# CalebisGross/fresnel

Measured on AMD Instinct MI355X. Metric: composited Gaussian-pixels/sec + train-step ms, 512^2 render, higher is better.
Workload: dtype f32

## Files before the change

### fresnel_amd/_binding.py

```python
import ctypes
import os
import re

_HERE = os.path.dirname(os.path.abspath(__file__))
LIB_PATH = os.environ.get("FGS_LIB", os.path.join(_HERE, "_lib", "libfgs_hip.so"))

FGS_CAMERA_FLOATS = 24
FGS_TILE = 16

_PROTOTYPES = """
int fgs_workspace_bytes(FgsDims* dims, size_t* saved_bytes scratch_bytes)
int fgs_saved_layout(FgsDims* dims, FgsSavedLayout* layout)
int fgs_forward(FgsDims* dims, ptr cameras pos scale quat color opacity phase out_rgb out_depth saved scratch, stream)
int fgs_backward(FgsDims* dims, ptr cameras pos scale quat color opacity phase saved scratch g_rgb g_depth g_pos g_scale g_quat g_color
                 g_opacity g_phase, stream)
int fgs_count_pairs(FgsDims* dims, ptr saved out_pairs, stream)
int fgs_asm_workspace_bytes(FgsAsmDims* dims, size_t* saved_bytes scratch_bytes)
int fgs_asm_forward(FgsAsmDims* dims, ptr cameras pos scale quat color opacity phase wavelengths out_rgb saved scratch, stream)
int fgs_asm_backward(FgsAsmDims* dims, ptr cameras pos scale quat color opacity phase wavelengths saved scratch g_rgb g_pos g_scale
                     g_quat g_color g_opacity g_phase g_wavelengths, stream)
int fgs_wave_workspace_bytes(FgsWaveDims* dims, size_t* saved_bytes scratch_bytes)
int fgs_wave_forward(FgsWaveDims* dims, ptr cameras pos scale quat color opacity phase out_rgb out_depth saved scratch, stream)
int fgs_wave_backward(FgsWaveDims* dims, ptr cameras pos scale quat color opacity phase saved scratch g_rgb g_depth g_pos g_scale
                      g_quat g_color g_opacity g_phase, stream)
int fgs_fourier_workspace_bytes(FgsFourierDims* dims, size_t* saved_bytes scratch_bytes)
int fgs_fourier_forward(FgsFourierDims* dims, ptr cameras pos scale quat color opacity out_rgb saved scratch, stream)
int fgs_fourier_backward(FgsFourierDims* dims, ptr cameras pos scale quat color opacity saved scratch g_rgb g_pos g_scale g_quat
                         g_color g_opacity, stream)
int fgs_asm_propagate_workspace_bytes(int32_t height width channels, size_t* scratch_bytes)
int fgs_asm_propagate_forward(int32_t height width channels, double pixel_pitch, int32_t band_limit, ptr field z wavelengths out
                              spectrum scratch, stream)
int fgs_asm_propagate_backward(int32_t height width channels, double pixel_pitch, int32_t band_limit, ptr spectrum z wavelengths
                               g_out g_field g_z g_wavelengths scratch, stream)
int fgs_spectral_workspace_bytes(FgsSpectralDims* dims, size_t* saved_bytes scratch_bytes)
int fgs_spectral_loss_forward(FgsSpectralDims* dims, ptr rendered target depth wavelength loss saved scratch, stream)
int fgs_spectral_loss_backward(FgsSpectralDims* dims, ptr rendered target depth wavelength saved scratch g_loss g_rendered g_target
                               g_depth g_wavelength, stream)
int fgs_helmholtz_loss_forward(int32_t images height width, float wavelength pixel_spacing, ptr field loss residual scratch, stream)
int fgs_helmholtz_loss_backward(int32_t images height width, float wavelength pixel_spacing, ptr residual g_loss g_field, stream)
size_t fgs_reduction_scratch_bytes()
int fgs_ssim_workspace_bytes(FgsSsimDims* dims, size_t* saved_bytes scratch_bytes)
int fgs_ssim_forward(FgsSsimDims* dims, ptr x y out saved scratch, stream)
int fgs_ssim_backward(FgsSsimDims* dims, ptr x y saved g_out g_x g_y scratch, stream)
int fgs_pixel_loss_workspace_bytes(FgsPixelLossDims* dims, size_t* stats_bytes scratch_bytes)
int fgs_pixel_loss_stage1(FgsPixelLossDims* dims, ptr rendered target rendered_depth target_depth density out stats scratch, stream)
int fgs_pixel_loss_stage2(FgsPixelLossDims* dims, ptr rendered_depth target_depth stats scratch, stream)
int fgs_pixel_loss_stage3(FgsPixelLossDims* dims, ptr rendered_depth target_depth out stats scratch, stream)
int fgs_pixel_loss_forward(FgsPixelLossDims* dims, ptr rendered target rendered_depth target_depth density out stats scratch, stream)
int fgs_pixel_loss_backward(FgsPixelLossDims* dims, ptr rendered target rendered_depth target_depth density stats g_rgb g_boundary
                            g_depth g_rendered g_rendered_depth, stream)
int fgs_head_workspace_bytes(FgsHeadDims* dims, size_t* scratch_bytes)
int fgs_head_forward(FgsHeadDims* dims, ptr raw base_xy base_z pose opacity_mod edge positions scales rotations colors opacities
                     phases, stream)
int fgs_head_backward(FgsHeadDims* dims, ptr raw pose opacity_mod edge g_positions g_scales g_rotations g_colors g_opacities g_phases
                      g_raw g_base_z g_edge g_opacity_mod scratch, stream)
int fgs_nca_workspace_bytes(FgsNcaDims* dims, size_t* scratch_bytes)
int fgs_nca_perceive_forward(FgsNcaDims* dims, ptr state perception neighbors, stream)
int fgs_nca_perceive_backward(FgsNcaDims* dims, ptr neighbors g_perception g_state, stream)
int fgs_nca_update_forward(FgsNcaDims* dims, ptr state delta step_size uniform, float update_prob, ptr new_state, stream)
int fgs_nca_update_backward(FgsNcaDims* dims, ptr delta step_size uniform, float update_prob, ptr g_new_state g_delta g_step_size
                            scratch, stream)
int fgs_saag_workspace_bytes(FgsSaagDims* dims, size_t* scratch_bytes)
int fgs_saag_inputs_forward(FgsSaagDims* dims, ptr features positions scales rotations colors opacities mlp_inputs, stream)
int fgs_saag_refine_forward(FgsSaagDims* dims, ptr raw positions scales rotations colors opacities gains o_positions o_scales
                            o_rotations o_colors o_opacities pos_delta scale_delta color_delta opacity_delta, stream)
int fgs_saag_refine_backward(FgsSaagDims* dims, ptr raw scales rotations colors opacities gains g_positions g_scales g_rotations
                             g_colors g_opacities g_pos_delta g_scale_delta g_color_delta g_opacity_delta g_raw g_gains scratch, stream)
int fgs_physics_workspace_bytes(FgsPhysicsDims* dims, size_t* scratch_bytes)
int fgs_physics_forward(FgsPhysicsDims* dims, ptr raw base_xy base_z wavelength_raw positions scales rotations colors opacities phases
                        range scratch, stream)
int fgs_physics_backward(FgsPhysicsDims* dims, ptr raw base_z wavelength_raw range g_positions g_scales g_rotations g_colors
                         g_opacities g_phases g_raw g_base_z g_wavelength_raw scratch, stream)
int fgs_surface_workspace_bytes(FgsSurfaceDims* dims, FgsSurfaceParams* params, size_t* scratch_bytes)
int fgs_surface_count(FgsSurfaceDims* dims, FgsSurfaceParams* params, ptr depth scratch offsets, stream)
int fgs_surface_emit(FgsSurfaceDims* dims, FgsSurfaceParams* params, ptr depth color scratch offsets o_positions o_scales o_rotations
                     o_colors o_opacities, int64_t capacity, stream)
int fgs_surface_emit_guided(FgsSurfaceDims* dims, FgsSurfaceParams* params, ptr depth color scratch offsets mods, int32_t mods_h mods_w,
                            ptr o_positions o_scales o_rotations o_colors o_opacities point_rows, int64_t capacity, stream)
int fgs_surface_guided_backward_bytes(FgsSurfaceDims* dims, FgsSurfaceParams* params, int32_t mods_h mods_w, size_t* bytes)
int fgs_surface_guided_backward(FgsSurfaceDims* dims, FgsSurfaceParams* params, ptr depth scratch offsets mods, int32_t mods_h mods_w,
                                ptr point_rows g_positions g_scales g_rotations g_opacities g_mods bwd_scratch, stream)
int fgs_match_workspace_bytes(FgsMatchDims* dims, size_t* saved_bytes scratch_bytes)
int fgs_match_forward(FgsMatchDims* dims, ptr pred target pred_keep target_keep terms counts saved scratch, stream)
int fgs_match_backward(FgsMatchDims* dims, ptr pred target saved g_total g_pred scratch, stream)
int fgs_slat_workspace_bytes(int32_t batch voxels per_voxel, size_t* scratch_bytes)
int fgs_slat_head_forward(int32_t batch voxels per_voxel, ptr raw coords gains keep gaussians counts scratch, stream)
int fgs_slat_head_backward(int32_t batch voxels per_voxel, ptr raw coords gains g_gaussians g_raw g_gains scratch, stream)
int fgs_gather_forward(int32_t batch n_in n_out phase_channels, ptr indices pos scale quat color opacity phase o_pos o_scale o_quat
                       o_color o_opacity o_phase, stream)
int fgs_gather_backward(int32_t batch n_in n_out phase_channels, ptr indices g_o_pos g_o_scale g_o_quat g_o_color g_o_opacity
                        g_o_phase g_pos g_scale g_quat g_color g_opacity g_phase, stream)
int fgs_stage_timing_enable(int enable)
int fgs_stage_timing_read(ptr ms count)
str fgs_last_error()
str fgs_version()
"""


def _parse_prototypes(text):
    table = {}
    for ret, name, params in re.findall(r"(\S+) (fgs_\w+)\(([^)]*)\)", text):
        flat = []
        for kind, *names in (group.split() for group in params.split(",") if group.strip()):
            flat += [(kind, n) for n in names or [kind]]
        table[name] = (ret, tuple(flat))
    return table


SIGNATURES = _parse_prototypes(_PROTOTYPES)
EXPORTED_SYMBOLS = list(SIGNATURES)

STAGES = ["project", "depth_sort", "dup_emit", "tile_sort", "tile_ranges", "composite_fwd",
          "composite_bwd", "project_bwd", "splat_fwd", "field_fwd", "field_bwd", "splat_bwd"]


FWD_EXIT_OFF, FWD_EXIT_ON = 0x100, 0x200
BWD_ZERO_OFF, BWD_ZERO_ON = 0x400, 0x800
BWD_TAIL_OFF, BWD_TAIL_ON = 0x2000, 0x4000


class FgsDims(ctypes.Structure):
    _fields_ = [("batch", ctypes.c_int32), ("num_gaussians", ctypes.c_int32),
                ("width", ctypes.c_int32), ("height", ctypes.c_int32),
                ("max_radius", ctypes.c_float), ("background", ctypes.c_float * 3),
                ("use_phase", ctypes.c_int32), ("phase_amplitude", ctypes.c_float),
                ("num_cameras", ctypes.c_int32), ("saturation_skip", ctypes.c_int32),
                ("seg_len", ctypes.c_int32), ("fwd_variant", ctypes.c_int32), ("bin_mode", ctypes.c_int32),
                ("tile_w", ctypes.c_int32), ("sort_mode", ctypes.c_int32), ("dup_capacity", ctypes.c_uint32)]


class FgsSavedLayout(ctypes.Structure):
    _fields_ = [("total_bytes", ctypes.c_size_t), ("rec", ctypes.c_size_t),
                ("depth_key", ctypes.c_size_t), ("tile_count", ctypes.c_size_t),
                ("order", ctypes.c_size_t), ("dup_off", ctypes.c_size_t), ("counters", ctypes.c_size_t),
                ("ranges", ctypes.c_size_t), ("tile_order", ctypes.c_size_t), ("dup_ids", ctypes.c_size_t),
                ("pix_state", ctypes.c_size_t), ("phase_ckpt", ctypes.c_size_t),
                ("dup_capacity", ctypes.c_size_t),
                ("tiles_x", ctypes.c_int32), ("tiles_y", ctypes.c_int32),
                ("seg_off", ctypes.c_size_t), ("seg_tile", ctypes.c_size_t), ("seg_ckpt", ctypes.c_size_t),
                ("seg_capacity", ctypes.c_size_t), ("seg_len", ctypes.c_int32), ("tile_w", ctypes.c_int32),
                ("unit_order", ctypes.c_size_t), ("fwd_open", ctypes.c_size_t),
                ("fwd_close", ctypes.c_size_t), ("rank_of", ctypes.c_size_t)]


class FgsAsmDims(ctypes.Structure):
    _fields_ = [("batch", ctypes.c_int32), ("num_gaussians", ctypes.c_int32),
                ("width", ctypes.c_int32), ("height", ctypes.c_int32),
                ("max_radius", ctypes.c_float), ("background", ctypes.c_float * 3),
                ("num_planes", ctypes.c_int32), ("depth_near", ctypes.c_float),
                ("depth_far", ctypes.c_float), ("focal_depth", ctypes.c_float),
                ("pixel_pitch", ctypes.c_double), ("phase_channels", ctypes.c_int32),
                ("num_cameras", ctypes.c_int32), ("bin_mode", ctypes.c_int32)]


class FgsWaveDims(ctypes.Structure):
    _fields_ = [("batch", ctypes.c_int32), ("num_gaussians", ctypes.c_int32),
                ("width", ctypes.c_int32), ("height", ctypes.c_int32),
                ("max_radius", ctypes.c_float), ("background", ctypes.c_float * 3),
                ("phase_channels", ctypes.c_int32), ("num_cameras", ctypes.c_int32)]


class FgsFourierDims(ctypes.Structure):
    _fields_ = [("batch", ctypes.c_int32), ("num_gaussians", ctypes.c_int32),
                ("width", ctypes.c_int32), ("height", ctypes.c_int32),
                ("background", ctypes.c_float * 3), ("num_cameras", ctypes.c_int32)]


class FgsSpectralDims(ctypes.Structure):
    _fields_ = [("images", ctypes.c_int32), ("channels", ctypes.c_int32), ("height", ctypes.c_int32),
                ("width", ctypes.c_int32), ("mode", ctypes.c_int32), ("cutoff", ctypes.c_float),
                ("high_weight", ctypes.c_float), ("focal_depth", ctypes.c_float), ("reserved", ctypes.c_int32)]


FGS_SSIM_MAX_TAPS = 15
FGS_SSIM_GRAD_X, FGS_SSIM_GRAD_Y, FGS_SSIM_NONNEGATIVE, FGS_SSIM_PER_IMAGE = 1, 2, 4, 8


class FgsSsimDims(ctypes.Structure):
    _fields_ = [("images", ctypes.c_int32), ("channels", ctypes.c_int32), ("height", ctypes.c_int32),
                ("width", ctypes.c_int32), ("taps", ctypes.c_float * FGS_SSIM_MAX_TAPS), ("num_taps", ctypes.c_int32),
                ("c1", ctypes.c_float), ("c2", ctypes.c_float), ("flags", ctypes.c_int32)]


FGS_PIXEL_MAX_BOUNDARIES = 65
FGS_PIXEL_RGB, FGS_PIXEL_DENSITY, FGS_PIXEL_BOUNDARY, FGS_PIXEL_HARD_MASK, FGS_PIXEL_DEPTH = 1, 2, 4, 8, 16
(FGS_PIXEL_STAT_RGB, FGS_PIXEL_STAT_BOUNDARY, FGS_PIXEL_STAT_DEPTH, FGS_PIXEL_STAT_SUM_X, FGS_PIXEL_STAT_SUM_Y,
 FGS_PIXEL_STAT_SSD_X, FGS_PIXEL_STAT_SSD_Y, FGS_PIXEL_STAT_SGN, FGS_PIXEL_STAT_SGN_U) = range(9)
FGS_PIXEL_STAT_SLOTS = 16
FGS_PIXEL_CROSS_RANK = {1: slice(3, 5), 2: slice(5, 7), 3: slice(7, 9)}


class FgsPixelLossDims(ctypes.Structure):
    _fields_ = [("images", ctypes.c_int32), ("height", ctypes.c_int32), ("width", ctypes.c_int32),
                ("flags", ctypes.c_int32), ("world", ctypes.c_int32), ("vlm_weight", ctypes.c_float),
                ("threshold", ctypes.c_float), ("num_boundaries", ctypes.c_int32),
                ("boundaries", ctypes.c_float * FGS_PIXEL_MAX_BOUNDARIES)]


class FgsHeadDims(ctypes.Structure):
    _fields_ = [("batch", ctypes.c_int32), ("points", ctypes.c_int32), ("k_full", ctypes.c_int32),
                ("k_used", ctypes.c_int32), ("channels", ctypes.c_int32), ("xy_gain", ctypes.c_float),
                ("edge_scale_factor", ctypes.c_float), ("edge_opacity_boost", ctypes.c_float)]


class FgsNcaDims(ctypes.Structure):
    _fields_ = [("batch", ctypes.c_int32), ("points", ctypes.c_int32), ("state_dim", ctypes.c_int32), ("k", ctypes.c_int32)]


class FgsSaagDims(ctypes.Structure):
    _fields_ = [("batch", ctypes.c_int32), ("points", ctypes.c_int32), ("channels", ctypes.c_int32),
                ("grid_h", ctypes.c_int32), ("grid_w", ctypes.c_int32),
                ("feat_stride_batch", ctypes.c_int64), ("feat_stride_channel", ctypes.c_int64),
                ("feat_stride_row", ctypes.c_int64), ("residual_scale", ctypes.c_float)]


class FgsPhysicsDims(ctypes.Structure):
    _fields_ = [("batch", ctypes.c_int32), ("points", ctypes.c_int32), ("k_full", ctypes.c_int32), ("k_used", ctypes.c_int32),
                ("xy_gain", ctypes.c_float), ("focal_depth", ctypes.c_float),
                ("wavelength_min", ctypes.c_float), ("wavelength_max", ctypes.c_float)]


FGS_PHYSICS_RANGE_BYTES = 16


class FgsSurfaceDims(ctypes.Structure):
    _fields_ = [("batch", ctypes.c_int32), ("height", ctypes.c_int32), ("width", ctypes.c_int32)]


class FgsSurfaceParams(ctypes.Structure):
    _fields_ = [("fx", ctypes.c_float), ("fy", ctypes.c_float), ("cx", ctypes.c_float), ("cy", ctypes.c_float),
                ("depth_scale", ctypes.c_float), ("subsample", ctypes.c_int32), ("opacity", ctypes.c_float),
                ("normalize_extent", ctypes.c_float),
                ("base_size", ctypes.c_float), ("aspect_ratio", ctypes.c_float), ("edge_threshold", ctypes.c_float),
                ("edge_shrink", ctypes.c_float), ("min_confidence", ctypes.c_float), ("gradient_scale", ctypes.c_float),
                ("normal_strength", ctypes.c_float),
                ("wrap_enabled", ctypes.c_int32), ("wrap_edge_threshold", ctypes.c_float), ("wrap_layers", ctypes.c_int32),
                ("wrap_layer_spacing", ctypes.c_float), ("wrap_opacity_falloff", ctypes.c_float),
                ("wrap_max_angle", ctypes.c_float), ("wrap_aspect", ctypes.c_float),
                ("shell_enabled", ctypes.c_int32), ("shell_thickness", ctypes.c_float), ("shell_back_opacity", ctypes.c_float),
                ("shell_back_darken", ctypes.c_float), ("shell_connect_walls", ctypes.c_int32),
                ("shell_wall_segments", ctypes.c_int32), ("shell_wall_opacity", ctypes.c_float),
                ("shell_edge_threshold", ctypes.c_float),
                ("density_enabled", ctypes.c_int32), ("density_gradient_threshold", ctypes.c_float),
                ("density_extra_count", ctypes.c_int32), ("density_position_jitter", ctypes.c_float),
                ("density_size_variance", ctypes.c_float), ("density_opacity_scale", ctypes.c_float), ("seed", ctypes.c_uint32)]


FGS_SURFACE_STATE_OFFSET = 64
(FGS_SURFACE_KEPT, FGS_SURFACE_BASE, FGS_SURFACE_BACK, FGS_SURFACE_WALLS, FGS_SURFACE_WRAPS, FGS_SURFACE_FILLS) = (1, 2, 4, 8, 16, 32)


FGS_MATCH_TILE = 1024


class FgsMatchDims(ctypes.Structure):
    _fields_ = [("batch", ctypes.c_int32), ("num_pred", ctypes.c_int32), ("num_target", ctypes.c_int32),
                ("w_pos", ctypes.c_float), ("w_scale", ctypes.c_float), ("w_rot", ctypes.c_float),
                ("w_color", ctypes.c_float), ("w_opacity", ctypes.c_float), ("w_coverage", ctypes.c_float)]


class FgsError(RuntimeError):
    pass


_lib = None

_SCALARS = {"int": ctypes.c_int, "int32_t": ctypes.c_int32, "int64_t": ctypes.c_int64, "uint32_t": ctypes.c_uint32,
            "float": ctypes.c_float, "double": ctypes.c_double, "size_t": ctypes.c_size_t, "str": ctypes.c_char_p,
            "ptr": ctypes.c_void_p, "stream": ctypes.c_void_p}


def _ctype(kind):
    if kind.endswith("*"):
        return ctypes.POINTER(_SCALARS.get(kind[:-1]) or globals()[kind[:-1]])
    return _SCALARS[kind]


def load():
    global _lib
    if _lib is not None:
        return _lib
    if not os.path.exists(LIB_PATH):
        raise FgsError(
            f"{LIB_PATH} not found: build it with `python -m fresnel_amd.build` "
            "(hipcc --offload-arch=gfx950).  There is no CPU fallback for the HIP rasterizer.")
    import torch
    lib = ctypes.CDLL(LIB_PATH)
    for name, (ret, params) in SIGNATURES.items():
        fn = getattr(lib, name)
        fn.restype, fn.argtypes = _ctype(ret), [_ctype(kind) for kind, _ in params]
    if b"EXPERIMENT" in lib.fgs_version():
        import sys
        sys.stderr.write(f"fresnel_amd: loaded {LIB_PATH}: {lib.fgs_version().decode()}\n")
    _lib = lib
    return lib


def version():
    return load().fgs_version().decode()


def check(rc, what):
    if rc != 0:
        raise FgsError(f"{what} failed (rc={rc}): {load().fgs_last_error().decode()}")


def make_dims(batch, num_gaussians, width, height, max_radius=64.0, background=(0.0, 0.0, 0.0),
              use_phase=False, phase_amplitude=0.25, num_cameras=1, saturation_skip=False, tuning=None, dup_capacity=0):
    if isinstance(dup_capacity, bool) or int(dup_capacity) != dup_capacity or not 0 <= int(dup_capacity) <= 0xFFFFFFFF:
        raise FgsError(f"dup_capacity must be an integer in [0, 2^32), got {dup_capacity!r}")
    d = FgsDims()
    d.batch, d.num_gaussians, d.width, d.height = int(batch), int(num_gaussians), int(width), int(height)
    d.max_radius = float(max_radius)
    for i in range(3):
        d.background[i] = float(background[i])
    d.use_phase = 1 if use_phase else 0
    d.phase_amplitude = float(phase_amplitude)
    d.num_cameras = int(num_cameras)
    d.saturation_skip = 1 if saturation_skip else 0
    tuning = dict(tuning or {})
    fwd_exit = int(tuning.pop("fwd_exit", 0))
    bwd_zero = int(tuning.pop("bwd_zero", 0))
    bwd_tail = int(tuning.pop("bwd_tail", 0))
    for k, v in tuning.items():
        if k not in ("seg_len", "fwd_variant", "bin_mode", "tile_w", "sort_mode"):
            raise FgsError(f"unknown tuning field {k!r}")
        setattr(d, k, int(v))
    if fwd_exit not in (0, 1, -1) or (fwd_exit and d.fwd_variant < 0):
        raise FgsError(f"fwd_exit must be 0, 1 or -1, and 0 with the row-split forward (fwd_variant < 0), got {fwd_exit!r}")
    if bwd_zero not in (0, 1, -1) or (bwd_zero and d.fwd_variant < 0):
        raise FgsError(f"bwd_zero must be 0, 1 or -1, and 0 with the row-split forward (fwd_variant < 0), got {bwd_zero!r}")
    if bwd_tail not in (0, 1, -1) or (bwd_tail and d.fwd_variant < 0):
        raise FgsError(f"bwd_tail must be 0, 1 or -1, and 0 with the row-split forward (fwd_variant < 0), got {bwd_tail!r}")
    d.fwd_variant |= ({0: 0, 1: FWD_EXIT_ON, -1: FWD_EXIT_OFF}[fwd_exit] | {0: 0, 1: BWD_ZERO_ON, -1: BWD_ZERO_OFF}[bwd_zero]
                      | {0: 0, 1: BWD_TAIL_ON, -1: BWD_TAIL_OFF}[bwd_tail])
    d.dup_capacity = int(dup_capacity)
    return d


_SIZE_OUTS = {name: sum(kind == "size_t*" for kind, _ in params) for name, (_, params) in SIGNATURES.items()}


def sizes(name, *args):
    n = _SIZE_OUTS[name]
    out = [ctypes.c_size_t(0) for _ in range(n)]
    check(getattr(load(), name)(*[ctypes.byref(a) if isinstance(a, ctypes.Structure) else a for a in args],
                                *[ctypes.byref(o) for o in out]), name)
    return out[0].value if n == 1 else tuple(o.value for o in out)


def workspace_bytes(dims):
    return sizes("fgs_workspace_bytes", dims)


def saved_layout(dims):
    L = FgsSavedLayout()
    check(load().fgs_saved_layout(ctypes.byref(dims), ctypes.byref(L)), "fgs_saved_layout")
    return L


def stage_timing_enable(on=True, stages=None):
    mask = 1 if on else 0
    if on and stages is not None:
        mask = 0
        for name in stages:
            mask |= 1 << (STAGES.index(name) + 1)
    check(load().fgs_stage_timing_enable(mask), "fgs_stage_timing_enable")


def stage_timing_read():
    n = len(STAGES)
    ms = (ctypes.c_float * n)()
    cnt = (ctypes.c_int32 * n)()
    check(load().fgs_stage_timing_read(ms, cnt), "fgs_stage_timing_read")
    return {STAGES[i]: (float(ms[i]), int(cnt[i])) for i in range(n)}
```

### fresnel_amd/csrc/fgs_api.hip

```cpp
#include <stdarg.h>
#include <stdio.h>
#include <string.h>
#include "fgs_internal.h"

static thread_local char g_err[512] = "";

void fgs_set_error(const char *fmt, ...) {
    va_list ap;
    va_start(ap, fmt);
    vsnprintf(g_err, sizeof(g_err), fmt, ap);
    va_end(ap);
}

#include <mutex>
#include <stdlib.h>
#include <vector>
namespace {
struct StageRec { int stage; hipEvent_t a, b; };
std::mutex g_tm;
unsigned g_timing = 0;
std::vector<StageRec> g_recs;
std::vector<hipEvent_t> g_pool;
hipEvent_t g_open[FGS_NUM_STAGES];

// ... 27 lines not shown

namespace {
struct FillList { float *p[6]; unsigned long long n[6]; };

__global__ __launch_bounds__(256) void k_overflow_fill(const uint32_t *__restrict__ counters, FillList f, uint32_t word) {
    if (counters[1] == 0u) return;
    const float v = __uint_as_float(word);
    const float4 v4 = make_float4(v, v, v, v);
    const size_t stride = (size_t)gridDim.x * 256, t = (size_t)blockIdx.x * 256 + threadIdx.x;
#pragma unroll
    for (int k = 0; k < 6; ++k) {
        float *q = f.p[k];
        const size_t n = f.n[k], n4 = n >> 2;
        for (size_t i = t; i < n4; i += stride) reinterpret_cast<float4 *>(q)[i] = v4;
        for (size_t i = (n4 << 2) + t; i < n; i += stride) q[i] = v;
    }
}

int launch_overflow_fill(const char *saved, const FgsPlan &p, const FillList &f, uint32_t word, hipStream_t st) {
    size_t total = 0;
    for (int k = 0; k < 6; ++k) total += f.n[k];
    size_t grid = (total / 4 + 255) / 256;
    if (grid > 2048) grid = 2048;
    if (grid < 1) grid = 1;
    hipLaunchKernelGGL(k_overflow_fill, dim3((unsigned)grid), dim3(256), 0, st,
                       reinterpret_cast<const uint32_t *>(saved + p.L.counters), f, word);
    FGS_LAUNCH_CHECK("k_overflow_fill");
    return FGS_OK;
}
}

extern "C" {

const char *fgs_last_error(void) { return g_err; }

int fgs_stage_timing_enable(int enable) {
    std::lock_guard<std::mutex> lk(g_tm);
    g_timing = enable == 1 ? ~0u : ((unsigned)enable >> 1);
    return FGS_OK;
}

int fgs_stage_timing_read(float *ms, int32_t *count) {
    std::lock_guard<std::mutex> lk(g_tm);
    for (const StageRec &r : g_recs) {
        float t = 0.0f;
        if (hipEventSynchronize(r.b) == hipSuccess && hipEventElapsedTime(&t, r.a, r.b) == hipSuccess) {
            if (ms) ms[r.stage] += t;
            if (count) count[r.stage] += 1;
        }
        g_pool.push_back(r.a);
        g_pool.push_back(r.b);
    }
    g_recs.clear();
    return FGS_OK;
}
#ifdef FGS_EXPERIMENT_BUILD
#ifndef FGS_BUILD_DEFINES
#define FGS_BUILD_DEFINES "(defines not recorded)"
#endif
const char *fgs_version(void) { return "fgs-hip 0.3 (gfx950) EXPERIMENT BUILD, NOT THE PRODUCT: " FGS_BUILD_DEFINES; }
#else
const char *fgs_version(void) { return "fgs-hip 0.3 (gfx950)"; }
#endif

int fgs_workspace_bytes(const FgsDims *dims, size_t *saved_bytes, size_t *scratch_bytes) {
    FgsPlan p;
    const int rc = fgs_make_plan(dims, &p);
    if (rc) return rc;
    if (saved_bytes) *saved_bytes = p.L.total_bytes;
    if (scratch_bytes) *scratch_bytes = p.s_total;
    return FGS_OK;
}

int fgs_saved_layout(const FgsDims *dims, FgsSavedLayout *layout) {
    FgsPlan p;
    const int rc = fgs_make_plan(dims, &p);
    if (rc) return rc;
    if (!layout) { fgs_set_error("null layout"); return FGS_EINVAL; }
    *layout = p.L;
    return FGS_OK;
}

int fgs_forward(const FgsDims *dims, const float *cameras, const float *pos, const float *scale,
                const float *quat, const float *color, const float *opacity, const float *phase,
                float *out_rgb, float *out_depth, void *saved, void *scratch, void *stream) {
    FgsPlan p;
    int rc = fgs_make_plan(dims, &p);
    if (rc) return rc;
    if (!cameras || !pos || !scale || !quat || !color || !opacity || !out_rgb || !out_depth || !saved || !scratch) {
        fgs_set_error("fgs_forward: null pointer argument");
        return FGS_EINVAL;
    }
    if (p.d.use_phase && !phase) { fgs_set_error("fgs_forward: use_phase set but phase is NULL"); return FGS_EINVAL; }
    hipStream_t st = reinterpret_cast<hipStream_t>(stream);
    char *sv = reinterpret_cast<char *>(saved), *sc = reinterpret_cast<char *>(scratch);
    fgs_stage_begin(ST_PROJECT, st);
    const bool handoff = (p.d.sort_mode >> 1) == 3;
    if ((rc = fgs_launch_project(p, cameras, pos, scale, quat, color, opacity, sv, st, 0, 0.0f, 0.0f,
                                 handoff ? reinterpret_cast<uint32_t *>(sc + p.s_hist) : nullptr,
                                 (uint32_t)(FGS_SORT_HANDOFF_PASSES * (size_t)p.d.batch * 16 * 256)))) return rc;
    fgs_stage_end(ST_PROJECT, st);
    if ((rc = fgs_launch_binning(p, sv, sc, st))) return rc;
    fgs_stage_begin(ST_COMPOSITE_FWD, st);
    if ((rc = fgs_launch_composite_fwd(p, phase, sv, out_rgb, out_depth, st))) return rc;
    fgs_stage_end(ST_COMPOSITE_FWD, st);
    if (p.capacity_hinted) {
        const size_t hw = (size_t)p.d.width * p.d.height, B = p.d.batch;
        const FillList f = {{out_rgb, out_depth, nullptr, nullptr, nullptr, nullptr}, {B * 3 * hw, B * hw, 0, 0, 0, 0}};
        if ((rc = launch_overflow_fill(sv, p, f, 0x7FC00000u, st))) return rc;
    }
    return FGS_OK;
}

int fgs_backward(const FgsDims *dims, const float *cameras, const float *pos, const float *scale,
                 const float *quat, const float *color, const float *opacity, const float *phase,
                 const void *saved, void *scratch, const float *g_rgb, const float *g_depth,
                 float *g_pos, float *g_scale, float *g_quat, float *g_color, float *g_opacity,
                 float *g_phase, void *stream) {
    FgsPlan p;
    int rc = fgs_make_plan(dims, &p);
    if (rc) return rc;
    if (!cameras || !pos || !scale || !quat || !color || !opacity || !saved || !scratch || !g_rgb || !g_depth ||
        !g_pos || !g_scale || !g_quat || !g_color || !g_opacity) {
        fgs_set_error("fgs_backward: null pointer argument");
        return FGS_EINVAL;
    }
    if (p.d.use_phase && (!phase || !g_phase)) {
        fgs_set_error("fgs_backward: use_phase set but phase/g_phase is NULL");
        return FGS_EINVAL;
    }
    hipStream_t st = reinterpret_cast<hipStream_t>(stream);
    const char *sv = reinterpret_cast<const char *>(saved);
    char *sc = reinterpret_cast<char *>(scratch);
    fgs_stage_begin(ST_COMPOSITE_BWD, st);
    if ((rc = fgs_launch_composite_bwd(p, phase, sv, sc, g_rgb, g_depth, g_phase, st))) return rc;
    fgs_stage_end(ST_COMPOSITE_BWD, st);
    fgs_stage_begin(ST_PROJECT_BWD, st);
    if ((rc = fgs_launch_project_bwd(p, cameras, pos, scale, quat, sv,
                                     reinterpret_cast<const float *>(sc + p.s_grows), g_pos, g_scale, g_quat,
                                     g_color, g_opacity, p.d.use_phase ? g_phase : nullptr, st,
                                     reinterpret_cast<float *>(sc + p.s_rsum),
                                     p.bwd_tail ? reinterpret_cast<const uint32_t *>(sc + p.s_zero_from) : nullptr)))
        return rc;
    fgs_stage_end(ST_PROJECT_BWD, st);
    if (p.capacity_hinted) {
        const size_t bn = (size_t)p.d.batch * p.d.num_gaussians;
        const FillList f = {{g_pos, g_scale, g_quat, g_color, g_opacity, p.d.use_phase ? g_phase : nullptr},
                            {bn * 3, bn * 3, bn * 4, bn * 3, bn, p.d.use_phase ? bn : 0}};
        if ((rc = launch_overflow_fill(sv, p, f, 0u, st))) return rc;
    }
    return FGS_OK;
}

int fgs_count_pairs(const FgsDims *dims, const void *saved, uint64_t *out_pairs, void *stream) {
    FgsPlan p;
    const int rc = fgs_make_plan(dims, &p);
    if (rc) return rc;
    if (!saved || !out_pairs) { fgs_set_error("fgs_count_pairs: null pointer"); return FGS_EINVAL; }
    return fgs_launch_count_pairs(p, reinterpret_cast<const char *>(saved), out_pairs,
                                  reinterpret_cast<hipStream_t>(stream));
}

}
```

### fresnel_amd/csrc/fgs_composite.hip

```cpp
#include <type_traits>
#include "fgs_internal.h"
#include "fgs_wave.h"

#if (defined(FGS_BWD_DYN_LDS) || defined(FGS_BWD_WIDE_WAVES) || defined(FGS_PHASE_SCAN) || defined(FGS_CKPT_NT) || defined(FGS_PHASE_WAVE_BLOCKS) || \
     defined(FGS_BWD_UNIT_TRACE) || defined(FGS_BWD_TILE_ORDER) || defined(FGS_FWD_HEAD_ENTRIES)) && !defined(FGS_EXPERIMENT_BUILD)
#error "work-split / timing switches of this unit are for experiment builds: python -m fresnel_amd.build --define ... (sets FGS_EXPERIMENT_BUILD; fgs_version() then says so)"
#endif

namespace {

typedef float v2f __attribute__((ext_vector_type(2)));
constexpr float FGS_SATURATION_EPS = 2.98023223876953125e-8f;
constexpr float NEG_HALF_LOG2E = -0.72134752044448170368f;
constexpr float ALPHA_MAX = 0.99f;
constexpr float INV_ALPHA_MAX = 1.0f / 0.99f;
constexpr float PHASE_KAPPA = 2.0f * 3.14159f;

__device__ __forceinline__ float phase_cos(float x) {
    const float y = x - 1.57079632679489661923f, y2 = y * y;
    float p = 2.6089300414764439e-6f;
    p = p * y2 - 1.9811111665926607e-4f;
    p = p * y2 + 8.3330881539788702e-3f;
    p = p * y2 - 1.6666660461917662e-1f;
    return -(y + y * (y2 * p));
// ... 314 lines not shown
            Cr[s] = nt_load(k); Cg[s] = nt_load(k + PL); Cb[s] = nt_load(k + 2 * PL); T[s] = nt_load(k + 3 * PL); Dm[s] = nt_load(k + 4 * PL);
            nt_store(k + 3 * PL, 1.0f - T[s]);
        }
        wstart = c.start + hs * seg_len;
    }
    const uint32_t wend = (!REST || mine) ? pend : wstart;
    for (uint32_t base = wstart; base < wend; base += 64) {
        const uint32_t n = min(64u, wend - base);
        if (base != wstart && ((base - c.start) % seg_len) == 0) {
            float *ck = slot0 + (size_t)((base - c.start) / seg_len) * SLOT;
#pragma unroll
            for (int s = 0; s < 4; ++s) ckpt_store<PL>(ck + cell(s), BlendState{Cr[s], Cg[s], Cb[s], T[s], Dm[s]});
        }
        blend_fwd_chunk(sh0[wave], sh1[wave], sh2[wave], lane, base, n, X0, c.Y0, dup_ids, rec, ln, T, Cr, Cg, Cb, Dm);
    }
    const uint32_t last = nseg ? (nseg - 1) / spp : 0u;
    if (NP > 1 && nseg > spp) {
        if (active && part != 0 && (!REST || mine)) {
            float *ck = (part == last) ? slot0 : slot0 + (size_t)((part + 1) * spp) * SLOT;
#pragma unroll
            for (int s = 0; s < 4; ++s) ckpt_store<PL>(ck + cell(s), BlendState{Cr[s], Cg[s], Cb[s], T[s], Dm[s]});
        }
        __threadfence_block();
        __syncthreads();
        if (part != 0 || (REST && !mine)) return;
        {
            float *ck = slot0 + (size_t)spp * SLOT;
#pragma unroll
            for (int s = 0; s < 4; ++s) ckpt_store<PL>(ck + cell(s), BlendState{Cr[s], Cg[s], Cb[s], T[s], Dm[s]});
        }
        for (uint32_t pp = 1; pp <= last; ++pp) {
            const float *src = (pp == last) ? slot0 : slot0 + (size_t)((pp + 1) * spp) * SLOT;
            float *dst = slot0 + (size_t)((pp + 1) * spp) * SLOT;
#pragma unroll
            for (int s = 0; s < 4; ++s) {
                const BlendState acc = compose(BlendState{Cr[s], Cg[s], Cb[s], T[s], Dm[s]}, ckpt_load<PL>(src + cell(s)));
                Cr[s] = acc.Cr; Cg[s] = acc.Cg; Cb[s] = acc.Cb; T[s] = acc.T; Dm[s] = acc.D;
                if (pp != last) ckpt_store<PL>(dst + cell(s), acc);
            }
        }
    } else if (part != 0 || (REST && !mine)) {
        return;
    }
    const size_t HW = (size_t)W * H;
#pragma unroll
    for (int s = 0; s < 4; ++s) {
        const uint32_t px = X0 + 8u * (s & 1) + lx, py = c.Y0 + 8u * (s >> 1) + ly;
        if (px < W && py < H)
            pixel_store(pix_state, out_rgb, out_depth, c.b, HW, (size_t)py * W + px, bg0, bg1, bg2, Cr[s], Cg[s], Cb[s], 1.0f - T[s],
                        T[s], Dm[s]);
    }
}

template <int WIDE>
__global__ __launch_bounds__(64 * (1 + WIDE)) __attribute__((amdgpu_waves_per_eu(8, 8))) void k_blend_fwd_head(
    uint32_t tiles, uint32_t tiles_x, uint32_t W, uint32_t H, float bg0, float bg1, float bg2,
    const uint32_t *__restrict__ tile_order, const uint32_t *__restrict__ ranges,
    const uint32_t *__restrict__ dup_ids, const float *__restrict__ rec, float *__restrict__ pix_state,
    float *__restrict__ out_rgb, float *__restrict__ out_depth, const uint32_t *__restrict__ seg_off,
    float *__restrict__ seg_ckpt, uint32_t seg_len, uint32_t order_groups, uint32_t *__restrict__ fwd_open, uint32_t head_segs,
    uint32_t np, const uint32_t *__restrict__ fwd_max, uint32_t max_recs, uint32_t *__restrict__ fwd_close) {
    constexpr int NW = 1 + WIDE;
    constexpr int TSX = WIDE ? 4 : 2;
    constexpr int PL = 2 * TSX * 64, SLOT = 5 * PL;
    __shared__ float4 sh0[NW][64], sh1[NW][64], sh2[NW][64];
    const uint32_t slot_in_order = order_groups > 1u ? fgs_xcd_remap(blockIdx.x, gridDim.x) : blockIdx.x;
    const TileCtx c = tile_ctx_of(tile_order[slot_in_order], tiles, tiles_x, ranges, 8u * TSX);
    const uint32_t lane = threadIdx.x & 63u;
    const uint32_t half = WIDE ? __builtin_amdgcn_readfirstlane(threadIdx.x >> 6) : 0u;
    const uint32_t X0 = c.X0 + 16u * half;
    const uint32_t lx = lane & 7u, ly = lane >> 3;
    const uint32_t len = c.end - c.start;
    const uint32_t nseg = (len + seg_len - 1) / seg_len;
    const uint32_t spp = (nseg + np - 1) / np;
    const uint32_t hs = np == 1u ? nseg : min(spp, head_segs);
    const uint32_t hlen = min(len, hs * seg_len);
    float *slot0 = seg_ckpt + (size_t)seg_off[c.tile] * SLOT + 2u * half * 64u + lane;
    auto cell = [](int s) { return ((s >> 1) * TSX + (s & 1)) * 64; };
    uint32_t kcb = 0u, kdb = 0u;
    {
        const uint32_t *fm = fwd_max + (size_t)c.b * max_recs * 2u;
        for (uint32_t i = lane; i < max_recs; i += 64u) { kcb = max(kcb, fm[2u * i]); kdb = max(kdb, fm[2u * i + 1u]); }
#pragma unroll
        for (int o = 32; o > 0; o >>= 1) { kcb = max(kcb, (uint32_t)__shfl_xor(kcb, o, 64)); kdb = max(kdb, (uint32_t)__shfl_xor(kdb, o, 64)); }
        kcb = max(max(kcb, __float_as_uint(bg0) & 0x7FFFFFFFu), max(__float_as_uint(bg1) & 0x7FFFFFFFu, __float_as_uint(bg2) & 0x7FFFFFFFu));
    }
    const float Kc = __uint_as_float(__builtin_amdgcn_readfirstlane(kcb)), Kd = __uint_as_float(__builtin_amdgcn_readfirstlane(kdb));
    bool inframe[4];
#pragma unroll
    for (int s = 0; s < 4; ++s) inframe[s] = X0 + 8u * (s & 1) + lx < W && c.Y0 + 8u * (s >> 1) + ly < H;
    float T[4], Cr[4], Cg[4], Cb[4], Dm[4];
#pragma unroll
    for (int s = 0; s < 4; ++s) { T[s] = 1.0f; Cr[s] = 0; Cg[s] = 0; Cb[s] = 0; Dm[s] = 0; }
    BlendLane ln = {lx, 16u + ly, (float)(X0 + lx), (float)(X0 + lx + 8u), (float)(c.Y0 + ly)};
    asm("" : "+v"(ln.fx0), "+v"(ln.fx1), "+v"(ln.fy0));
    constexpr float Q = 1.490116119384765625e-8f;
    uint32_t done = 0;
    bool closed = false;
    while (done < hlen && !closed) {
        if (done != 0u && (done % seg_len) == 0) {
            float *ck = slot0 + (size_t)(done / seg_len) * SLOT;
#pragma unroll
            for (int s = 0; s < 4; ++s) ckpt_store<PL>(ck + cell(s), BlendState{Cr[s], Cg[s], Cb[s], T[s], Dm[s]});
        }
        const uint32_t n = min(64u, hlen - done);
        blend_fwd_chunk(sh0[half], sh1[half], sh2[half], lane, c.start + done, n, X0, c.Y0, dup_ids, rec, ln, T, Cr, Cg, Cb, Dm);
        done += n;
        bool veto = false;
#pragma unroll
        for (int s = 0; s < 4; ++s) {
            const float tc = T[s] * Kc;
            const bool ok = T[s] <= Q && tc < Q * fabsf(Cr[s]) && tc < Q * fabsf(Cg[s]) && tc < Q * fabsf(Cb[s]) && T[s] * Kd < Q * fabsf(Dm[s]);
            veto |= inframe[s] && !ok;
        }
        closed = __ballot(veto) == 0ull;
    }
    const bool finished = closed || done == len;
    const uint32_t kclose = (done + seg_len - 1) / seg_len;
    const bool close_slot = closed && kclose < nseg;
    if (lane == 0) {
        fwd_open[2u * c.tile + half] = finished ? 0u : 1u;
        fwd_close[2u * c.tile + half] = close_slot ? kclose : 0xFFFFFFFFu;
    }
    if (!WIDE && lane == 1) fwd_close[2u * c.tile + 1u] = 0xFFFFFFFFu;
    if (!finished) {
        float *ck = slot0 + (size_t)hs * SLOT;
#pragma unroll
        for (int s = 0; s < 4; ++s) {
            float *k = ck + cell(s);
            nt_store(k, Cr[s]); nt_store(k + PL, Cg[s]); nt_store(k + 2 * PL, Cb[s]); nt_store(k + 3 * PL, T[s]); nt_store(k + 4 * PL, Dm[s]);
        }
        return;
    }
    const size_t HW = (size_t)W * H;
#pragma unroll
    for (int s = 0; s < 4; ++s) {
        const uint32_t px = X0 + 8u * (s & 1) + lx, py = c.Y0 + 8u * (s >> 1) + ly;
        if (px < W && py < H)
            pixel_store(pix_state, out_rgb, out_depth, c.b, HW, (size_t)py * W + px, bg0, bg1, bg2, Cr[s], Cg[s], Cb[s], 1.0f - T[s],
                        T[s], Dm[s]);
    }
    if (close_slot) {
        float *ck = slot0 + (size_t)kclose * SLOT;
#pragma unroll
        for (int s = 0; s < 4; ++s) ckpt_store<PL>(ck + cell(s), BlendState{Cr[s], Cg[s], Cb[s], T[s], Dm[s]});
    }
}

__shared__ float4 bwd_sh0[CH], bwd_sh1[CH], bwd_sh2[CH];
__shared__ uint32_t bwd_she[CH];
__shared__ __attribute__((aligned(16))) float bwd_red[10 * FGS_RED_PITCH];
__shared__ __attribute__((aligned(16))) float bwd_red_pairs[12 * FGS_RED_PITCH];
#define FGS_BWD_G __attribute__((address_space(1)))

template <int NSX, bool DEAD>
__device__ __forceinline__ void composite_bwd_walk(const TileCtx &c, uint32_t lane, uint32_t lx, uint32_t ly, uint32_t dcap, uint32_t alive,
                                                   const uint32_t *__restrict__ dup_ids, const float *__restrict__ rec,
                                                   const uint32_t *__restrict__ dup_off, float *__restrict__ grad_rows,
                                                   const float (&gr)[2 * NSX], const float (&gg)[2 * NSX], const float (&gb)[2 * NSX],
                                                   const float (&gd)[2 * NSX], float (&S)[2 * NSX], float (&T)[2 * NSX]) {
    constexpr int NS = 2 * NSX;
    constexpr bool ROW_MOMENTS = NSX == 4;
    auto &sh0 = bwd_sh0; auto &sh1 = bwd_sh1; auto &sh2 = bwd_sh2; auto &she = bwd_she;
    auto &red = *[]() { if constexpr (NSX == 4) return &bwd_red_pairs; else return &bwd_red; }();
    const uint32_t shx = lx, shy = 16u + ly;
    float fx0 = (float)(c.X0 + lx), fy0 = (float)(c.Y0 + ly);
    asm("" : "+v"(fx0), "+v"(fy0));
    uint32_t e_prev = ~0u;
    auto reduce_parked = [&]() {
        const float tot = wave_sum_addtid_finish(red, lane, 10u);
        if ((lane & 3u) == 3u && lane < 4u * FGS_BLEND_ROW_FLOATS && e_prev < dcap) ((FGS_BWD_G float *)grad_rows)[(size_t)e_prev * FGS_BLEND_ROW_FLOATS + (lane >> 2)] = tot;
    };
    constexpr bool PAIRS = NSX == 4;
    constexpr uint32_t DSUMS = 6, DROWS = PAIRS ? 2 : 1, DZERO = FGS_BLEND_ROW_FLOATS - DSUMS;
    static_assert(4 * DSUMS * DROWS + DROWS * DZERO <= 64, "dead walk: one lane per zero float behind the sums' lanes");
    [[maybe_unused]] uint32_t e_prevB = ~0u;
    [[maybe_unused]] auto reduce_parked_dead = [&]() {
        const float tot = wave_sum_addtid_finish(red, lane, DSUMS * DROWS);
        const uint32_t k = lane >> 2, z = lane - 4u * DSUMS * DROWS;
        const bool sum_lane = (lane & 3u) == 3u && k < DSUMS * DROWS, zero_lane = lane >= 4u * DSUMS * DROWS && z < DROWS * DZERO;
        const bool second = sum_lane ? k >= DSUMS : z >= DZERO;
        const uint32_t col = sum_lane ? (second ? k - DSUMS : k) : DSUMS + (second ? z - DZERO : z);
        const uint32_t e = PAIRS && second ? e_prevB : e_prev;
        if ((sum_lane || zero_lane) && e < dcap) ((FGS_BWD_G float *)grad_rows)[(size_t)e * FGS_BLEND_ROW_FLOATS + col] = tot;
    };
    struct DeadTerms {
        float ca, dya, dyb, bdya, bdyb, cyya, cyyb, dxs[NSX];
        uint32_t mxs[NSX], my0, my1, msk, cflag;
    };
    [[maybe_unused]] auto dead_terms = [&](const float4 &q0, const float4 &q1, const float4 &q2, const uint32_t fl) {
        DeadTerms t;
        t.msk = fl & alive;
        t.cflag = fl & 256u;
        asm("" : "+s"(t.cflag));
        const uint32_t cbits = __float_as_uint(q2.z), rbits = __float_as_uint(q2.w);
        const float cbc = q0.w, cd = q1.x, lop = q1.y;
        t.ca = q0.z;
        const float dxa = fx0 - q0.x;
        t.dya = fy0 - q0.y; t.dyb = t.dya + 8.0f;
        t.bdya = cbc * t.dya; t.bdyb = cbc * t.dyb; t.cyya = fmaf(cd * t.dya, t.dya, lop); t.cyyb = fmaf(cd * t.dyb, t.dyb, lop);
        asm("" : "+v"(t.bdya), "+v"(t.bdyb), "+v"(t.cyya), "+v"(t.cyyb));
#pragma unroll
        for (int col = 0; col < NSX; ++col) {
            t.mxs[col] = (uint32_t)__builtin_amdgcn_sbfe((int)cbits, shx + 8u * col, 1);
            t.dxs[col] = dxa + 8.0f * col;
        }
        t.my0 = (uint32_t)__builtin_amdgcn_sbfe((int)rbits, shy, 1); t.my1 = (uint32_t)__builtin_amdgcn_sbfe((int)rbits, shy + 8u, 1);
        return t;
    };
    [[maybe_unused]] auto dead_passes = [&](const DeadTerms &t, float (&vals)[DSUMS]) {
        float v_mx = 0, v_my = 0, v_ca = 0, v_cbc = 0, v_cd = 0, v_op = 0;
        float mA[2] = {0.0f, 0.0f}, mB[2] = {0.0f, 0.0f}, mC[2] = {0.0f, 0.0f};
        auto pass = [&](const int s) {
            const int col = s % NSX, row = s / NSX;
            const float dx = t.dxs[col], dy = row ? t.dyb : t.dya;
            const uint32_t mk = t.mxs[col] & (row ? t.my1 : t.my0);
            const float tt = __builtin_fmaf(dx, t.ca, row ? t.bdyb : t.bdya);
            const float a1 = blend_alpha1(__builtin_fmaf(tt, dx, row ? t.cyyb : t.cyya), mk);
            float dalpha = S[s] * __builtin_amdgcn_rcpf(a1 - INV_ALPHA_MAX);
            uint32_t cf = t.cflag;
            asm("" : "+s"(cf));
            if (!cf) dalpha = select_lt1(a1, dalpha);
            float dG = dalpha * a1;
            asm("" : "+v"(dG));
            if constexpr (ROW_MOMENTS) {
                mA[row] = __builtin_fmaf(dalpha, a1, mA[row]);
                float dmx = dG * dx;
                asm("" : "+v"(dmx));
                mB[row] = __builtin_fmaf(dG, dx, mB[row]); mC[row] = __builtin_fmaf(dmx, dx, mC[row]);
            } else {
                v_op = __builtin_fmaf(dalpha, a1, v_op);
                float dmx = dG * dx, dmy = dG * dy;
                asm("" : "+v"(dmx), "+v"(dmy));
                v_mx = __builtin_fmaf(dG, dx, v_mx); v_my = __builtin_fmaf(dG, dy, v_my);
                v_ca = __builtin_fmaf(dmx, dx, v_ca); v_cbc = __builtin_fmaf(dmx, dy, v_cbc); v_cd = __builtin_fmaf(dmy, dy, v_cd);
            }
        };
#pragma unroll
        for (int s = 0; s < NS; ++s) {
            if (!((t.msk >> s) & 1u)) continue;
            pass(s);
        }
        if constexpr (ROW_MOMENTS) {
            v_op = mA[0] + mA[1]; v_mx = mB[0] + mB[1]; v_ca = mC[0] + mC[1];
            float t0 = t.dya * mA[0], t1 = t.dyb * mA[1];
            asm("" : "+v"(t0), "+v"(t1));
            float p0 = t0 * t.dya, pb = mB[0] * t.dya;
            asm("" : "+v"(p0), "+v"(pb));
            v_my = __builtin_fmaf(mA[1], t.dyb, t0);
            v_cd = __builtin_fmaf(t1, t.dyb, p0);
            v_cbc = __builtin_fmaf(mB[1], t.dyb, pb);
        }
        vals[0] = v_mx; vals[1] = v_my; vals[2] = v_ca; vals[3] = v_cbc; vals[4] = v_cd; vals[5] = v_op;
    };
    [[maybe_unused]] auto dead_chunk = [&](const uint32_t n) {
        for (uint32_t j = 0; j < n; j += DROWS) {
            const float4 a0 = sh0[j], a1 = sh1[j], a2 = sh2[j];
            uint32_t eA = __builtin_amdgcn_readfirstlane(she[j]), eB = ~0u;
            float4 b0 = a0, b1 = a1, b2 = a2;
            if constexpr (PAIRS) {
                b0 = sh0[j + 1]; b1 = sh1[j + 1]; b2 = sh2[j + 1];
                eB = __builtin_amdgcn_readfirstlane(she[j + 1]);
            }
            reduce_parked_dead();
            asm volatile("" : "+s"(eA), "+s"(eB));
            const bool paired = PAIRS && j + 1 < n;
            e_prev = eA; e_prevB = paired ? eB : ~0u;
            const uint32_t flA = __builtin_amdgcn_readfirstlane(__float_as_uint(a2.w));
            const DeadTerms ta = dead_terms(a0, a1, a2, flA);
            float va[DSUMS];
            if constexpr (PAIRS) {
                const uint32_t flB = paired ? __builtin_amdgcn_readfirstlane(__float_as_uint(b2.w)) : 0u;
                const DeadTerms tb = dead_terms(b0, b1, b2, flB);
                float vb[DSUMS];
                dead_passes(ta, va);
                addtid_park(red, va);
                dead_passes(tb, vb);
                addtid_park(red + DSUMS * FGS_RED_PITCH, vb);
            } else {
                dead_passes(ta, va);
                addtid_park(red, va);
            }
        }
    };
    for (uint32_t base = c.start; base < c.end; base += CH) {
        const uint32_t n = __builtin_amdgcn_readfirstlane(min((uint32_t)CH, c.end - base));
        uint32_t sl;
        asm volatile("v_mbcnt_lo_u32_b32 %0, -1, 0\n\tv_mbcnt_hi_u32_b32 %0, -1, %0" : "=v"(sl));
        if (sl < n) {
            const uint32_t gid = ((FGS_BWD_G const uint32_t *)dup_ids)[base + sl];
            const float4 *r = reinterpret_cast<const float4 *>(rec + (size_t)gid * FGS_REC_FLOATS);
            float4 q2 = r[2];
            const uint32_t bbx = __float_as_uint(q2.z), bby = __float_as_uint(q2.w);
            she[sl] = fgs_emission_slot<8 * NSX>(c.tx, c.ty, gid, bbx, bby, dup_off);
            float4 q0 = r[0], q1 = r[1];
            const bool conic_ok = q0.z > 0.0f && q1.x > 0.0f && 3.996f * q0.z * q1.x > q0.w * q0.w;
            uint32_t flags, cbits;
            stage_decode_w<NSX>(c.X0, c.Y0, bbx, bby, q1.y, flags, cbits, conic_ok);
            blend_stage_fold(q0, q1, q2, flags, cbits, fgs_opacity_floored(q1.y) ? FGS_FOLD_FLOOR_LOG2 : blend_lop(q1.y));
            sh0[sl] = q0; sh1[sl] = q1; sh2[sl] = q2;
        }
        __syncthreads();
        if constexpr (DEAD) dead_chunk(n);
        for (uint32_t j = 0; !DEAD && j < n; ++j) {
            const float4 q0 = sh0[j], q1 = sh1[j], q2 = sh2[j];
            uint32_t e = __builtin_amdgcn_readfirstlane(she[j]);
            reduce_parked();
            asm volatile("" : "+s"(e));
            e_prev = e;
            const uint32_t fl = __builtin_amdgcn_readfirstlane(__float_as_uint(q2.w));
            const uint32_t msk = fl & alive;
            const uint32_t cbits = __float_as_uint(q2.z), rbits = __float_as_uint(q2.w);
            const float ca = q0.z, cbc = q0.w, cd = q1.x, lop = q1.y;
            const float dxa = fx0 - q0.x, dya = fy0 - q0.y, dyb = dya + 8.0f;
            float bdya = cbc * dya, bdyb = cbc * dyb, cyya = fmaf(cd * dya, dya, lop), cyyb = fmaf(cd * dyb, dyb, lop);
            asm("" : "+v"(bdya), "+v"(bdyb), "+v"(cyya), "+v"(cyyb));
            float v_mx = 0, v_my = 0, v_ca = 0, v_cbc = 0, v_cd = 0, v_op = 0, v_r = 0, v_g = 0, v_b = 0, v_d = 0;
            float mA[2] = {0.0f, 0.0f}, mB[2] = {0.0f, 0.0f}, mC[2] = {0.0f, 0.0f};
            {
                uint32_t cflag = fl & 256u;
                asm("" : "+s"(cflag));
                uint32_t mxs[NSX];
                float dxs[NSX];
#pragma unroll
                for (int col = 0; col < NSX; ++col) {
                    mxs[col] = (uint32_t)__builtin_amdgcn_sbfe((int)cbits, shx + 8u * col, 1);
                    dxs[col] = dxa + 8.0f * col;
                }
                const uint32_t my0 = (uint32_t)__builtin_amdgcn_sbfe((int)rbits, shy, 1), my1 = (uint32_t)__builtin_amdgcn_sbfe((int)rbits, shy + 8u, 1);
                auto pass = [&](const int s, const uint32_t mk) {
                    const int col = s % NSX, row = s / NSX;
                    const float dx = dxs[col], dy = row ? dyb : dya;
                    const float t = ca * dx + (row ? bdyb : bdya);
                    const float a1 = blend_alpha1(t * dx + (row ? cyyb : cyya), mk);
                    const float w = a1 * T[s];
                    const float q = gr[s] * q1.z + gg[s] * q1.w + gb[s] * q2.x + gd[s] * q2.y;
                    S[s] -= w * q;
                    float dalpha = T[s] * q - S[s] * __builtin_amdgcn_rcpf(INV_ALPHA_MAX - a1);
                    T[s] = fmaf(w, -ALPHA_MAX, T[s]);
                    uint32_t cf = cflag;
                    asm("" : "+s"(cf));
                    if (!cf) dalpha = select_lt1(a1, dalpha);
                    const float dG = dalpha * a1;
                    if constexpr (ROW_MOMENTS) {
                        mA[row] += dG;
                        const float dmx = dG * dx;
                        mB[row] += dmx; mC[row] += dmx * dx;
                    } else {
                        v_op += dG;
                        const float dmx = dG * dx, dmy = dG * dy;
                        v_mx += dmx; v_my += dmy;
                        v_ca += dmx * dx; v_cbc += dmx * dy; v_cd += dmy * dy;
                    }
                    v_r += w * gr[s]; v_g += w * gg[s]; v_b += w * gb[s]; v_d += w * gd[s];
                };
#pragma unroll
                for (int s = 0; s < NS; ++s) {
                    if (!((msk >> s) & 1u)) continue;
                    pass(s, mxs[s % NSX] & (s / NSX ? my1 : my0));
                }
                if constexpr (ROW_MOMENTS) {
                    v_op = mA[0] + mA[1]; v_mx = mB[0] + mB[1]; v_ca = mC[0] + mC[1];
                    const float t0 = dya * mA[0], t1 = dyb * mA[1];
                    v_my = t0 + t1;
                    v_cd = dya * t0 + dyb * t1;
                    v_cbc = dya * mB[0] + dyb * mB[1];
                }
            }
            {
                const float vals[10] = {v_mx, v_my, v_ca, v_cbc, v_cd, v_op, v_r, v_g, v_b, v_d};
                addtid_park(red, vals);
            }
        }
        __syncthreads();
    }
    if constexpr (DEAD) reduce_parked_dead(); else reduce_parked();
}

template <int NSX>
struct BwdDeadArgs {
    TileCtx c;
    uint32_t dcap;
    uint32_t alive;
    const uint32_t *dup_ids; const float *rec; const uint32_t *dup_off; float *grad_rows;
    float S[2 * NSX];
};
template <int NSX>
__device__ __attribute__((noinline)) void composite_bwd_dead_walk(BwdDeadArgs<NSX> a) {
    const uint32_t lane = threadIdx.x;
    float z[2 * NSX] = {}, T[2 * NSX] = {};
    const uint32_t alive = __builtin_amdgcn_readfirstlane(a.alive);
    composite_bwd_walk<NSX, true>(a.c, lane, lane & 7u, lane >> 3, a.dcap, alive, a.dup_ids, a.rec, a.dup_off, a.grad_rows, z, z, z, z,
                                  a.S, T);
}

template <int NSX>
__device__ __attribute__((noinline)) void composite_bwd_zero_rows(TileCtx c, uint32_t dcap, const uint32_t *__restrict__ dup_ids,
                                                                  const float *__restrict__ rec, const uint32_t *__restrict__ dup_off,
                                                                  float *__restrict__ grad_rows) {
    static_assert(FGS_BLEND_ROW_FLOATS % 2 == 0 && FGS_BLEND_ROW_FLOATS >= 4, "zero rows: stored as pairs, floats 1 and 3 in the first two");
    const float fy7 = (float)(c.Y0 + 7u);
    for (uint32_t i = c.start + threadIdx.x; i < c.end; i += 64) {
        const uint32_t gid = dup_ids[i];
        const float *r = rec + (size_t)gid * FGS_REC_FLOATS;
        const float4 q2 = reinterpret_cast<const float4 *>(r)[2];
        const uint32_t e = fgs_emission_slot<8 * NSX>(c.tx, c.ty, gid, __float_as_uint(q2.z), __float_as_uint(q2.w), dup_off);
        uint32_t zy = 0u;
        if constexpr (NSX == 4) {
            float dya = fy7 - r[1];
            asm("" : "+v"(dya));
            if (dya + 8.0f < 0.0f) zy = 0x80000000u;
        }
        if (e < dcap) {
            uint2 *row = reinterpret_cast<uint2 *>(grad_rows + (size_t)e * FGS_BLEND_ROW_FLOATS);
            row[0] = make_uint2(0u, zy); row[1] = make_uint2(0u, zy);
#pragma unroll
            for (int q = 2; q < FGS_BLEND_ROW_FLOATS / 2; ++q) row[q] = make_uint2(0u, 0u);
        }
    }
}

template <int NSX>
__device__ __forceinline__ bool composite_bwd_prologue(const TileCtx &c, uint32_t unit, uint32_t seg, uint32_t rebase_seg,
                                                       const uint32_t (&kclose)[NSX / 2], uint32_t lane, uint32_t lx, uint32_t ly,
                                                       uint32_t W, uint32_t H, float bg0, float bg1, float bg2,
                                                       const float *__restrict__ seg_ckpt, const float *__restrict__ pix_state,
                                                       const float *__restrict__ g_rgb, const float *__restrict__ g_depth,
                                                       float (&gr)[2 * NSX], float (&gg)[2 * NSX], float (&gb)[2 * NSX],
                                                       float (&gd)[2 * NSX], float (&S)[2 * NSX], float (&T)[2 * NSX]) {
    constexpr int NS = 2 * NSX, PL = NS * 64, SLOT = 5 * PL;
    const size_t HW = (size_t)W * H;
    bool live_px = false;
#pragma unroll
    for (int s = 0; s < NS; ++s) {
        const uint32_t px = c.X0 + 8u * (s % NSX) + lx, py = c.Y0 + 8u * (s / NSX) + ly;
        gr[s] = gg[s] = gb[s] = gd[s] = S[s] = 0.0f;
        T[s] = 1.0f;
        if (px < W && py < H) {
            const PixelGrad g = pixel_grad_load(pix_state, g_rgb, g_depth, c.b, HW, (size_t)py * W + px, bg0, bg1, bg2);
            gr[s] = g.gr; gg[s] = g.gg; gb[s] = g.gb; gd[s] = g.gd;
            const float bgs = __builtin_fmaf(gb[s], bg2, __builtin_fmaf(gg[s], bg1, gr[s] * bg0));
            S[s] = __builtin_fmaf(bgs, g.Tf, __builtin_fmaf(gd[s], g.D, __builtin_fmaf(gb[s], g.Cb, __builtin_fmaf(gg[s], g.Cg, gr[s] * g.Cr))));
        }
        if (seg) {
            const bool behind = seg >= kclose[(s % NSX) >> 1];
            const size_t own = behind ? (size_t)unit - seg + kclose[(s % NSX) >> 1] : (size_t)unit;
            BlendState st = ckpt_load<PL>(seg_ckpt + own * SLOT + s * 64 + lane);
            if (rebase_seg != seg && !behind) {
                const size_t slot = (size_t)unit - seg + rebase_seg;
                st = compose(ckpt_load<PL>(seg_ckpt + slot * SLOT + s * 64 + lane), st);
            }
            T[s] = st.T;
            S[s] -= __builtin_fmaf(gd[s], st.D, __builtin_fmaf(gb[s], st.Cb, __builtin_fmaf(gg[s], st.Cg, gr[s] * st.Cr)));
            if (px < W && py < H && T[s] != 0.0f) live_px = true;
        }
    }
    return live_px;
}

template <int NSX>
__device__ __forceinline__ uint32_t composite_bwd_nonzero_subtiles(const float (&S)[2 * NSX]) {
    uint32_t walk = 0u;
#pragma unroll
    for (int s = 0; s < 2 * NSX; ++s)
        if (__ballot((__float_as_uint(S[s]) & 0x7FFFFFFFu) != 0u) != 0ull) walk |= 1u << s;
    return walk;
}

template <int NSX>
__global__ __launch_bounds__(64) void k_bwd_tail_verdict(
    uint32_t ntiles, uint32_t tiles, uint32_t tiles_x, uint32_t W, uint32_t H, float bg0, float bg1, float bg2, uint32_t dcap,
    const uint32_t *__restrict__ counters, const uint32_t *__restrict__ seg_off, const float *__restrict__ seg_ckpt,
    const uint32_t *__restrict__ ranges, const uint32_t *__restrict__ dup_ids, const float *__restrict__ pix_state,
    const float *__restrict__ g_rgb, const float *__restrict__ g_depth, const uint32_t *__restrict__ fwd_close,
    const uint32_t *__restrict__ rank_of, uint32_t *__restrict__ zero_from) {
    constexpr int NS = 2 * NSX;
    const uint32_t tile = blockIdx.x;
    if (tile >= ntiles) return;
    const uint32_t lane = threadIdx.x;
    uint32_t verdict = 0xFFFFFFFFu;
    const TileCtx c = tile_ctx_of(tile, tiles, tiles_x, ranges, 8u * NSX);
    const uint32_t seg_len = counters[4];
    uint32_t kclose[NSX / 2], seg = 0u;
#pragma unroll
    for (int h = 0; h < NSX / 2; ++h) { kclose[h] = fwd_close[2u * tile + h]; seg = max(seg, kclose[h]); }
    const uint32_t len = c.end - c.start;
    const bool tail = c.end > c.start && seg_len != 0u && seg != 0xFFFFFFFFu && seg != 0u && (unsigned long long)seg * seg_len < len &&
                      (unsigned long long)c.start + (unsigned long long)seg * seg_len < dcap;
    if (tail) {
        float gr[NS], gg[NS], gb[NS], gd[NS], S[NS], T[NS];
        const bool live_px = composite_bwd_prologue<NSX>(c, seg_off[tile] + seg, seg, seg, kclose, lane, lane & 7u, lane >> 3, W, H, bg0, bg1,
                                                         bg2, seg_ckpt, pix_state, g_rgb, g_depth, gr, gg, gb, gd, S, T);
        if (__ballot(live_px) == 0ull && composite_bwd_nonzero_subtiles<NSX>(S) == 0u) verdict = rank_of[dup_ids[c.start + seg * seg_len]];
    }
    if (lane == 0) zero_from[tile] = verdict;
}

__global__ __launch_bounds__(256) void k_bwd_tail_min(uint32_t tiles, uint32_t *__restrict__ zero_from) {
    __shared__ uint32_t part[4];
    const uint32_t *z = zero_from + (size_t)blockIdx.x * tiles;
    uint32_t m = 0xFFFFFFFFu;
    for (uint32_t t = threadIdx.x; t < tiles; t += 256u) m = min(m, z[t]);
#pragma unroll
    for (int o = 32; o > 0; o >>= 1) m = min(m, (uint32_t)__shfl_xor(m, o, 64));
    if ((threadIdx.x & 63u) == 0u) part[threadIdx.x >> 6] = m;
    __syncthreads();
    if (threadIdx.x == 0) zero_from[(size_t)gridDim.x * tiles + blockIdx.x] = min(min(part[0], part[1]), min(part[2], part[3]));
}

#ifndef FGS_BWD_WIDE_WAVES
#define FGS_BWD_WIDE_WAVES 5
#endif
#ifndef FGS_BWD_DYN_LDS
#define FGS_BWD_DYN_LDS 0
#endif
#ifdef FGS_BWD_UNIT_TRACE
#define FGS_BWD_TRACE_PARAM , unsigned long long *__restrict__ trace
#define FGS_BWD_TRACE_EXIT(dead)                                                                                        \
    do {                                                                                                                \
        if (threadIdx.x == 0) {                                                                                         \
            trace[3 * (size_t)blockIdx.x + 1] = wall_clock64();                                                         \
            trace[3 * (size_t)blockIdx.x + 2] = (unsigned long long)unit | ((unsigned long long)(dead) << 32) | (1ull << 63); \
        }                                                                                                               \
    } while (0)
#else
#define FGS_BWD_TRACE_PARAM
#define FGS_BWD_TRACE_EXIT(dead) do { } while (0)
#endif
template <int NSX>
__global__ __launch_bounds__(64) __attribute__((amdgpu_waves_per_eu(NSX == 2 ? 6 : FGS_BWD_WIDE_WAVES, NSX == 2 ? 6 : FGS_BWD_WIDE_WAVES))) void k_composite_bwd(
    uint32_t tiles, uint32_t tiles_x, uint32_t W, uint32_t H, float bg0, float bg1, float bg2, uint32_t dcap,
    const uint32_t *__restrict__ counters, const uint32_t *__restrict__ seg_off,
    const uint32_t *__restrict__ seg_tile, const float *__restrict__ seg_ckpt, const uint32_t *__restrict__ ranges,
    const uint32_t *__restrict__ dup_ids, const float *__restrict__ rec, const uint32_t *__restrict__ dup_off,
    const float *__restrict__ pix_state, const float *__restrict__ g_rgb, const float *__restrict__ g_depth,
    float *__restrict__ grad_rows, float t_eps, const uint32_t *__restrict__ unit_order,
    const uint32_t *__restrict__ fwd_close, uint32_t zero_units, const uint32_t *__restrict__ zero_from FGS_BWD_TRACE_PARAM) {
    constexpr int NS = 2 * NSX, PL = NS * 64, SLOT = 5 * PL;
    const uint32_t num_units = counters[2];
    if (blockIdx.x >= num_units) return;
#ifdef FGS_BWD_UNIT_TRACE
    if (threadIdx.x == 0) trace[3 * (size_t)blockIdx.x] = wall_clock64();
#endif
#ifdef FGS_BWD_TILE_ORDER
    const uint32_t unit = fgs_xcd_remap(blockIdx.x, num_units);
#else
    const uint32_t unit = unit_order[fgs_xcd_remap(blockIdx.x, num_units)];
#endif
    const uint32_t seg_len = counters[4];
    const uint32_t fwd_parts = (int32_t)counters[5] > 1 ? counters[5] : 0u;
    const uint32_t unit_tile = seg_tile[unit];
    uint32_t kclose[NSX / 2];
#pragma unroll
    for (int h = 0; h < NSX / 2; ++h) kclose[h] = 0xFFFFFFFFu;
    if (fwd_close) {
#pragma unroll
        for (int h = 0; h < NSX / 2; ++h) kclose[h] = fwd_close[2u * unit_tile + h];
    }
    const uint32_t seg = unit - seg_off[unit_tile];
    if (zero_from) {
        bool tail = true;
#pragma unroll
        for (int h = 0; h < NSX / 2; ++h) tail = tail && seg >= kclose[h];
        if (tail && zero_from[unit_tile] != 0xFFFFFFFFu) {
            FGS_BWD_TRACE_EXIT(5);
            return;
        }
    }
    TileCtx c = tile_ctx_of(unit_tile, tiles, tiles_x, ranges, 8u * NSX);
    uint32_t rebase_seg = seg;
    if (fwd_parts > 1) {
        const uint32_t nseg = (c.end - c.start + seg_len - 1) / seg_len;
        const uint32_t spp = (nseg + fwd_parts - 1) / fwd_parts, first = seg / spp * spp;
        if (first != 0) rebase_seg = first;
    }
    c.start += seg * seg_len;
    c.end = min(c.end, c.start + seg_len);
    const uint32_t lane = threadIdx.x;
    const uint32_t lx = lane & 7u, ly = lane >> 3;
    if (t_eps > 0.0f) {
        const uint32_t live = reinterpret_cast<const uint32_t *>(seg_ckpt + (size_t)seg_off[unit_tile] * SLOT)[0];
        if (seg >= live) {
            for (uint32_t i = c.start + lane; i < c.end; i += 64) {
                const uint32_t gid = dup_ids[i];
                const float4 q2 = reinterpret_cast<const float4 *>(rec + (size_t)gid * FGS_REC_FLOATS)[2];
                const uint32_t e = fgs_emission_slot<8 * NSX>(c.tx, c.ty, gid, __float_as_uint(q2.z), __float_as_uint(q2.w), dup_off);
                if (e < dcap) {
                    float2 *row = reinterpret_cast<float2 *>(grad_rows + (size_t)e * FGS_BLEND_ROW_FLOATS);
#pragma unroll
                    for (int q = 0; q < FGS_BLEND_ROW_FLOATS / 2; ++q) row[q] = make_float2(0.0f, 0.0f);
                }
            }
            FGS_BWD_TRACE_EXIT(2);
            return;
        }
    }
    float gr[NS], gg[NS], gb[NS], gd[NS], S[NS], T[NS];
    const bool live_px = composite_bwd_prologue<NSX>(c, unit, seg, rebase_seg, kclose, lane, lx, ly, W, H, bg0, bg1, bg2, seg_ckpt, pix_state,
                                                     g_rgb, g_depth, gr, gg, gb, gd, S, T);
    const bool dead_unit = seg != 0 && !(t_eps > 0.0f) && __ballot(live_px) == 0ull;
    uint32_t alive = (1u << NS) - 1u;
    if (t_eps > 0.0f) {
        alive = 0u;
#pragma unroll
        for (int s = 0; s < NS; ++s)
            if (__ballot(T[s] >= t_eps) != 0ull) alive |= 1u << s;
    }
    if (dead_unit) {
        uint32_t walk = (1u << NS) - 1u;
        if (zero_units) {
            walk = composite_bwd_nonzero_subtiles<NSX>(S);
            if (walk == 0u) {
                composite_bwd_zero_rows<NSX>(c, dcap, dup_ids, rec, dup_off, grad_rows);
                FGS_BWD_TRACE_EXIT(3);
                return;
            }
        }
        BwdDeadArgs<NSX> a;
        a.c = c; a.dcap = dcap; a.alive = walk; a.dup_ids = dup_ids; a.rec = rec; a.dup_off = dup_off; a.grad_rows = grad_rows;
#pragma unroll
        for (int s = 0; s < NS; ++s) a.S[s] = S[s];
        composite_bwd_dead_walk<NSX>(a);
        FGS_BWD_TRACE_EXIT(walk == (1u << NS) - 1u ? 1 : 4);
        return;
    }
    composite_bwd_walk<NSX, false>(c, lane, lx, ly, dcap, alive, dup_ids, rec, dup_off, grad_rows, gr, gg, gb, gd, S, T);
    FGS_BWD_TRACE_EXIT(0);
}

#ifndef FGS_PHASE_SCAN
#define FGS_PHASE_SCAN 64
#endif
static_assert(FGS_PHASE_SCAN <= 64 && FGS_PHASE_SCAN % FGS_PHASE_CKPT == 0, "scan block");
#ifndef FGS_PHASE_WAVE_BLOCKS
#define FGS_PHASE_WAVE_BLOCKS 0
#endif
__device__ __forceinline__ bool phase_wave_block(uint32_t total_slots, uint32_t &slot, uint32_t &wave) {
    const uint32_t L = blockIdx.x;
    slot = (L >> 5) * 8u + (L & 7u);
    wave = (L >> 3) & 3u;
    return slot < total_slots;
}
struct PhaseRec {
    float4 a[FGS_PHASE_SCAN];
    float4 b[FGS_PHASE_SCAN];
    float4 c[FGS_PHASE_SCAN];
};

template <bool FWD>
__device__ __forceinline__ unsigned long long phase_scan(PhaseRec &st, uint32_t *rows, uint32_t gid, bool have, uint32_t sx,
                                                         uint32_t sy, const TileCtx &c,
                                                         const float *__restrict__ rec, const float *__restrict__ phase,
                                                         const uint32_t *__restrict__ dup_off) {
    float4 q0, q1, q2;
    uint32_t bits = 0, e = 0;
    if (have) {
        const float4 *r = reinterpret_cast<const float4 *>(rec + (size_t)gid * FGS_REC_FLOATS);
        q0 = r[0]; q1 = r[1]; q2 = r[2];
        const uint32_t bbx = __float_as_uint(q2.z), bby = __float_as_uint(q2.w);
        const int x0 = (int)(bbx & 0xFFFFu), x1 = (int)(bbx >> 16), y0 = (int)(bby & 0xFFFFu), y1 = (int)(bby >> 16);
        const int lx0 = max(x0 - (int)sx, 0), lx1 = min(x1 - (int)sx, 8), ly0 = max(y0 - (int)sy, 0), ly1 = min(y1 - (int)sy, 8);
        const uint32_t cm = lx1 > lx0 ? ((1u << (lx1 - lx0)) - 1u) << lx0 : 0u;
        const uint32_t rm = ly1 > ly0 ? ((1u << (ly1 - ly0)) - 1u) << ly0 : 0u;
        bits = (cm && rm) ? (cm | (rm << 8)) : 0u;
        if (!FWD) e = fgs_emission_slot<FGS_TILE>(c.tx, c.ty, gid, bbx, bby, dup_off);
    }
    const unsigned long long touched = __ballot(bits != 0u);
    if (bits) {
        const uint32_t slot = __builtin_amdgcn_mbcnt_hi((uint32_t)(touched >> 32), __builtin_amdgcn_mbcnt_lo((uint32_t)touched, 0u));
        q0.z *= NEG_HALF_LOG2E; q0.w *= NEG_HALF_LOG2E; q1.x *= NEG_HALF_LOG2E;
        st.a[slot] = q0; st.b[slot] = q1;
        st.c[slot] = make_float4(q2.x, q2.y, phase[gid], __uint_as_float(bits));
        if (!FWD) rows[slot] = e;
    }
    __builtin_amdgcn_wave_barrier();
    return touched;
}

__device__ __forceinline__ float phase_step(const float4 &q0, const float4 &q1, const float4 &q2, uint32_t lx, uint32_t ly, float fpx,
                                            float fpy, float base_amp, float amp, float &A, float &Ph) {
    const uint32_t bits = __float_as_uint(q2.w);
    const uint32_t mk = (uint32_t)__builtin_amdgcn_sbfe((int)bits, lx, 1) & (uint32_t)__builtin_amdgcn_sbfe((int)bits, 8u + ly, 1);
    const float dx = fpx - q0.x, dy = fpy - q0.y;
    const float mm = (q0.z * dx) * dx + (q0.w * dx) * dy + (q1.x * dy) * dy;
    float alpha = __builtin_amdgcn_exp2f(mm) * q1.y;
    float pd = fabsf(q2.z - Ph);
    pd = fminf(pd, 1.0f - pd);
    alpha *= base_amp + amp * phase_cos(pd * PHASE_KAPPA);
    alpha = __builtin_amdgcn_fmed3f(alpha, 0.0f, ALPHA_MAX);
    alpha = __uint_as_float(__float_as_uint(alpha) & mk);
    const float w = alpha * (1.0f - A);
    A += w;
    const float pc = w / fmaxf(A, 1e-6f);
    Ph = Ph * (1.0f - pc) + q2.z * pc;
    return w;
}

__global__ __launch_bounds__(FGS_PHASE_WAVE_BLOCKS ? 64 : 256) void k_phase_fwd(
    uint32_t tiles, uint32_t tiles_x, uint32_t W, uint32_t H, float bg0, float bg1, float bg2, float amp,
    const uint32_t *__restrict__ tile_order, const uint32_t *__restrict__ ranges, const uint32_t *__restrict__ dup_ids,
    const float *__restrict__ rec, const float *__restrict__ phase, float *__restrict__ pix_state,
    float *__restrict__ phase_ckpt, float *__restrict__ out_rgb, float *__restrict__ out_depth, uint32_t total_slots) {
    constexpr int PCK = FGS_PHASE_CKPT;
    __shared__ PhaseRec st4[FGS_PHASE_WAVE_BLOCKS ? 1 : 4];
#if FGS_PHASE_WAVE_BLOCKS
    uint32_t pslot, wave;
    if (!phase_wave_block(total_slots, pslot, wave)) return;
    const TileCtx c = tile_ctx_of(tile_order[pslot], tiles, tiles_x, ranges);
    const uint32_t lane = threadIdx.x & 63u;
    PhaseRec &st = st4[0];
#else
    const TileCtx c = tile_ctx(tiles, tiles_x, tile_order, ranges);
    const uint32_t lane = threadIdx.x & 63u;
    const uint32_t wave = __builtin_amdgcn_readfirstlane(threadIdx.x >> 6);
    PhaseRec &st = st4[wave];
#endif
    const uint32_t lx = lane & 7u, ly = lane >> 3;
    const uint32_t sx = c.X0 + 8u * (wave & 1u), sy = c.Y0 + 8u * (wave >> 1);
    float fpx = (float)(sx + lx), fpy = (float)(sy + ly);
    asm("" : "+v"(fpx), "+v"(fpy));
    float A = 0.0f, Ph = 0.0f, Cr = 0.0f, Cg = 0.0f, Cb = 0.0f, Dm = 0.0f;
    const float base_amp = 1.0f - amp;
    constexpr uint32_t SCAN = FGS_PHASE_SCAN;
    uint32_t gid_next = (lane < SCAN && c.start + lane < c.end) ? dup_ids[c.start + lane] : 0u;
    for (uint32_t base = c.start; base < c.end; base += SCAN) {
        const uint32_t gid = gid_next;
        const bool have = lane < SCAN && base + lane < c.end;
        if (lane < SCAN && base + SCAN + lane < c.end) gid_next = dup_ids[base + SCAN + lane];
        const unsigned long long touched = phase_scan<true>(st, nullptr, gid, have, sx, sy, c, rec, phase, nullptr);
        const uint32_t nt = (uint32_t)__popcll(touched);
        for (uint32_t j0 = 0; j0 < nt; j0 += PCK) {
            const size_t slot = (size_t)(c.start / PCK) + (base - c.start + j0) / PCK + c.tile;
            float *ck = phase_ckpt + slot * 512 + lane;
            ck[wave * 64] = A; ck[(4 + wave) * 64] = Ph;
            const uint32_t m = min((uint32_t)PCK, nt - j0);
#pragma unroll
            for (int k = 0; k < PCK; ++k) {
                if (k >= (int)m) break;
                const float4 q0 = st.a[j0 + k], q1 = st.b[j0 + k], q2 = st.c[j0 + k];
                const float w = phase_step(q0, q1, q2, lx, ly, fpx, fpy, base_amp, amp, A, Ph);
                Cr += w * q1.z; Cg += w * q1.w; Cb += w * q2.x; Dm += w * q2.y;
            }
        }
        __builtin_amdgcn_wave_barrier();
    }
    const uint32_t px = sx + lx, py = sy + ly;
    if (px < W && py < H) {
        const size_t HW = (size_t)W * H, o = (size_t)py * W + px;
        pixel_store(pix_state, out_rgb, out_depth, c.b, HW, o, bg0, bg1, bg2, Cr, Cg, Cb, A, 1.0f - A, Dm);
        nt_store(pix_state + (size_t)c.b * 6 * HW + o + 5 * HW, Ph);
    }
}

__global__ __launch_bounds__(FGS_PHASE_WAVE_BLOCKS ? 64 : 256) void k_phase_bwd(
    uint32_t tiles, uint32_t tiles_x, uint32_t W, uint32_t H, float bg0, float bg1, float bg2, float amp,
    uint32_t dcap, const uint32_t *__restrict__ tile_order, const uint32_t *__restrict__ ranges,
    const uint32_t *__restrict__ dup_ids, const float *__restrict__ rec, const float *__restrict__ phase,
    const uint32_t *__restrict__ dup_off, const float *__restrict__ pix_state,
    const float *__restrict__ phase_ckpt, const float *__restrict__ g_rgb, const float *__restrict__ g_depth,
    float *__restrict__ grad_rows, uint32_t total_slots) {
    constexpr int PCK = FGS_PHASE_CKPT;
    constexpr int NWB = FGS_PHASE_WAVE_BLOCKS ? 1 : 4;
    __shared__ PhaseRec st4[NWB];
    __shared__ uint32_t rows4[NWB][FGS_PHASE_SCAN];
    __shared__ __attribute__((aligned(16))) float red4[NWB][11 * FGS_RED_PITCH];
#if FGS_PHASE_WAVE_BLOCKS
    uint32_t pslot, wave;
    if (!phase_wave_block(total_slots, pslot, wave)) return;
    const TileCtx c = tile_ctx_of(tile_order[pslot], tiles, tiles_x, ranges);
    const uint32_t lane = threadIdx.x & 63u;
    PhaseRec &st = st4[0];
    uint32_t *rows = rows4[0];
    float *red = red4[0];
#else
    const TileCtx c = tile_ctx(tiles, tiles_x, tile_order, ranges);
    const uint32_t lane = threadIdx.x & 63u;
    const uint32_t wave = __builtin_amdgcn_readfirstlane(threadIdx.x >> 6);
    PhaseRec &st = st4[wave];
    uint32_t *rows = rows4[wave];
    float *red = red4[wave];
// ... 94 lines not shown
    }
}

}

template <typename T>
static T *fgs_at(const char *base, size_t offset) {
    return reinterpret_cast<T *>(const_cast<char *>(base) + offset);
}

#ifndef FGS_FWD_HEAD_ENTRIES
#define FGS_FWD_HEAD_ENTRIES 384u
#endif

int fgs_launch_composite_fwd(const FgsPlan &p, const float *phase, char *saved, float *out_rgb,
                             float *out_depth, hipStream_t st) {
    const uint32_t grid = (uint32_t)p.d.batch * p.tiles;
    const uint32_t tiles = (uint32_t)p.tiles, tiles_x = (uint32_t)p.L.tiles_x, W = (uint32_t)p.d.width, H = (uint32_t)p.d.height;
    const float bg0 = p.d.background[0], bg1 = p.d.background[1], bg2 = p.d.background[2];
    const uint32_t *ranges = fgs_at<const uint32_t>(saved, p.L.ranges), *dup_ids = fgs_at<const uint32_t>(saved, p.L.dup_ids);
    const uint32_t *tile_order = fgs_at<const uint32_t>(saved, p.L.tile_order), *seg_off = fgs_at<const uint32_t>(saved, p.L.seg_off);
    const float *rec = fgs_at<const float>(saved, p.L.rec);
    float *pix = fgs_at<float>(saved, p.L.pix_state), *seg_ckpt = fgs_at<float>(saved, p.L.seg_ckpt);
    if (p.d.use_phase) {
        float *phase_ckpt = fgs_at<float>(saved, p.L.phase_ckpt);
        hipLaunchKernelGGL(k_phase_fwd, dim3(FGS_PHASE_WAVE_BLOCKS ? (grid + 7u) / 8u * 32u : grid), dim3(FGS_PHASE_WAVE_BLOCKS ? 64 : 256), 0, st,
                           tiles, tiles_x, W, H, bg0, bg1, bg2, p.d.phase_amplitude, tile_order, ranges, dup_ids, rec, phase, pix,
                           phase_ckpt, out_rgb, out_depth, grid);
        FGS_LAUNCH_CHECK("k_phase_fwd");
        return FGS_OK;
    }
    const float t_eps = p.d.saturation_skip ? FGS_SATURATION_EPS : 0.0f;
    const int fw = p.fwd_waves;
    if (const int np = p.fwd_parts) {
        const uint32_t seg_len = (uint32_t)p.L.seg_len, order_groups = (uint32_t)p.order_groups;
        const bool exiting = p.fwd_exit;
        uint32_t *fwd_open = exiting ? fgs_at<uint32_t>(saved, p.L.fwd_open) : nullptr;
        const uint32_t head_segs = FGS_FWD_HEAD_ENTRIES / seg_len > 0u ? FGS_FWD_HEAD_ENTRIES / seg_len : 1u;
        if (exiting) {
            const uint32_t *fwd_max = fgs_at<const uint32_t>(saved, p.s_fwd_max);
            const uint32_t max_recs = ((uint32_t)p.d.num_gaussians + 255u) / 256u;
            uint32_t *fwd_close = fgs_at<uint32_t>(saved, p.L.fwd_close);
#define FGS_HEAD_LAUNCH(WD)                                                                                               \
    hipLaunchKernelGGL((k_blend_fwd_head<WD>), dim3(grid), dim3(64 * (1 + WD)), 0, st, tiles, tiles_x, W, H, bg0, bg1, bg2, tile_order, \
                       ranges, dup_ids, rec, pix, out_rgb, out_depth, seg_off, seg_ckpt, seg_len, order_groups, fwd_open, head_segs, \
                       (uint32_t)np, fwd_max, max_recs, fwd_close)
            if (p.tile_w == 32) FGS_HEAD_LAUNCH(1); else FGS_HEAD_LAUNCH(0);
#undef FGS_HEAD_LAUNCH
            FGS_LAUNCH_CHECK("k_blend_fwd_head");
            if (np == 1) return FGS_OK;
        }
#define FGS_PARTS_LAUNCH(NP, WD)                                                                                          \
    do {                                                                                                                  \
        if (exiting)                                                                                                      \
            hipLaunchKernelGGL((k_blend_fwd_parts<NP, WD, true>), dim3(grid), dim3(64 * NP * (1 + WD)), 0, st, tiles, tiles_x, W, H, bg0, \
                               bg1, bg2, tile_order, ranges, dup_ids, rec, pix, out_rgb, out_depth, seg_off, seg_ckpt, seg_len,   \
                               order_groups, fwd_open, head_segs);                                                        \
        else                                                                                                              \
            hipLaunchKernelGGL((k_blend_fwd_parts<NP, WD, false>), dim3(grid), dim3(64 * NP * (1 + WD)), 0, st, tiles, tiles_x, W, H, bg0, \
                               bg1, bg2, tile_order, ranges, dup_ids, rec, pix, out_rgb, out_depth, seg_off, seg_ckpt, seg_len,   \
                               order_groups, fwd_open, head_segs);                                                        \
    } while (0)
        if (p.tile_w == 32) {
            if (np == 1) FGS_PARTS_LAUNCH(1, 1); else if (np == 2) FGS_PARTS_LAUNCH(2, 1); else if (np == 4) FGS_PARTS_LAUNCH(4, 1);
            else FGS_PARTS_LAUNCH(8, 1);
        } else {
            if (np == 1) FGS_PARTS_LAUNCH(1, 0); else if (np == 2) FGS_PARTS_LAUNCH(2, 0); else if (np == 4) FGS_PARTS_LAUNCH(4, 0);
            else if (np == 8) FGS_PARTS_LAUNCH(8, 0); else FGS_PARTS_LAUNCH(16, 0);
        }
#undef FGS_PARTS_LAUNCH
        FGS_LAUNCH_CHECK("k_blend_fwd_parts");
        return FGS_OK;
    }
#define FGS_FWD_LAUNCH(FW, SK)                                                                                            \
    hipLaunchKernelGGL((k_composite_fwd<FW, SK>), dim3(grid), dim3(64 * FW), 0, st, tiles, tiles_x, W, H, bg0, bg1, bg2, tile_order, \
                       ranges, dup_ids, rec, pix, out_rgb, out_depth, seg_off, seg_ckpt, t_eps)
    if (t_eps > 0.0f) {
        if (fw == 1) FGS_FWD_LAUNCH(1, true); else if (fw == 4) FGS_FWD_LAUNCH(4, true); else FGS_FWD_LAUNCH(2, true);
    } else {
        if (fw == 1) FGS_FWD_LAUNCH(1, false); else if (fw == 4) FGS_FWD_LAUNCH(4, false); else FGS_FWD_LAUNCH(2, false);
    }
#undef FGS_FWD_LAUNCH
    FGS_LAUNCH_CHECK("k_composite_fwd");
    return FGS_OK;
}

#ifdef FGS_BWD_UNIT_TRACE
static unsigned long long *g_bwd_trace = nullptr;
static uint32_t g_bwd_trace_slots = 0, g_bwd_trace_last = 0;
extern "C" long fgs_bwd_unit_trace(unsigned long long *host, size_t slots) {
    if (!g_bwd_trace || hipDeviceSynchronize() != hipSuccess) return -1;
    const size_t n = slots < g_bwd_trace_last ? slots : g_bwd_trace_last;
    if (hipMemcpy(host, g_bwd_trace, n * 24, hipMemcpyDeviceToHost) != hipSuccess) return -1;
    return (long)n;
}
#endif

int fgs_launch_composite_bwd(const FgsPlan &p, const float *phase, const char *saved, char *scratch,
                             const float *g_rgb, const float *g_depth, float *g_phase, hipStream_t st) {
    (void)g_phase;
    const uint32_t grid = (uint32_t)p.d.batch * p.tiles;
    const uint32_t tiles = (uint32_t)p.tiles, tiles_x = (uint32_t)p.L.tiles_x, W = (uint32_t)p.d.width, H = (uint32_t)p.d.height;
    const uint32_t dcap = (uint32_t)p.L.dup_capacity;
    const float bg0 = p.d.background[0], bg1 = p.d.background[1], bg2 = p.d.background[2];
    const uint32_t *ranges = fgs_at<const uint32_t>(saved, p.L.ranges), *dup_ids = fgs_at<const uint32_t>(saved, p.L.dup_ids);
    const uint32_t *dup_off = fgs_at<const uint32_t>(saved, p.L.dup_off);
    const float *rec = fgs_at<const float>(saved, p.L.rec), *pix = fgs_at<const float>(saved, p.L.pix_state);
    float *grad_rows = fgs_at<float>(scratch, p.s_grows);
    if (p.d.use_phase) {
        const uint32_t *tile_order = fgs_at<const uint32_t>(saved, p.L.tile_order);
        const float *phase_ckpt = fgs_at<const float>(saved, p.L.phase_ckpt);
        hipLaunchKernelGGL(k_phase_bwd, dim3(FGS_PHASE_WAVE_BLOCKS ? (grid + 7u) / 8u * 32u : grid), dim3(FGS_PHASE_WAVE_BLOCKS ? 64 : 256), 0, st,
                           tiles, tiles_x, W, H, bg0, bg1, bg2, p.d.phase_amplitude, dcap, tile_order, ranges, dup_ids, rec, phase,
                           dup_off, pix, phase_ckpt, g_rgb, g_depth, grad_rows, grid);
        FGS_LAUNCH_CHECK("k_phase_bwd");
        return FGS_OK;
    }
    const uint32_t ugrid = (uint32_t)p.L.seg_capacity;
    const uint32_t *counters = fgs_at<const uint32_t>(saved, p.L.counters), *seg_off = fgs_at<const uint32_t>(saved, p.L.seg_off);
    const uint32_t *seg_tile = fgs_at<const uint32_t>(saved, p.L.seg_tile);
    const float *seg_ckpt = fgs_at<const float>(saved, p.L.seg_ckpt);
    const float t_eps = p.d.saturation_skip ? FGS_SATURATION_EPS : 0.0f;
    if (!p.has_unit_order) { fgs_set_error("k_composite_bwd: the plan has no unit_order table"); return FGS_EINVAL; }
    const uint32_t *unit_order = fgs_at<const uint32_t>(saved, p.L.unit_order);
    const uint32_t *fwd_close = p.fwd_exit ? fgs_at<const uint32_t>(saved, p.L.fwd_close) : nullptr;
    uint32_t *zero_from = p.bwd_tail ? fgs_at<uint32_t>(scratch, p.s_zero_from) : nullptr;
    if (zero_from) {
        const uint32_t *rank_of = fgs_at<const uint32_t>(saved, p.L.rank_of);
#define FGS_VERDICT_LAUNCH(NSXV)                                                                                          \
    hipLaunchKernelGGL(k_bwd_tail_verdict<NSXV>, dim3(grid), dim3(64), 0, st, grid, tiles, tiles_x, W, H, bg0, bg1, bg2, dcap, counters, \
                       seg_off, seg_ckpt, ranges, dup_ids, pix, g_rgb, g_depth, fwd_close, rank_of, zero_from)
        if (p.tile_w == 32) FGS_VERDICT_LAUNCH(4); else FGS_VERDICT_LAUNCH(2);
#undef FGS_VERDICT_LAUNCH
        FGS_LAUNCH_CHECK("k_bwd_tail_verdict");
        hipLaunchKernelGGL(k_bwd_tail_min, dim3((uint32_t)p.d.batch), dim3(256), 0, st, tiles, zero_from);
        FGS_LAUNCH_CHECK("k_bwd_tail_min");
    }
#ifdef FGS_BWD_UNIT_TRACE
    if (g_bwd_trace_slots < ugrid) {
        if (g_bwd_trace) (void)hipFree(g_bwd_trace);
        g_bwd_trace = nullptr; g_bwd_trace_slots = 0;
        if (hipMalloc(&g_bwd_trace, (size_t)ugrid * 24) != hipSuccess) { fgs_set_error("unit trace: hipMalloc"); return FGS_ELAUNCH; }
        g_bwd_trace_slots = ugrid;
    }
    if (hipMemsetAsync(g_bwd_trace, 0, (size_t)ugrid * 24, st) != hipSuccess) { fgs_set_error("unit trace: memset"); return FGS_ELAUNCH; }
    g_bwd_trace_last = ugrid;
#define FGS_BWD_TRACE_ARG , g_bwd_trace
#else
#define FGS_BWD_TRACE_ARG
#endif
#define FGS_BWD_LAUNCH(NSXV)                                                                                              \
    hipLaunchKernelGGL(k_composite_bwd<NSXV>, dim3(ugrid), dim3(64), FGS_BWD_DYN_LDS, st, tiles, tiles_x, W, H, bg0, bg1, bg2, dcap, \
                       counters, seg_off, seg_tile, seg_ckpt, ranges, dup_ids, rec, dup_off, pix, g_rgb, g_depth, grad_rows, t_eps, unit_order, fwd_close, \
                       (uint32_t)p.bwd_zero, (const uint32_t *)zero_from FGS_BWD_TRACE_ARG)
    if (p.tile_w == 32) FGS_BWD_LAUNCH(4); else FGS_BWD_LAUNCH(2);
#undef FGS_BWD_LAUNCH
#undef FGS_BWD_TRACE_ARG
    FGS_LAUNCH_CHECK("k_composite_bwd");
    return FGS_OK;
}
```

### fresnel_amd/csrc/fgs_internal.h

```cpp
#pragma once
#include <hip/hip_runtime.h>
#include <stdint.h>
#include "../../include/fgs.h"

#include "fgs_plan.h"

#define FGS_LAUNCH_CHECK(what)                                              \
    do {                                                                    \
        hipError_t e__ = hipGetLastError();                                 \
        if (e__ != hipSuccess) {                                            \
            fgs_set_error("%s: %s", what, hipGetErrorString(e__));          \
            return FGS_ELAUNCH;                                             \
        }                                                                   \
    } while (0)

enum FgsStage { ST_PROJECT = 0, ST_DEPTH_SORT, ST_DUP_EMIT, ST_TILE_SORT, ST_TILE_RANGES, ST_COMPOSITE_FWD,
                ST_COMPOSITE_BWD, ST_PROJECT_BWD, ST_SPLAT_FWD, ST_FIELD_FWD, ST_FIELD_BWD, ST_SPLAT_BWD };
static_assert(ST_SPLAT_BWD + 1 == FGS_NUM_STAGES, "stage list and FGS_NUM_STAGES disagree");
void fgs_stage_begin(int stage, hipStream_t st);
void fgs_stage_end(int stage, hipStream_t st);

int fgs_launch_project(const FgsPlan &p, const float *cams, const float *pos, const float *scale,
                       const float *quat, const float *color, const float *opacity, char *saved,
                       hipStream_t st, int num_planes = 0, float plane_near = 0.0f, float plane_far = 0.0f,
                       uint32_t *zero_words = nullptr , uint32_t zero_count = 0);
int fgs_launch_project_bwd(const FgsPlan &p, const float *cams, const float *pos, const float *scale,
                           const float *quat, const char *saved, const float *grad_rows, float *g_pos,
                           float *g_scale, float *g_quat, float *g_color, float *g_opacity, float *g_phase,
                           hipStream_t st, float *row_sums = nullptr ,
                           const uint32_t *zero_from = nullptr );

int fgs_launch_asm_project_bwd(const FgsPlan &p, const float *cams, const float *pos, const float *scale,
                               const float *quat, const float *color, const float *phase, int phase_channels,
                               const char *saved, const float *grad_rows, float *g_pos, float *g_scale,
                               float *g_quat, float *g_color, float *g_opacity, float *g_phase, hipStream_t st,
                               bool wave_rows = false);

#define FGS_FOURIER_REC_FLOATS 8
enum { FR_U = 0, FR_V, FR_IS , FR_WR, FR_WG, FR_WB, FR_VIS , FR_OP };
int fgs_launch_fourier_project(int32_t B, int32_t N, int32_t W, int32_t H, int32_t num_cameras, const float *cams,
                               const float *pos, const float *scale, const float *quat, const float *color,
                               const float *opacity, float *frec, hipStream_t st);
int fgs_launch_fourier_project_bwd(int32_t B, int32_t N, int32_t num_cameras, const float *cams, const float *pos,
                                   const float *scale, const float *quat, const float *color, const float *frec,
                                   const float *sums, float *g_pos, float *g_scale, float *g_quat, float *g_color,
                                   float *g_opacity, hipStream_t st);

struct FgsRadixSort {
    uint32_t *keys_in, *vals_in, *keys_alt, *vals_alt;
    uint32_t *vals_final;
    uint32_t seg_len;
    const uint32_t *seg_len_dev;
    uint32_t seg_capacity, seg_stride, num_segs, key_bits;
    uint32_t *hist;
    hipStream_t st;
    const uint32_t *keys_first;
    uint32_t index_payload_mod;
    const uint32_t *key_stats;
    uint32_t key_recs;
    int pass_mode;
    const uint32_t *key_range;
    uint32_t *bucket_tab;
    uint32_t *keys_sorted;
    uint32_t *vals_sorted;
};
int fgs_launch_radix_sort(FgsRadixSort &s);

int fgs_launch_binning(const FgsPlan &p, char *saved, char *scratch, hipStream_t st);

int fgs_fft_work_bytes(int H, int W, int batch, size_t *bytes);
int fgs_fft_exec(int H, int W, int batch, float2 *data, int dir, void *work, hipStream_t st);
int fgs_fft_rows_exec(int W, int rows, float2 *data, int dir, void *work, hipStream_t st);
int fgs_fft_rows_work_bytes(int W, int rows, size_t *bytes);
int fgs_fft2_work_bytes(int H, int W, int batch, size_t *bytes);
int fgs_fft2_exec(int H, int W, int batch, float2 *data, int dir, void *work, hipStream_t st);
int fgs_fft2_inverse_with_max(int H, int W, int images, float2 *data, void *work, float *amax, int slots, float inv_hw,
                              bool *fused, hipStream_t st);
int fgs_launch_composite_fwd(const FgsPlan &p, const float *phase, char *saved, float *out_rgb,
                             float *out_depth, hipStream_t st);
int fgs_launch_composite_bwd(const FgsPlan &p, const float *phase, const char *saved, char *scratch,
                             const float *g_rgb, const float *g_depth, float *g_phase, hipStream_t st);
int fgs_launch_count_pairs(const FgsPlan &p, const char *saved, uint64_t *out, hipStream_t st);

__device__ __forceinline__ uint32_t fgs_lane() { return threadIdx.x & 63u; }

__device__ __forceinline__ uint32_t fgs_xcd_remap(uint32_t bid, uint32_t nwg) {
    const uint32_t q = nwg >> 3, r = nwg & 7u, xcd = bid & 7u, i = bid >> 3;
    return (xcd < r ? xcd * (q + 1u) : r * (q + 1u) + (xcd - r) * q) + i;
}

constexpr float FGS_FOLD_FLOOR_LOG2 = -64.0f;
constexpr float FGS_FOLD_FLOOR = 5.42101086242752217e-20f;
constexpr float FGS_FOLD_MIN_OPACITY = 0.99f * FGS_FOLD_FLOOR;
__host__ __device__ __forceinline__ bool fgs_opacity_floored(float opacity) { return !(opacity >= FGS_FOLD_MIN_OPACITY); }

template <int TW>
__device__ __forceinline__ uint32_t fgs_emission_slot(uint32_t tx, uint32_t ty, uint32_t gid, uint32_t bbx, uint32_t bby,
                                                      const uint32_t *__restrict__ dup_off) {
    const uint32_t tx0 = (bbx & 0xFFFFu) / TW, tx1 = ((bbx >> 16) - 1) / TW, ty0 = (bby & 0xFFFFu) / FGS_TILE;
    return dup_off[gid] + (ty - ty0) * (tx1 - tx0 + 1) + (tx - tx0);
}

__device__ __forceinline__ uint32_t fgs_float_key(float f) {
    f = f + 0.0f;
    uint32_t b = __float_as_uint(f);
    return (b & 0x80000000u) ? ~b : (b | 0x80000000u);
}

__device__ __forceinline__ float fgs_rounded(float x) {
    asm volatile("" : "+v"(x));
    return x;
}

__device__ __forceinline__ float fgs_kz2(float il, float fx, float fy) {
    const float a = fgs_rounded(il * il), b = fgs_rounded(fx * fx), c = fgs_rounded(fy * fy);
    return fgs_rounded(fgs_rounded(a - b) - c);
}

__device__ __forceinline__ float fgs_asm_intensity(float2 u, float inv_hw) {
    const float ur = fgs_rounded(u.x * inv_hw), ui = fgs_rounded(u.y * inv_hw);
    return fgs_rounded(fgs_rounded(ur * ur) + fgs_rounded(ui * ui));
}
__device__ __forceinline__ float fgs_asm_amplitude(float intensity) { return sqrtf(fgs_rounded(intensity + 1e-8f)); }
```

### fresnel_amd/csrc/fgs_plan.cpp

```cpp
#include <string.h>
#include "fgs_plan.h"

uint32_t fgs_radix_blocks_per_seg(uint32_t seg_capacity, uint32_t num_segs) {
    uint32_t bps = (seg_capacity + 1023) / 1024;
    uint32_t cap = 1024;
    if (num_segs > 1) cap = 64;
    if (bps > cap) bps = cap;
    if (bps < 1) bps = 1;
    return bps;
}

size_t fgs_radix_hist_bytes(uint32_t seg_capacity, uint32_t num_segs) {
    const size_t bps = fgs_radix_blocks_per_seg(seg_capacity, num_segs);
    size_t words = (size_t)num_segs * 256 * bps + (size_t)num_segs * 256;
    const size_t handoff = (size_t)FGS_SORT_HANDOFF_PASSES * num_segs * 16 * 256;
    if (handoff > words) words = handoff;
    return words * sizeof(uint32_t);
}

static size_t align256(size_t x) { return (x + 255) & ~(size_t)255; }

int fgs_make_plan(const FgsDims *d, FgsPlan *p, int layers, bool segment_ckpt) {
    if (!d || !p) { fgs_set_error("null dims"); return FGS_EINVAL; }
    if (d->batch < 1 || d->batch > 65535  || d->num_gaussians < 1 || d->width < 1 || d->height < 1 || d->width > 32768 ||
        d->height > 32768 || !(d->max_radius > 0.0f) || !(d->max_radius <= 65536.0f)  || (d->num_cameras != 1 && d->num_cameras != d->batch)) {
        fgs_set_error("invalid dims: B=%d N=%d W=%d H=%d max_radius=%g num_cameras=%d", d->batch,
                      d->num_gaussians, d->width, d->height, (double)d->max_radius, d->num_cameras);
        return FGS_EINVAL;
    }
    const int exit_flags = d->fwd_variant >= 0 ? (d->fwd_variant & (FGS_FWD_EXIT_OFF | FGS_FWD_EXIT_ON)) : 0;
    const int zero_flags = d->fwd_variant >= 0 ? (d->fwd_variant & (FGS_BWD_ZERO_OFF | FGS_BWD_ZERO_ON)) : 0;
    const int tail_flags = d->fwd_variant >= 0 ? (d->fwd_variant & (FGS_BWD_TAIL_OFF | FGS_BWD_TAIL_ON)) : 0;
    const int fv = d->fwd_variant - exit_flags - zero_flags - tail_flags, afv = fv < -16 || fv > 16 ? 3  : (fv < 0 ? -fv : fv);
    if (d->seg_len < 0 || d->seg_len > 512 || d->seg_len % 64 != 0 || (afv != 0 && afv != 1 && afv != 2 && afv != 4 && !(fv == 8 || fv == 16)) ||
        d->bin_mode < 0 || d->bin_mode > 2 || (d->tile_w != 0 && d->tile_w != 16 && d->tile_w != 32) || d->sort_mode < 0 || d->sort_mode > 11 ||
        exit_flags == (FGS_FWD_EXIT_OFF | FGS_FWD_EXIT_ON) || zero_flags == (FGS_BWD_ZERO_OFF | FGS_BWD_ZERO_ON) ||
        tail_flags == (FGS_BWD_TAIL_OFF | FGS_BWD_TAIL_ON)) {
        fgs_set_error("invalid tuning: seg_len=%d fwd_variant=%d bin_mode=%d tile_w=%d sort_mode=%d", d->seg_len, d->fwd_variant,
                      d->bin_mode, d->tile_w, d->sort_mode);
        return FGS_EINVAL;
    }
    const size_t B = d->batch, N = d->num_gaussians;
    if (B * N >= (1ull << 31)) { fgs_set_error("B*N too large"); return FGS_EINVAL; }
    memset(p, 0, sizeof(*p));
    p->d = *d;
    p->layers = layers;
    const bool wide_ok = !d->use_phase && !d->saturation_skip && fv >= 0 && layers == 1 && segment_ckpt;
    if (d->tile_w == 32 && !wide_ok) {
        fgs_set_error("tile_w=32 needs the blend path with the depth-split forward");
        return FGS_EINVAL;
    }
    const size_t tiles16 = B * (size_t)((d->width + 15) / 16) * (size_t)((d->height + 15) / 16);
    p->tile_w = d->tile_w ? d->tile_w : ((wide_ok && d->width >= 512 && tiles16 >= 3072) ? 32 : 16);
    const int tx = (d->width + p->tile_w - 1) / p->tile_w, ty = (d->height + FGS_TILE - 1) / FGS_TILE;
    p->tiles = tx * ty;
    int span = (int)((2.0 * (double)d->max_radius + 1.0) / p->tile_w) + 2;
    if (span > tx) span = tx;
    int spany = (int)((2.0 * (double)d->max_radius + 1.0) / FGS_TILE) + 2;
    if (spany > ty) spany = ty;
    p->tiles_per_gauss = span * spany;
    const size_t worst = B * N * (size_t)p->tiles_per_gauss;
    if (worst >= (1ull << 32) - 256) { fgs_set_error("duplicate capacity exceeds 2^32"); return FGS_EINVAL; }
    p->capacity_hinted = d->dup_capacity != 0 && (size_t)d->dup_capacity < worst;
    const size_t dcap = p->capacity_hinted ? (size_t)d->dup_capacity : worst;
    uint32_t bits = 0;
    while ((1ull << bits) < B * (size_t)layers * p->tiles) ++bits;
    p->tile_key_bits = bits;

    FgsSavedLayout &L = p->L;
    size_t o = 0;
    L.rec = o; o = align256(o + B * N * FGS_REC_FLOATS * 4);
    L.depth_key = o; o = align256(o + B * N * 4);
    L.tile_count = o; o = align256(o + B * N * 4);
    L.order = o; o = align256(o + B * N * 4);
    L.dup_off = o; o = align256(o + B * N * 4);
    L.counters = o; o = align256(o + 16 * 4);
    L.ranges = o; o = align256(o + B * layers * p->tiles * 2 * 4);
    L.tile_order = o; o = align256(o + B * layers * p->tiles * 4);
    L.dup_ids = o; o = align256(o + dcap * 4);
    L.pix_state = o; o = align256(o + B * 6 * (size_t)d->width * d->height * 4);
    L.phase_ckpt = o;
    if (d->use_phase) o = align256(o + (dcap / FGS_PHASE_CKPT + B * p->tiles + 2) * 8 * 64 * 4);
    p->s_layer = o;
    if (layers > 1) o = align256(o + B * N * 4);
    p->s_keybits = o; o = align256(o + B * ((N + 255) / 256) * (4 + 1) * 4);
    const uint32_t grid_tiles = (uint32_t)(B * p->tiles);
    if (afv > 4 && (d->use_phase || d->saturation_skip || layers != 1 || !segment_ckpt)) {
        fgs_set_error("fwd_variant=%d: 8 / 16 list parts exist on the blend path's depth-split forward only", fv);
        return FGS_EINVAL;
    }
    if (d->use_phase) {
        if (afv != 0 && afv != 4) {
            fgs_set_error("fwd_variant=%d: the phase path has one work split (one wave per 8 x 8 sub-tile)", fv);
            return FGS_EINVAL;
        }
        p->fwd_parts = 0;
        p->fwd_waves = 4;
        p->fwd_variant = -4;
    } else if (d->saturation_skip || fv < 0) {
        p->fwd_parts = 0;
        p->fwd_waves = fv < 0 ? afv : (grid_tiles >= 24576u ? 1 : (grid_tiles <= 6144u ? 4 : 2));
        p->fwd_variant = -p->fwd_waves;
    } else {
        p->fwd_parts = fv > 0 ? fv : (grid_tiles >= 24576u ? 1 : (p->tile_w != 16 ? 4 : (grid_tiles <= 1024u ? 16 : (grid_tiles <= 2048u ? 8 : 4))));
        if (p->tile_w == 32 && p->fwd_parts > 8) p->fwd_parts = 8;
        p->fwd_waves = p->fwd_parts;
        p->fwd_variant = p->fwd_parts;
    }
    const bool row_split = !d->use_phase && p->fwd_parts == 0;
    if (row_split && d->seg_len != 0 && d->seg_len != FGS_SEG) {
        fgs_set_error("seg_len=%d is not available with the row-split forward (saturation_skip / fwd_variant < 0)", d->seg_len);
        return FGS_EINVAL;
    }
#ifndef FGS_SEG64_MAX_GAUSSIANS
#define FGS_SEG64_MAX_GAUSSIANS 200000
#endif
    L.seg_len = d->seg_len ? d->seg_len : ((B * N <= FGS_SEG64_MAX_GAUSSIANS && !row_split) ? 64 : FGS_SEG);
    p->direct_binning = p->tiles <= FGS_BIN_MAX_TILES && tx + ty <= FGS_MASK_MAX_LINES && d->bin_mode != 2;
    if (d->bin_mode == 1 && !p->direct_binning) {
        fgs_set_error("bin_mode=1 (direct binning) needs <= %d tiles and <= %d tile columns + rows per image",
                      FGS_BIN_MAX_TILES, FGS_MASK_MAX_LINES);
        return FGS_EINVAL;
    }
    L.tile_w = p->tile_w;
#ifndef FGS_ORDER_GROUPS
#define FGS_ORDER_GROUPS 8
#endif
    p->order_groups = (p->fwd_parts > 0 && layers == 1 && segment_ckpt) ? FGS_ORDER_GROUPS : 1;
#ifdef FGS_SPLAT_ORDER_GROUPS
    if (!segment_ckpt && B * (size_t)layers * p->tiles >= 24576) p->order_groups = FGS_ORDER_GROUPS;
#endif
    p->depth_ordered = segment_ckpt;
    const size_t ucap = dcap / L.seg_len + B * layers * p->tiles;
    L.seg_off = o; L.seg_tile = o; L.seg_ckpt = o; L.seg_capacity = 0;
    if (!d->use_phase) {
        L.seg_capacity = ucap;
        L.seg_off = o; o = align256(o + (B * layers * p->tiles + 1) * 4);
        L.seg_tile = o; o = align256(o + ucap * 4);
        L.seg_ckpt = o;
        if (segment_ckpt && layers == 1) o = align256(o + ucap * 5 * 64 * (size_t)(p->tile_w / 4) * 4);
    }
    L.unit_order = o;
    p->has_unit_order = !d->use_phase && segment_ckpt && layers == 1;
    if (p->has_unit_order) o = align256(o + ucap * 4);
    L.fwd_open = o;
    const bool exit_ok = p->fwd_parts > 0 && layers == 1 && segment_ckpt;
    p->fwd_exit = exit_ok && (exit_flags == FGS_FWD_EXIT_ON || (exit_flags == 0 && B * p->tiles * (size_t)(p->tile_w / 16) >= 8192));
    p->bwd_zero = zero_flags == FGS_BWD_ZERO_ON || (zero_flags == 0 && B * p->tiles * (size_t)(p->tile_w / 16) >= 8192);
    p->s_fwd_max = o;
    if (p->fwd_exit) {
        p->s_fwd_max = o = align256(o + B * p->tiles * 2 * 4);
        o = align256(o + B * ((N + 255) / 256) * 2 * 4);
    }
    L.fwd_close = o;
    if (p->fwd_exit) o = align256(o + B * p->tiles * 2 * 4);
    p->bwd_tail = p->fwd_exit && p->bwd_zero && p->direct_binning && p->has_unit_order && tail_flags != FGS_BWD_TAIL_OFF;
    L.rank_of = o;
    if (p->bwd_tail) o = align256(o + B * N * 4);
    L.total_bytes = o;
    if (!p->bwd_tail) L.rank_of = o;
    L.dup_capacity = dcap;
    L.tiles_x = tx; L.tiles_y = ty;

    size_t nsort = dcap > B * N ? dcap : B * N;
    const size_t bin_words = B * (size_t)layers * p->tiles;
    if (bin_words > nsort) nsort = bin_words;
    const size_t mask_words = p->direct_binning ? B * (size_t)(tx + ty) * fgs_mask_words((uint32_t)N) * 2 : 0;
    if (mask_words > nsort) nsort = mask_words;
    p->tile_table_words = ((bin_words + FGS_TILE_TABLE_TILES - 1) / FGS_TILE_TABLE_TILES) * (2 + 64 * (size_t)p->order_groups);
    if (p->tile_table_words > nsort) nsort = p->tile_table_words;
    p->sort_words = nsort;
    const size_t nblk = B * ((N + FGS_BIN_G - 1) / FGS_BIN_G) + (B * N + 255) / 256 + 1;
    size_t hist = fgs_radix_hist_bytes((uint32_t)N, (uint32_t)B);
    const size_t hist2 = fgs_radix_hist_bytes((uint32_t)dcap, 1);
    if (hist2 > hist) hist = hist2;
    o = 0;
    p->s_keys0 = o; o = align256(o + nsort * 4);
    p->s_keys1 = o; o = align256(o + nsort * 4);
    p->s_vals0 = o; o = align256(o + nsort * 4);
    p->s_vals1 = o; o = align256(o + nsort * 4);
    p->s_hist = o; o = align256(o + hist);
    p->s_bsum = o; o = align256(o + nblk * 4);
    p->s_grows = o; o = align256(o + dcap * 4 * (d->use_phase ? 4 * FGS_GROW_FLOATS
                                                             : (FGS_BLEND_ROW_FLOATS > FGS_GROW_FLOATS ? FGS_BLEND_ROW_FLOATS : FGS_GROW_FLOATS)));
    p->s_plane = o; o = align256(o + B * ((size_t)layers + 1) * 4);
    p->s_rsum = o; o = align256(o + B * N * 12 * 4);
    p->s_bucket = o; o = align256(o + B * FGS_SORT_BUCKET_WORDS * 4);
    p->s_zero_from = o;
    if (p->bwd_tail) o = align256(o + (B * (size_t)p->tiles + B) * 4);
    p->s_total = o;
    if (!p->bwd_tail) p->s_zero_from = o;
    return FGS_OK;
}
```

### fresnel_amd/csrc/fgs_plan.h

```cpp
#pragma once
#include <stddef.h>
#include <stdint.h>
#include "../../include/fgs.h"

#define FGS_REC_FLOATS 12
#define FGS_WAVE 64

enum { G_U = 0, G_V, G_CA, G_CBC, G_CD, G_OP, G_CR, G_CG, G_CB, G_DEPTH, G_PHASE, G_PAD1 };
#define FGS_GROW_FLOATS 12
#ifndef FGS_BLEND_ROW_FLOATS
#define FGS_BLEND_ROW_FLOATS 10
#endif
#define FGS_BIN_G 256
#define FGS_TILE_TABLE_TILES 1024
enum { R_U = 0, R_V, R_CA, R_CBC, R_CD, R_OP, R_CR, R_CG, R_CB, R_DEPTH, R_BBX, R_BBY };

struct FgsPlan {
    FgsDims d;
    FgsSavedLayout L;
    int32_t layers;
    size_t s_layer;
    size_t s_keybits;
    int32_t tile_w;
    int32_t tiles;
    int32_t tiles_per_gauss;
    bool capacity_hinted;
    uint32_t tile_key_bits;
    int32_t fwd_parts;
    int32_t fwd_waves;
    int32_t fwd_variant;
    bool direct_binning;
    bool depth_ordered;
    int32_t order_groups;
    bool has_unit_order;
    bool fwd_exit;
    bool bwd_zero;
    bool bwd_tail;
    size_t s_fwd_max;
    size_t sort_words;
    size_t tile_table_words;
    size_t s_total;
    size_t s_keys0, s_keys1;
    size_t s_vals0, s_vals1;
    size_t s_hist;
    size_t s_bsum;
    size_t s_grows;
    size_t s_plane;
    size_t s_rsum;
    size_t s_bucket;
    size_t s_zero_from;
};

int fgs_make_plan(const FgsDims *dims, FgsPlan *plan, int layers = 1, bool segment_ckpt = true);
void fgs_set_error(const char *fmt, ...);

#define FGS_BIN_MAX_TILES 4096
#define FGS_MASK_MAX_LINES 512
static inline uint32_t fgs_mask_words(uint32_t n) { return (((n + 63u) / 64u) + 7u) & ~7u; }
#define FGS_SORT_HANDOFF_PASSES 4
#define FGS_SORT_BUCKET_WORDS 260
size_t fgs_radix_hist_bytes(uint32_t seg_capacity, uint32_t num_segs);
uint32_t fgs_radix_blocks_per_seg(uint32_t seg_capacity, uint32_t num_segs);
```

### fresnel_amd/csrc/fgs_project.hip

```cpp
#include "fgs_internal.h"

#pragma clang fp contract(off)

namespace {

__device__ __forceinline__ float clamp_min(float x, float lo) { return x < lo ? lo : x; }
__device__ __forceinline__ float clamp_max(float x, float hi) { return x > hi ? hi : x; }
__device__ __forceinline__ float sgnf(float x) { return (float)((x > 0.0f) - (x < 0.0f)); }

struct Proj {
    float xc, yc, zc, dep;
    float w, x, y, z, nrm;
    float Rc[3][3];
    float M[3][3];
    float S[3][3];
    float zs, z2, J00, J02, J11, J12;
    float T0[3], T1[3];
    float a, b, c, d, u, v;
};

__device__ __forceinline__ void project_one(const float *__restrict__ V, float fx, float fy, float cx,
                                            float cy, const float p[3], const float s[3],
                                            const float q[4], Proj &o) {
    o.xc = ((V[0] * p[0] + V[1] * p[1]) + V[2] * p[2]) + V[3];
// ... 43 lines not shown
    o.b = o.T0[1] * o.J11 + o.T0[2] * o.J12;
    o.c = o.T1[0] * o.J00 + o.T1[2] * o.J02;
    o.d = o.T1[1] * o.J11 + o.T1[2] * o.J12;
    o.u = __fdiv_rn(fx * o.xc, -o.zs) + cx;
    o.v = __fdiv_rn(fy * (-o.yc), -o.zs) + cy;
}

__global__ __launch_bounds__(256) void k_project(
    int32_t N, int32_t W, int32_t H, int32_t num_cameras, float max_radius,
    const float *__restrict__ cams, const float *__restrict__ pos, const float *__restrict__ scale,
    const float *__restrict__ quat, const float *__restrict__ color, const float *__restrict__ opacity,
    float *__restrict__ rec, uint32_t *__restrict__ depth_key, uint32_t *__restrict__ tile_count,
    uint32_t *__restrict__ layer, int32_t num_planes, float plane_near, float plane_far, int32_t tile_w,
    uint32_t *__restrict__ key_bits, uint32_t *__restrict__ zero_words, uint32_t zero_count, uint32_t *__restrict__ fwd_max) {
    for (uint32_t i = (blockIdx.y * gridDim.x + blockIdx.x) * 256u + threadIdx.x; i < zero_count; i += gridDim.x * gridDim.y * 256u)
        zero_words[i] = 0u;
    const int32_t n = blockIdx.x * 256 + threadIdx.x, b = blockIdx.y;
    uint32_t key = 0xFFFFFFFFu;
    uint32_t cmax = 0u, dmax = 0u;
    if (n < N) {
        const int32_t idx = b * N + n;
        const float *__restrict__ cam = cams + (num_cameras > 1 ? b : 0) * FGS_CAMERA_FLOATS;
        const float p[3] = {pos[3 * idx], pos[3 * idx + 1], pos[3 * idx + 2]};
        const float s[3] = {scale[3 * idx], scale[3 * idx + 1], scale[3 * idx + 2]};
        const float4 q4 = reinterpret_cast<const float4 *>(quat)[idx];
        const float q[4] = {q4.x, q4.y, q4.z, q4.w};
        const float fx = cam[16], fy = cam[17], cx = cam[18], cy = cam[19], nearp = cam[20], farp = cam[21];
        Proj o;
        project_one(cam, fx, fy, cx, cy, p, s, q, o);

        const float tr = o.a + o.d;
        float det = o.a * o.d - o.b * o.c;
        det = clamp_min(det, 1e-6f);
        const float disc = clamp_min(tr * tr - 4.0f * det, 0.0f);
        const float lam = __fdiv_rn(tr + __fsqrt_rn(disc), 2.0f);
        float r = 3.0f * __fsqrt_rn(clamp_min(lam, 1e-6f));
        r = clamp_max(r, max_radius);
        const bool vis = (o.dep > nearp) && (o.dep < farp) && (o.u + r > 0.0f) && (o.u - r < (float)W) &&
                         (o.v + r > 0.0f) && (o.v - r < (float)H);
        int32_t x0 = 0, x1 = 0, y0 = 0, y1 = 0;
        if (vis) {
            const double ud = (double)o.u, vd = (double)o.v, rd = (double)r;
            double e;
            e = trunc(ud - rd); x0 = e < 0.0 ? 0 : (e > (double)W ? W : (int32_t)e);
            e = trunc(ud + rd) + 1.0; x1 = e > (double)W ? W : (e < 0.0 ? 0 : (int32_t)e);
            e = trunc(vd - rd); y0 = e < 0.0 ? 0 : (e > (double)H ? H : (int32_t)e);
            e = trunc(vd + rd) + 1.0; y1 = e > (double)H ? H : (e < 0.0 ? 0 : (int32_t)e);
        }
        uint32_t ntiles = 0;
        if (vis && x0 < x1 && y0 < y1)
            ntiles = (uint32_t)(((x1 - 1) / tile_w - x0 / tile_w + 1) * ((y1 - 1) / FGS_TILE - y0 / FGS_TILE + 1));
        const float ar = o.a + 1e-4f, dr = o.d + 1e-4f;
        const float detr = ar * dr - o.b * o.c;
        const float ia = __fdiv_rn(dr, detr);
        const float ibc = __fdiv_rn(-o.b, detr) + __fdiv_rn(-o.c, detr);
        const float id = __fdiv_rn(ar, detr);

        float4 *out = reinterpret_cast<float4 *>(rec + (size_t)idx * FGS_REC_FLOATS);
        out[0] = make_float4(o.u, o.v, ia, ibc);
        out[1] = make_float4(id, opacity[idx], color[3 * idx], color[3 * idx + 1]);
        out[2] = make_float4(color[3 * idx + 2], o.dep, __uint_as_float((uint32_t)x0 | ((uint32_t)x1 << 16)),
                             __uint_as_float((uint32_t)y0 | ((uint32_t)y1 << 16)));
        key = vis ? fgs_float_key(o.dep) : 0xFFFFFFFFu;
        depth_key[idx] = key;
        tile_count[idx] = ntiles;
        if (fwd_max && ntiles) {
            const float m = 0.99f;
            cmax = max(max(__float_as_uint(color[3 * idx] * m) & 0x7FFFFFFFu, __float_as_uint(color[3 * idx + 1] * m) & 0x7FFFFFFFu),
                       __float_as_uint(color[3 * idx + 2] * m) & 0x7FFFFFFFu);
            dmax = __float_as_uint(o.dep * m) & 0x7FFFFFFFu;
        }
        if (layer) {
            const float step = (plane_far - plane_near) / (float)(num_planes - 1);
            int32_t best = 0;
            float bd = 3.4e38f;
            for (int32_t k = 0; k < num_planes; ++k) {
                const float pk = (k < num_planes / 2) ? plane_near + step * (float)k
                                                      : plane_far - step * (float)(num_planes - 1 - k);
                const float dd = fabsf(o.dep - pk);
                if (dd < bd) { bd = dd; best = k; }
            }
            layer[idx] = (uint32_t)best;
        }
    }
    {
        const bool visk = key != 0xFFFFFFFFu;
        uint32_t vor = visk ? key : 0u, vand = key;
        uint32_t vmin = key, vmax = vor;
#pragma unroll
        for (int o2 = 32; o2 > 0; o2 >>= 1) {
            vor |= __shfl_xor(vor, o2, 64); vand &= __shfl_xor(vand, o2, 64);
            vmin = min(vmin, (uint32_t)__shfl_xor(vmin, o2, 64)); vmax = max(vmax, (uint32_t)__shfl_xor(vmax, o2, 64));
        }
        const uint32_t fl = (__ballot(visk) != 0ull ? 2u : 0u) | (__ballot(n < N && !visk) != 0ull ? 1u : 0u);
        __shared__ uint32_t wv[4][5];
        const uint32_t wave = threadIdx.x >> 6;
        if ((threadIdx.x & 63u) == 0) { wv[wave][0] = vor; wv[wave][1] = vand; wv[wave][2] = fl; wv[wave][3] = vmin; wv[wave][4] = vmax; }
        __syncthreads();
        if (threadIdx.x == 0) {
            uint32_t *o3 = key_bits + ((size_t)b * gridDim.x + blockIdx.x) * 4;
            o3[0] = (wv[0][0] | wv[1][0]) | (wv[2][0] | wv[3][0]);
            o3[1] = (wv[0][1] & wv[1][1]) & (wv[2][1] & wv[3][1]);
            o3[2] = (wv[0][2] | wv[1][2]) | (wv[2][2] | wv[3][2]);
            o3[3] = min(min(wv[0][3], wv[1][3]), min(wv[2][3], wv[3][3]));
            key_bits[(size_t)gridDim.y * gridDim.x * 4 + (size_t)b * gridDim.x + blockIdx.x] =
                max(max(wv[0][4], wv[1][4]), max(wv[2][4], wv[3][4]));
        }
    }
    if (fwd_max) {
#pragma unroll
        for (int o2 = 32; o2 > 0; o2 >>= 1) {
            cmax = max(cmax, (uint32_t)__shfl_xor(cmax, o2, 64)); dmax = max(dmax, (uint32_t)__shfl_xor(dmax, o2, 64));
        }
        __shared__ uint32_t wm[4][2];
        if ((threadIdx.x & 63u) == 0) { wm[threadIdx.x >> 6][0] = cmax; wm[threadIdx.x >> 6][1] = dmax; }
        __syncthreads();
        if (threadIdx.x == 0) {
            uint32_t *o4 = fwd_max + ((size_t)b * gridDim.x + blockIdx.x) * 2;
            o4[0] = max(max(wm[0][0], wm[1][0]), max(wm[2][0], wm[3][0]));
            o4[1] = max(max(wm[0][1], wm[1][1]), max(wm[2][1], wm[3][1]));
        }
    }
}

__global__ __launch_bounds__(256) void k_fourier_project(
    int32_t N, int32_t W, int32_t H, int32_t num_cameras, const float *__restrict__ cams, const float *__restrict__ pos,
    const float *__restrict__ scale, const float *__restrict__ quat, const float *__restrict__ color,
    const float *__restrict__ opacity, float *__restrict__ frec) {
    const int32_t n = blockIdx.x * 256 + threadIdx.x, b = blockIdx.y;
    if (n >= N) return;
    const int32_t idx = b * N + n;
    const float *__restrict__ cam = cams + (num_cameras > 1 ? b : 0) * FGS_CAMERA_FLOATS;
    const float p[3] = {pos[3 * idx], pos[3 * idx + 1], pos[3 * idx + 2]};
    const float s[3] = {scale[3 * idx], scale[3 * idx + 1], scale[3 * idx + 2]};
    const float4 q4 = reinterpret_cast<const float4 *>(quat)[idx];
    const float q[4] = {q4.x, q4.y, q4.z, q4.w};
    Proj o;
    project_one(cam, cam[16], cam[17], cam[18], cam[19], p, s, q, o);
    const bool vis = (o.dep > cam[20]) && (o.dep < cam[21]) && (o.u > -(float)W) && (o.u < (float)(2 * W)) &&
                     (o.v > -(float)H) && (o.v < (float)(2 * H));
    const float op = opacity[idx];
    float4 r0 = make_float4(0.0f, 0.0f, 0.0f, 0.0f), r1 = make_float4(0.0f, 0.0f, 0.0f, op);
    if (vis) {
        const float sigma = __fsqrt_rn(__fdiv_rn(o.a + o.d, 2.0f) + 1e-8f);
        const float den = 2.0f * (sigma * sigma) + 1e-8f;
        r0 = make_float4(o.u, o.v, __fdiv_rn(1.0f, den), color[3 * idx] * op);
        r1 = make_float4(color[3 * idx + 1] * op, color[3 * idx + 2] * op, __uint_as_float(1u), op);
    }
    float4 *out = reinterpret_cast<float4 *>(frec + (size_t)idx * FGS_FOURIER_REC_FLOATS);
    out[0] = r0;
    out[1] = r1;
}

__global__ __launch_bounds__(256) __attribute__((amdgpu_waves_per_eu(8, 8))) void k_row_sum(int32_t total, int32_t N, uint32_t dcap,
                                                 const uint32_t *__restrict__ order,
                                                 const uint32_t *__restrict__ dup_off,
                                                 const uint32_t *__restrict__ tile_count,
                                                 const float *__restrict__ grad_rows, const float *__restrict__ rec,
                                                 float *__restrict__ sums, const uint32_t *__restrict__ zero_from,
                                                 const uint32_t *__restrict__ zero_min, uint32_t tiles, uint32_t tiles_x,
                                                 uint32_t tile_w) {
    const int32_t tid = blockIdx.x * 256 + threadIdx.x;
    const int32_t ri = tid >> 2;
    const uint32_t sub = threadIdx.x & 3u;
    const bool live = ri < total;
    float acc[10] = {0, 0, 0, 0, 0, 0, 0, 0, 0, 0};
    int32_t idx = 0;
    if (live) {
        idx = ri / N * N + (int32_t)order[ri];
        const uint32_t off = dup_off[idx];
        uint32_t cnt = tile_count[idx];
        if (off >= dcap) cnt = 0; else if (cnt > dcap - off) cnt = dcap - off;
        double m[6] = {0, 0, 0, 0, 0, 0};
        const float *base = grad_rows + (size_t)off * FGS_BLEND_ROW_FLOATS;
        uint32_t k = sub;
        const uint32_t rank = (uint32_t)(ri - ri / N * N);
        const uint32_t *zf = nullptr;
        uint32_t t0 = 0u, rw = 1u;
        float inv_rw = 1.0f;
        if (zero_from && cnt != 0u && rank >= zero_min[ri / N]) {
            const uint32_t bbx = __float_as_uint(rec[(size_t)idx * FGS_REC_FLOATS + R_BBX]), bby = __float_as_uint(rec[(size_t)idx * FGS_REC_FLOATS + R_BBY]);
            const uint32_t tx0 = (bbx & 0xFFFFu) / tile_w;
            t0 = (bby & 0xFFFFu) / FGS_TILE * tiles_x + tx0;
            rw = max(((bbx >> 16) - 1u) / tile_w - tx0 + 1u, 1u);
            inv_rw = 1.0f / (float)rw;
            zf = zero_from + (size_t)(ri / N) * tiles;
        }
        auto written = [&](uint32_t row) -> bool {
            if (!zf) return true;
            const uint32_t ky = (uint32_t)(((float)row + 0.5f) * inv_rw), t = t0 + ky * tiles_x + (row - ky * rw);
            return t >= tiles || rank < zf[t];
        };
#if FGS_BLEND_ROW_FLOATS == 16
        auto add_row = [&](const float4 a, const float4 b, const float4 c) {
            m[0] += a.x; m[1] += a.y; m[2] += a.z; m[3] += a.w; m[4] += b.x; m[5] += b.y;
            acc[6] += b.z; acc[7] += b.w; acc[8] += c.x; acc[9] += c.y;
        };
        for (; k + 4 < cnt; k += 8) {
            const float4 *r = reinterpret_cast<const float4 *>(base + (size_t)k * 16);
            const float4 *r2 = reinterpret_cast<const float4 *>(base + (size_t)(k + 4) * 16);
            const bool w1 = written(k), w2 = written(k + 4);
            if (w1 && w2) {
                const float4 a = r[0], b = r[1], c = r[2], a2 = r2[0], b2 = r2[1], c2 = r2[2];
                add_row(a, b, c); add_row(a2, b2, c2);
            } else if (w1) {
                add_row(r[0], r[1], r[2]);
            } else if (w2) {
                add_row(r2[0], r2[1], r2[2]);
            }
        }
        if (k < cnt && written(k)) {
            const float4 *r = reinterpret_cast<const float4 *>(base + (size_t)k * 16);
            add_row(r[0], r[1], r[2]);
        }
#else
        auto add_row = [&](const float2 a, const float2 bq, const float2 cq, const float2 dq, const float2 eq) {
            m[0] += a.x; m[1] += a.y; m[2] += bq.x; m[3] += bq.y; m[4] += cq.x; m[5] += cq.y;
            acc[6] += dq.x; acc[7] += dq.y; acc[8] += eq.x; acc[9] += eq.y;
        };
        for (; k + 4 < cnt; k += 8) {
            const float2 *r = reinterpret_cast<const float2 *>(base + (size_t)k * FGS_BLEND_ROW_FLOATS);
            const float2 *r2 = reinterpret_cast<const float2 *>(base + (size_t)(k + 4) * FGS_BLEND_ROW_FLOATS);
            const bool w1 = written(k), w2 = written(k + 4);
            if (w1 && w2) {
                const float2 a = r[0], bq = r[1], cq = r[2], dq = r[3], eq = r[4];
                const float2 a2 = r2[0], bq2 = r2[1], cq2 = r2[2], dq2 = r2[3], eq2 = r2[4];
                add_row(a, bq, cq, dq, eq);
                add_row(a2, bq2, cq2, dq2, eq2);
            } else if (w1) {
                add_row(r[0], r[1], r[2], r[3], r[4]);
            } else if (w2) {
                add_row(r2[0], r2[1], r2[2], r2[3], r2[4]);
            }
        }
        if (k < cnt && written(k)) {
            const float2 *r = reinterpret_cast<const float2 *>(base + (size_t)k * FGS_BLEND_ROW_FLOATS);
            add_row(r[0], r[1], r[2], r[3], r[4]);
        }
#endif
        const float opacity = rec[(size_t)idx * FGS_REC_FLOATS + R_OP];
        const bool floored = fgs_opacity_floored(opacity);
        const double unfloor = 1.0 / ((double)0.99f * (double)FGS_FOLD_FLOOR);
        const double hp = 0.69314718055994530942 * (floored ? (double)opacity * unfloor : 1.0);
        acc[0] = (float)(hp * m[0]); acc[1] = (float)(hp * m[1]);
        acc[2] = (float)(-0.72134752044448170368 * hp * m[2]); acc[3] = (float)(-0.72134752044448170368 * hp * m[3]);
        acc[4] = (float)(-0.72134752044448170368 * hp * m[4]);
        acc[5] = (float)(m[5] * (floored ? unfloor : 1.0 / (double)opacity));
        if (floored) {
            const float back = (float)((double)opacity * unfloor);
            acc[6] *= back; acc[7] *= back; acc[8] *= back; acc[9] *= back;
        }
        acc[6] *= 0.99f; acc[7] *= 0.99f; acc[8] *= 0.99f; acc[9] *= 0.99f;
    }
#pragma unroll
    for (int k = 0; k < 10; ++k) {
        acc[k] += __shfl_xor(acc[k], 1, 64);
        acc[k] += __shfl_xor(acc[k], 2, 64);
    }
    if (!live || sub != 0) return;
    float4 *o = reinterpret_cast<float4 *>(sums + (size_t)idx * 12);
    o[0] = make_float4(acc[0], acc[1], acc[2], acc[3]);
    o[1] = make_float4(acc[4], acc[5], acc[6], acc[7]);
    o[2] = make_float4(acc[8], acc[9], 0.0f, 0.0f);
}

template <int MODE, bool PRESUM = false>
__global__ __launch_bounds__(256) void k_project_bwd(
    int32_t total, int32_t N, int32_t num_cameras, uint32_t dcap, const float *__restrict__ cams,
    const float *__restrict__ pos, const float *__restrict__ scale, const float *__restrict__ quat,
    const uint32_t *__restrict__ depth_key, const uint32_t *__restrict__ order,
    const uint32_t *__restrict__ dup_off, const uint32_t *__restrict__ tile_count,
    const float *__restrict__ grad_rows, float *__restrict__ g_pos, float *__restrict__ g_scale,
    float *__restrict__ g_quat, float *__restrict__ g_color, float *__restrict__ g_opacity,
    float *__restrict__ g_phase, const float *__restrict__ color, const float *__restrict__ phase,
    int32_t phase_channels, uint32_t rows_per_dup, const float *__restrict__ rec) {
    const int32_t tid = blockIdx.x * 256 + threadIdx.x;
    const int32_t ri = PRESUM ? tid : tid >> 2;
    const uint32_t sub = PRESUM ? 0u : threadIdx.x & 3u;
    const bool live = ri < total;
    const int32_t b = live ? ri / N : 0;
    const int32_t idx = live ? (PRESUM ? ri : b * N + (int32_t)order[ri]) : 0;
    float gp[3] = {0, 0, 0}, gs[3] = {0, 0, 0}, gq[4] = {0, 0, 0, 0};
    constexpr bool ASM = MODE == 1 || MODE == 2;
    constexpr int ROWF = MODE == 2 ? 16 : FGS_GROW_FLOATS;
    float acc[13] = {0, 0, 0, 0, 0, 0, 0, 0, 0, 0, 0, 0, 0};
    if constexpr (PRESUM) {
        if (live) {
            const float4 *r = reinterpret_cast<const float4 *>(grad_rows + (size_t)idx * 12);
            const float4 a = r[0], bq = r[1], cq = r[2];
            acc[0] = a.x; acc[1] = a.y; acc[2] = a.z; acc[3] = a.w; acc[4] = bq.x; acc[5] = bq.y; acc[6] = bq.z;
            acc[7] = bq.w; acc[8] = cq.x; acc[9] = cq.y;
        }
    } else if (live) {
        const uint32_t cnt = tile_count[idx] * rows_per_dup, off = dup_off[idx] * rows_per_dup;
        if (MODE == 0) {
            const uint32_t bbx = __float_as_uint(rec[(size_t)idx * FGS_REC_FLOATS + R_BBX]);
            const uint32_t bby = __float_as_uint(rec[(size_t)idx * FGS_REC_FLOATS + R_BBY]);
            const uint32_t x0 = bbx & 0xFFFFu, x1 = bbx >> 16, y0 = bby & 0xFFFFu, y1 = bby >> 16;
            const uint32_t tx0 = x0 / FGS_TILE, ty0 = y0 / FGS_TILE, tw = (x1 - 1) / FGS_TILE - tx0 + 1;
            uint32_t tx = 0, ty = 0;
            for (uint32_t k = sub; k < cnt && off + k < dcap * rows_per_dup; k += 4) {
                const uint32_t sx = (tx0 + tx) * FGS_TILE + 8u * (sub & 1u), sy = (ty0 + ty) * FGS_TILE + 8u * (sub >> 1);
                if (++tx == tw) { tx = 0; ++ty; }
                if (x1 <= sx || x0 >= sx + 8u || y1 <= sy || y0 >= sy + 8u) continue;
                const float4 *r = reinterpret_cast<const float4 *>(grad_rows + (size_t)(off + k) * ROWF);
                const float4 a = r[0], bq = r[1], cq = r[2];
                acc[0] += a.x; acc[1] += a.y; acc[2] += a.z; acc[3] += a.w;
                acc[4] += bq.x; acc[5] += bq.y; acc[6] += bq.z; acc[7] += bq.w;
                acc[8] += cq.x; acc[9] += cq.y; acc[10] += cq.z; acc[11] += cq.w;
            }
            acc[0] *= 0.69314718055994530942f; acc[1] *= 0.69314718055994530942f;
            acc[2] *= -0.5f; acc[3] *= -0.5f; acc[4] *= -0.5f;
        } else {
            const uint32_t room = dcap * rows_per_dup, lim = off >= room ? 0u : min(cnt, room - off);
            auto add_row = [&](const float4 &a, const float4 &bq, const float4 &cq, float extra) {
                if (MODE == 2) acc[12] += extra;
                acc[0] += a.x; acc[1] += a.y; acc[2] += a.z; acc[3] += a.w;
                acc[4] += bq.x; acc[5] += bq.y; acc[6] += bq.z; acc[7] += bq.w;
                acc[8] += cq.x; acc[9] += cq.y; acc[10] += cq.z; acc[11] += cq.w;
            };
            uint32_t k = sub;
            for (; k + 4 < lim; k += 8) {
                const float4 *r = reinterpret_cast<const float4 *>(grad_rows + (size_t)(off + k) * ROWF);
                const float4 *r2 = reinterpret_cast<const float4 *>(grad_rows + (size_t)(off + k + 4) * ROWF);
                const float4 a = r[0], bq = r[1], cq = r[2], a2 = r2[0], bq2 = r2[1], cq2 = r2[2];
                const float e = MODE == 2 ? r[3].x : 0.0f, e2 = MODE == 2 ? r2[3].x : 0.0f;
                add_row(a, bq, cq, e);
                add_row(a2, bq2, cq2, e2);
            }
            if (k < lim) {
                const float4 *r = reinterpret_cast<const float4 *>(grad_rows + (size_t)(off + k) * ROWF);
                const float4 a = r[0], bq = r[1], cq = r[2];
                add_row(a, bq, cq, MODE == 2 ? r[3].x : 0.0f);
            }
        }
    }
    if constexpr (!PRESUM) {
#pragma unroll
        for (int k = 0; k < 13; ++k) {
            acc[k] += __shfl_xor(acc[k], 1, 64);
            acc[k] += __shfl_xor(acc[k], 2, 64);
        }
    }
    if (!live || sub != 0) return;
    const float4 s0 = make_float4(acc[0], acc[1], acc[2], acc[3]);
    const float4 s1 = make_float4(acc[4], acc[5], acc[6], acc[7]);
    const float4 s2 = make_float4(acc[8], acc[9], acc[10], acc[11]);
    const float g_mean[2] = {s0.x, s0.y};
    const float op_asm = ASM ? rec[(size_t)idx * FGS_REC_FLOATS + R_OP] : 0.0f;
    const float kcon = ASM ? -0.5f * op_asm : 1.0f;
    const float g_conic[3] = {kcon * s0.z, kcon * s0.w, kcon * s1.x};
    float g_depth = s2.y;
    if constexpr (MODE == 3) {
        g_depth = 0.0f;
        const float op = rec[(size_t)idx * FGS_FOURIER_REC_FLOATS + FR_OP];
        const float dw[3] = {s0.w, s1.x, s1.y};
        g_opacity[idx] = (dw[0] * color[3 * idx] + dw[1] * color[3 * idx + 1]) + dw[2] * color[3 * idx + 2];
        g_color[3 * idx] = dw[0] * op; g_color[3 * idx + 1] = dw[1] * op; g_color[3 * idx + 2] = dw[2] * op;
    } else {
    g_opacity[idx] = s1.y;
    if (!ASM) {
        if (g_phase) g_phase[idx] = s2.z;
        g_color[3 * idx] = s1.z; g_color[3 * idx + 1] = s1.w; g_color[3 * idx + 2] = s2.x;
    } else {
        g_depth = MODE == 2 ? acc[12] : 0.0f;
        const float dcc[3] = {s1.z, s1.w, s2.x}, dcs[3] = {s2.y, s2.z, acc[11]};
        float gph = 0.0f;
#pragma unroll
        for (int ch = 0; ch < 3; ++ch) {
            const float ph = phase_channels == 3 ? phase[3 * idx + ch] : phase[idx];
            float sn, cs;
            sincosf(ph, &sn, &cs);
// ... 23 lines not shown
        const double yc = V[1][0] * p[0] + V[1][1] * p[1] + V[1][2] * p[2] + V[1][3];
        const double zc = V[2][0] * p[0] + V[2][1] * p[1] + V[2][2] * p[2] + V[2][3];
        const double nrm = sqrt(q0[0] * q0[0] + q0[1] * q0[1] + q0[2] * q0[2] + q0[3] * q0[3]);
        const double inn = 1.0 / (nrm < 1e-12 ? 1e-12 : nrm);
        const double w = q0[0] * inn, x = q0[1] * inn, y = q0[2] * inn, z = q0[3] * inn;
        const double R[3][3] = {{1 - 2 * y * y - 2 * z * z, 2 * x * y - 2 * w * z, 2 * x * z + 2 * w * y},
                                {2 * x * y + 2 * w * z, 1 - 2 * x * x - 2 * z * z, 2 * y * z - 2 * w * x},
                                {2 * x * z - 2 * w * y, 2 * y * z + 2 * w * x, 1 - 2 * x * x - 2 * y * y}};
        double Rc[3][3], M[3][3], S[3][3];
#pragma unroll
        for (int i = 0; i < 3; ++i)
#pragma unroll
            for (int j = 0; j < 3; ++j) {
                Rc[i][j] = V[i][0] * R[0][j] + V[i][1] * R[1][j] + V[i][2] * R[2][j];
                M[i][j] = Rc[i][j] * s[j];
            }
#pragma unroll
        for (int i = 0; i < 3; ++i)
#pragma unroll
            for (int j = 0; j < 3; ++j) S[i][j] = M[i][0] * M[j][0] + M[i][1] * M[j][1] + M[i][2] * M[j][2];
        const double az = fabs(zc);
        const double sg = (double)sgnf((float)zc + 1e-8f);
        const double zs = (az < 0.01 ? 0.01 : az) * sg;
        const double izs = 1.0 / zs, iz2 = izs * izs, iz3 = iz2 * izs;
        const double J[2][3] = {{-fx * izs, 0.0, fx * xc * iz2}, {0.0, fy * izs, fy * yc * iz2}};
        double T[2][3], C2[2][2];
#pragma unroll
        for (int i = 0; i < 2; ++i)
#pragma unroll
            for (int j = 0; j < 3; ++j) T[i][j] = J[i][0] * S[0][j] + J[i][1] * S[1][j] + J[i][2] * S[2][j];
#pragma unroll
        for (int i = 0; i < 2; ++i)
#pragma unroll
            for (int j = 0; j < 2; ++j) C2[i][j] = T[i][0] * J[j][0] + T[i][1] * J[j][1] + T[i][2] * J[j][2];
        const double ar = C2[0][0] + (double)1e-4f, dr = C2[1][1] + (double)1e-4f, cb = C2[0][1], cc = C2[1][0];
        const double rdet = 1.0 / (ar * dr - cb * cc);
        const double Y[2][2] = {{dr * rdet, -cb * rdet}, {-cc * rdet, ar * rdet}};
        const double GY[2][2] = {{g_conic[0], g_conic[1]}, {g_conic[1], g_conic[2]}};
        double tmp[2][2], G2[2][2];
        if constexpr (MODE == 3) {
            G2[0][0] = G2[1][1] = (double)s0.z; G2[0][1] = G2[1][0] = 0.0;
        } else {
#pragma unroll
        for (int i = 0; i < 2; ++i)
#pragma unroll
            for (int j = 0; j < 2; ++j) tmp[i][j] = Y[0][i] * GY[0][j] + Y[1][i] * GY[1][j];
#pragma unroll
        for (int i = 0; i < 2; ++i)
#pragma unroll
            for (int j = 0; j < 2; ++j) G2[i][j] = -(tmp[i][0] * Y[j][0] + tmp[i][1] * Y[j][1]);
        }
        double GS[3][3];
#pragma unroll
        for (int i = 0; i < 3; ++i)
#pragma unroll
            for (int j = 0; j < 3; ++j) {
                double acc = 0.0;
#pragma unroll
                for (int a2 = 0; a2 < 2; ++a2)
#pragma unroll
                    for (int b2 = 0; b2 < 2; ++b2) acc += J[a2][i] * G2[a2][b2] * J[b2][j];
                GS[i][j] = acc;
            }
        double JS[2][3], JSt[2][3];
#pragma unroll
        for (int i = 0; i < 2; ++i)
#pragma unroll
            for (int j = 0; j < 3; ++j) {
                JS[i][j] = J[i][0] * S[0][j] + J[i][1] * S[1][j] + J[i][2] * S[2][j];
                JSt[i][j] = J[i][0] * S[j][0] + J[i][1] * S[j][1] + J[i][2] * S[j][2];
            }
        double GJ[2][3];
#pragma unroll
        for (int i = 0; i < 2; ++i)
#pragma unroll
            for (int j = 0; j < 3; ++j)
                GJ[i][j] = (G2[i][0] * JSt[0][j] + G2[i][1] * JSt[1][j]) + (G2[0][i] * JS[0][j] + G2[1][i] * JS[1][j]);
        double gu = g_mean[0], gv = g_mean[1];
        if (ASM) {
            const double h = 0.5 * (double)op_asm, cbc = Y[0][1] + Y[1][0];
            gu = h * (2.0 * Y[0][0] * (double)g_mean[0] + cbc * (double)g_mean[1]);
            gv = h * (cbc * (double)g_mean[0] + 2.0 * Y[1][1] * (double)g_mean[1]);
        } else if (MODE == 0 && phase_channels) {
            const double kc = 0.72134752044448170368, cbc = Y[0][1] + Y[1][0];
            gu = kc * (2.0 * Y[0][0] * (double)g_mean[0] + cbc * (double)g_mean[1]);
            gv = kc * (cbc * (double)g_mean[0] + 2.0 * Y[1][1] * (double)g_mean[1]);
        }
        const double gxc = GJ[0][2] * fx * iz2 + gu * (-fx * izs);
        const double gyc = GJ[1][2] * fy * iz2 + gv * (fy * izs);
        const double gzs = GJ[0][0] * fx * iz2 + GJ[0][2] * (-2.0 * fx * xc * iz3) + GJ[1][1] * (-fy * iz2) +
                           GJ[1][2] * (-2.0 * fy * yc * iz3) + gu * (fx * xc * iz2) + gv * (-fy * yc * iz2);
        const double dzs = (az >= 0.01 ? (double)sgnf((float)zc) : 0.0) * sg;
        const double gpc[3] = {gxc, gyc, gzs * dzs - (double)g_depth};
#pragma unroll
        for (int j = 0; j < 3; ++j) gp[j] = (float)(V[0][j] * gpc[0] + V[1][j] * gpc[1] + V[2][j] * gpc[2]);
        double GRc[3][3];
#pragma unroll
        for (int j = 0; j < 3; ++j) {
            double acc = 0.0;
#pragma unroll
            for (int i = 0; i < 3; ++i) {
                double gm = 0.0;
#pragma unroll
                for (int k = 0; k < 3; ++k) gm += (GS[i][k] + GS[k][i]) * M[k][j];
                acc += gm * Rc[i][j];
                GRc[i][j] = gm * s[j];
            }
            gs[j] = (float)acc;
        }
        double GR[3][3];
#pragma unroll
        for (int i = 0; i < 3; ++i)
#pragma unroll
            for (int j = 0; j < 3; ++j) GR[i][j] = V[0][i] * GRc[0][j] + V[1][i] * GRc[1][j] + V[2][i] * GRc[2][j];
        double gh[4];
        gh[0] = -2 * z * GR[0][1] + 2 * y * GR[0][2] + 2 * z * GR[1][0] - 2 * x * GR[1][2] - 2 * y * GR[2][0] + 2 * x * GR[2][1];
        gh[1] = 2 * y * GR[0][1] + 2 * z * GR[0][2] + 2 * y * GR[1][0] - 4 * x * GR[1][1] - 2 * w * GR[1][2] + 2 * z * GR[2][0] + 2 * w * GR[2][1] - 4 * x * GR[2][2];
        gh[2] = -4 * y * GR[0][0] + 2 * x * GR[0][1] + 2 * w * GR[0][2] + 2 * x * GR[1][0] + 2 * z * GR[1][2] - 2 * w * GR[2][0] + 2 * z * GR[2][1] - 4 * y * GR[2][2];
        gh[3] = -4 * z * GR[0][0] - 2 * w * GR[0][1] + 2 * x * GR[0][2] + 2 * w * GR[1][0] - 4 * z * GR[1][1] + 2 * y * GR[1][2] + 2 * x * GR[2][0] + 2 * y * GR[2][1];
        const double qh[4] = {w, x, y, z};
        if (nrm >= 1e-12) {
            const double dot = qh[0] * gh[0] + qh[1] * gh[1] + qh[2] * gh[2] + qh[3] * gh[3];
#pragma unroll
            for (int i = 0; i < 4; ++i) gq[i] = (float)((gh[i] - qh[i] * dot) * inn);
        } else {
#pragma unroll
            for (int i = 0; i < 4; ++i) gq[i] = (float)(gh[i] * 1e12);
        }
    }
    g_pos[3 * idx] = gp[0]; g_pos[3 * idx + 1] = gp[1]; g_pos[3 * idx + 2] = gp[2];
    g_scale[3 * idx] = gs[0]; g_scale[3 * idx + 1] = gs[1]; g_scale[3 * idx + 2] = gs[2];
    reinterpret_cast<float4 *>(g_quat)[idx] = make_float4(gq[0], gq[1], gq[2], gq[3]);
}

}

int fgs_launch_project(const FgsPlan &p, const float *cams, const float *pos, const float *scale,
                       const float *quat, const float *color, const float *opacity, char *saved,
                       hipStream_t st, int num_planes, float plane_near, float plane_far, uint32_t *zero_words,
                       uint32_t zero_count) {
    const dim3 grid((unsigned)((p.d.num_gaussians + 255) / 256), (unsigned)p.d.batch);
    hipLaunchKernelGGL(k_project, grid, dim3(256), 0, st, p.d.num_gaussians, p.d.width,
                       p.d.height, p.d.num_cameras, p.d.max_radius, cams, pos, scale, quat, color, opacity,
                       reinterpret_cast<float *>(saved + p.L.rec),
                       reinterpret_cast<uint32_t *>(saved + p.L.depth_key),
                       reinterpret_cast<uint32_t *>(saved + p.L.tile_count),
                       num_planes > 1 ? reinterpret_cast<uint32_t *>(saved + p.s_layer) : nullptr, num_planes,
                       plane_near, plane_far, p.tile_w, reinterpret_cast<uint32_t *>(saved + p.s_keybits), zero_words,
                       zero_words ? zero_count : 0u, p.fwd_exit ? reinterpret_cast<uint32_t *>(saved + p.s_fwd_max) : nullptr);
    FGS_LAUNCH_CHECK("k_project");
    return FGS_OK;
}

int fgs_launch_project_bwd(const FgsPlan &p, const float *cams, const float *pos, const float *scale,
                           const float *quat, const char *saved, const float *grad_rows, float *g_pos,
                           float *g_scale, float *g_quat, float *g_color, float *g_opacity, float *g_phase,
                           hipStream_t st, float *row_sums, const uint32_t *zero_from) {
    const int32_t total = p.d.batch * p.d.num_gaussians;
    const int grid = (int)(((size_t)total * 4 + 255) / 256);
    const uint32_t *depth_key = reinterpret_cast<const uint32_t *>(saved + p.L.depth_key);
    const uint32_t *order = reinterpret_cast<const uint32_t *>(saved + p.L.order);
    const uint32_t *dup_off = reinterpret_cast<const uint32_t *>(saved + p.L.dup_off);
    const uint32_t *tile_count = reinterpret_cast<const uint32_t *>(saved + p.L.tile_count);
    const float *rec = reinterpret_cast<const float *>(saved + p.L.rec);
    if (!p.d.use_phase) {
        if (!row_sums) { fgs_set_error("fgs_launch_project_bwd: the blend path needs the row-sum scratch"); return FGS_EINVAL; }
        hipLaunchKernelGGL(k_row_sum, dim3(grid), dim3(256), 0, st, total, p.d.num_gaussians,
                           (uint32_t)p.L.dup_capacity, order, dup_off, tile_count, grad_rows, rec, row_sums,
                           p.bwd_tail ? zero_from : nullptr, p.bwd_tail && zero_from ? zero_from + (size_t)p.d.batch * p.tiles : nullptr,
                           (uint32_t)p.tiles, (uint32_t)p.L.tiles_x, (uint32_t)p.tile_w);
        FGS_LAUNCH_CHECK("k_row_sum");
        hipLaunchKernelGGL((k_project_bwd<0, true>), dim3((total + 255) / 256), dim3(256), 0, st, total,
                           p.d.num_gaussians, p.d.num_cameras, (uint32_t)p.L.dup_capacity, cams, pos, scale, quat,
                           depth_key, order, dup_off, tile_count, row_sums, g_pos, g_scale, g_quat, g_color, g_opacity,
                           g_phase, nullptr, nullptr, 1, 1u, rec);
        FGS_LAUNCH_CHECK("k_project_bwd");
        return FGS_OK;
    }
    hipLaunchKernelGGL(k_project_bwd<0>, dim3(grid), dim3(256), 0, st, total, p.d.num_gaussians,
                       p.d.num_cameras, (uint32_t)p.L.dup_capacity, cams, pos, scale, quat, depth_key, order, dup_off,
                       tile_count, grad_rows, g_pos, g_scale, g_quat, g_color, g_opacity, g_phase, nullptr, nullptr,
                       1, 4u, rec);
    FGS_LAUNCH_CHECK("k_project_bwd");
    return FGS_OK;
}

int fgs_launch_asm_project_bwd(const FgsPlan &p, const float *cams, const float *pos, const float *scale,
                               const float *quat, const float *color, const float *phase, int phase_channels,
                               const char *saved, const float *grad_rows, float *g_pos, float *g_scale,
                               float *g_quat, float *g_color, float *g_opacity, float *g_phase, hipStream_t st,
                               bool wave_rows) {
    const int32_t total = p.d.batch * p.d.num_gaussians;
    const int grid = (int)(((size_t)total * 4 + 255) / 256);
    if (wave_rows) {
        hipLaunchKernelGGL(k_project_bwd<2>, dim3(grid), dim3(256), 0, st, total, p.d.num_gaussians,
                           p.d.num_cameras, (uint32_t)p.L.dup_capacity, cams, pos, scale, quat,
                           reinterpret_cast<const uint32_t *>(saved + p.L.depth_key),
                           reinterpret_cast<const uint32_t *>(saved + p.L.order),
                           reinterpret_cast<const uint32_t *>(saved + p.L.dup_off),
                           reinterpret_cast<const uint32_t *>(saved + p.L.tile_count), grad_rows, g_pos, g_scale,
                           g_quat, g_color, g_opacity, g_phase, color, phase, phase_channels, 1u,
                           reinterpret_cast<const float *>(saved + p.L.rec));
        FGS_LAUNCH_CHECK("k_wave_project_bwd");
        return FGS_OK;
    }
    hipLaunchKernelGGL(k_project_bwd<1>, dim3(grid), dim3(256), 0, st, total, p.d.num_gaussians,
                       p.d.num_cameras, (uint32_t)p.L.dup_capacity, cams, pos, scale, quat,
                       reinterpret_cast<const uint32_t *>(saved + p.L.depth_key),
                       reinterpret_cast<const uint32_t *>(saved + p.L.order),
                       reinterpret_cast<const uint32_t *>(saved + p.L.dup_off),
                       reinterpret_cast<const uint32_t *>(saved + p.L.tile_count), grad_rows, g_pos, g_scale,
                       g_quat, g_color, g_opacity, g_phase, color, phase, phase_channels, 1u,
                       reinterpret_cast<const float *>(saved + p.L.rec));
    FGS_LAUNCH_CHECK("k_asm_project_bwd");
    return FGS_OK;
}

int fgs_launch_fourier_project(int32_t B, int32_t N, int32_t W, int32_t H, int32_t num_cameras, const float *cams,
                               const float *pos, const float *scale, const float *quat, const float *color,
                               const float *opacity, float *frec, hipStream_t st) {
    hipLaunchKernelGGL(k_fourier_project, dim3((unsigned)((N + 255) / 256), (unsigned)B), dim3(256), 0, st, N, W, H,
                       num_cameras, cams, pos, scale, quat, color, opacity, frec);
    FGS_LAUNCH_CHECK("k_fourier_project");
    return FGS_OK;
}

int fgs_launch_fourier_project_bwd(int32_t B, int32_t N, int32_t num_cameras, const float *cams, const float *pos,
                                   const float *scale, const float *quat, const float *color, const float *frec,
                                   const float *sums, float *g_pos, float *g_scale, float *g_quat, float *g_color,
                                   float *g_opacity, hipStream_t st) {
    const int32_t total = B * N;
    hipLaunchKernelGGL((k_project_bwd<3, true>), dim3((unsigned)((total + 255) / 256)), dim3(256), 0, st, total, N,
                       num_cameras, 0u, cams, pos, scale, quat, nullptr, nullptr, nullptr, nullptr, sums, g_pos, g_scale,
                       g_quat, g_color, g_opacity, nullptr, color, nullptr, 0, 1u, frec);
    FGS_LAUNCH_CHECK("k_fourier_project_bwd");
    return FGS_OK;
}
```

### include/fgs.h

```cpp
#ifndef FGS_H
#define FGS_H

#include <stddef.h>
#include <stdint.h>

#ifdef __cplusplus
extern "C" {
#endif

#define FGS_OK 0
#define FGS_EINVAL (-1)
#define FGS_ELAUNCH (-2)
#define FGS_EUNSUPPORTED (-3)

#define FGS_TILE 16
#define FGS_SEG 128
#define FGS_FWD_EXIT_OFF 0x100
#define FGS_FWD_EXIT_ON 0x200
#define FGS_BWD_ZERO_OFF 0x400
#define FGS_BWD_ZERO_ON 0x800
#define FGS_BWD_TAIL_OFF 0x2000
#define FGS_BWD_TAIL_ON 0x4000
#define FGS_TUNE_AUTO 0
#ifndef FGS_PHASE_CKPT
#define FGS_PHASE_CKPT 8
#endif
#define FGS_CAMERA_FLOATS 24

typedef struct FgsDims {
    int32_t batch;
    int32_t num_gaussians;
    int32_t width, height;
    float max_radius;
    float background[3];
    int32_t use_phase;
    float phase_amplitude;
    int32_t num_cameras;
    int32_t saturation_skip;
    int32_t seg_len;
    int32_t fwd_variant;
    int32_t bin_mode;
    int32_t tile_w;
    int32_t sort_mode;
    uint32_t dup_capacity;
} FgsDims;


typedef struct FgsSavedLayout {
    size_t total_bytes;
    size_t rec;
    size_t depth_key;
    size_t tile_count;
    size_t order;
    size_t dup_off;
    size_t counters;
    size_t ranges;
    size_t tile_order;
    size_t dup_ids;
    size_t pix_state;
    size_t phase_ckpt;
    size_t dup_capacity;
    int32_t tiles_x, tiles_y;
    size_t seg_off;
    size_t seg_tile;
    size_t seg_ckpt;
    size_t seg_capacity;
    int32_t seg_len;
    int32_t tile_w;
    size_t unit_order;
    size_t fwd_open;
    size_t fwd_close;
    size_t rank_of;
} FgsSavedLayout;

int fgs_workspace_bytes(const FgsDims *dims, size_t *saved_bytes, size_t *scratch_bytes);
int fgs_saved_layout(const FgsDims *dims, FgsSavedLayout *layout);

int fgs_forward(const FgsDims *dims, const float *cameras, const float *pos, const float *scale,
                const float *quat, const float *color, const float *opacity, const float *phase,
                float *out_rgb, float *out_depth, void *saved, void *scratch, void *stream);

int fgs_backward(const FgsDims *dims, const float *cameras, const float *pos, const float *scale,
                 const float *quat, const float *color, const float *opacity, const float *phase,
                 const void *saved, void *scratch, const float *g_rgb, const float *g_depth,
                 float *g_pos, float *g_scale, float *g_quat, float *g_color, float *g_opacity,
                 float *g_phase, void *stream);

int fgs_count_pairs(const FgsDims *dims, const void *saved, uint64_t *out_pairs, void *stream);

typedef struct FgsAsmDims {
    int32_t batch, num_gaussians, width, height;
    float max_radius;
    float background[3];
    int32_t num_planes;
    float depth_near, depth_far;
    float focal_depth;
    double pixel_pitch;
    int32_t phase_channels;
    int32_t num_cameras;
    int32_t bin_mode;
} FgsAsmDims;

int fgs_asm_workspace_bytes(const FgsAsmDims *dims, size_t *saved_bytes, size_t *scratch_bytes);
int fgs_asm_forward(const FgsAsmDims *dims, const float *cameras, const float *pos, const float *scale,
                    const float *quat, const float *color, const float *opacity, const float *phase,
                    const float *wavelengths, float *out_rgb, void *saved, void *scratch, void *stream);
int fgs_asm_backward(const FgsAsmDims *dims, const float *cameras, const float *pos, const float *scale,
                     const float *quat, const float *color, const float *opacity, const float *phase,
                     const float *wavelengths, void *saved, void *scratch, const float *g_rgb,
                     float *g_pos, float *g_scale, float *g_quat, float *g_color, float *g_opacity,
                     float *g_phase, float *g_wavelengths, void *stream);

typedef struct FgsWaveDims {
    int32_t batch, num_gaussians, width, height;
    float max_radius;
    float background[3];
    int32_t phase_channels;
    int32_t num_cameras;
} FgsWaveDims;

int fgs_wave_workspace_bytes(const FgsWaveDims *dims, size_t *saved_bytes, size_t *scratch_bytes);
int fgs_wave_forward(const FgsWaveDims *dims, const float *cameras, const float *pos, const float *scale,
                     const float *quat, const float *color, const float *opacity, const float *phase,
                     float *out_rgb, float *out_depth, void *saved, void *scratch, void *stream);
int fgs_wave_backward(const FgsWaveDims *dims, const float *cameras, const float *pos, const float *scale,
                      const float *quat, const float *color, const float *opacity, const float *phase,
                      void *saved, void *scratch, const float *g_rgb, const float *g_depth, float *g_pos,
                      float *g_scale, float *g_quat, float *g_color, float *g_opacity, float *g_phase,
                      void *stream);

typedef struct FgsFourierDims {
    int32_t batch, num_gaussians, width, height;
    float background[3];
    int32_t num_cameras;
} FgsFourierDims;

int fgs_fourier_workspace_bytes(const FgsFourierDims *dims, size_t *saved_bytes, size_t *scratch_bytes);
int fgs_fourier_forward(const FgsFourierDims *dims, const float *cameras, const float *pos, const float *scale,
                        const float *quat, const float *color, const float *opacity, float *out_rgb, void *saved,
                        void *scratch, void *stream);
int fgs_fourier_backward(const FgsFourierDims *dims, const float *cameras, const float *pos, const float *scale,
                         const float *quat, const float *color, const float *opacity, const void *saved, void *scratch,
                         const float *g_rgb, float *g_pos, float *g_scale, float *g_quat, float *g_color,
                         float *g_opacity, void *stream);

int fgs_asm_propagate_workspace_bytes(int32_t height, int32_t width, int32_t channels, size_t *scratch_bytes);
int fgs_asm_propagate_forward(int32_t height, int32_t width, int32_t channels, double pixel_pitch, int32_t band_limit,
                              const float *field, const float *z, const float *wavelengths, float *out,
                              float *spectrum, void *scratch, void *stream);
int fgs_asm_propagate_backward(int32_t height, int32_t width, int32_t channels, double pixel_pitch, int32_t band_limit,
                               const float *spectrum, const float *z, const float *wavelengths, const float *g_out,
                               float *g_field, float *g_z, float *g_wavelengths, void *scratch, void *stream);

typedef struct FgsSpectralDims {
    int32_t images, channels, height, width;
    int32_t mode;
    float cutoff, high_weight;
    float focal_depth;
    int32_t reserved;
} FgsSpectralDims;
int fgs_spectral_workspace_bytes(const FgsSpectralDims *dims, size_t *saved_bytes, size_t *scratch_bytes);
int fgs_spectral_loss_forward(const FgsSpectralDims *dims, const float *rendered, const float *target,
                              const float *depth, const float *wavelength, float *loss, void *saved, void *scratch,
                              void *stream);
int fgs_spectral_loss_backward(const FgsSpectralDims *dims, const float *rendered, const float *target,
                               const float *depth, const float *wavelength, void *saved, void *scratch,
                               const float *g_loss, float *g_rendered, float *g_target, float *g_depth,
                               float *g_wavelength, void *stream);
int fgs_helmholtz_loss_forward(int32_t images, int32_t height, int32_t width, float wavelength, float pixel_spacing,
                               const float *field, float *loss, float *residual, void *scratch, void *stream);
int fgs_helmholtz_loss_backward(int32_t images, int32_t height, int32_t width, float wavelength, float pixel_spacing,
                                const float *residual, const float *g_loss, float *g_field, void *stream);
size_t fgs_reduction_scratch_bytes(void);

#define FGS_SSIM_MAX_TAPS 15
#define FGS_SSIM_GRAD_X 1
#define FGS_SSIM_GRAD_Y 2
#define FGS_SSIM_NONNEGATIVE 4
#define FGS_SSIM_PER_IMAGE 8
typedef struct FgsSsimDims {
    int32_t images, channels, height, width;
    float taps[FGS_SSIM_MAX_TAPS];
    int32_t num_taps;
    float c1, c2;
    int32_t flags;
} FgsSsimDims;
int fgs_ssim_workspace_bytes(const FgsSsimDims *dims, size_t *saved_bytes, size_t *scratch_bytes);
int fgs_ssim_forward(const FgsSsimDims *dims, const float *x, const float *y, float *out, void *saved, void *scratch,
                     void *stream);
int fgs_ssim_backward(const FgsSsimDims *dims, const float *x, const float *y, const void *saved, const float *g_out,
                      float *g_x, float *g_y, void *scratch, void *stream);

#define FGS_PIXEL_MAX_BOUNDARIES 65
#define FGS_PIXEL_RGB 1
#define FGS_PIXEL_DENSITY 2
#define FGS_PIXEL_BOUNDARY 4
#define FGS_PIXEL_HARD_MASK 8
#define FGS_PIXEL_DEPTH 16
#define FGS_PIXEL_STAT_RGB 0
#define FGS_PIXEL_STAT_BOUNDARY 1
#define FGS_PIXEL_STAT_DEPTH 2
#define FGS_PIXEL_STAT_SUM_X 3
#define FGS_PIXEL_STAT_SUM_Y 4
#define FGS_PIXEL_STAT_SSD_X 5
#define FGS_PIXEL_STAT_SSD_Y 6
#define FGS_PIXEL_STAT_SGN 7
#define FGS_PIXEL_STAT_SGN_U 8
#define FGS_PIXEL_STAT_SLOTS 16
typedef struct FgsPixelLossDims {
    int32_t images, height, width;
    int32_t flags;
    int32_t world;
    float vlm_weight;
    float threshold;
    int32_t num_boundaries;
    float boundaries[FGS_PIXEL_MAX_BOUNDARIES];
} FgsPixelLossDims;
int fgs_pixel_loss_workspace_bytes(const FgsPixelLossDims *dims, size_t *stats_bytes, size_t *scratch_bytes);
int fgs_pixel_loss_stage1(const FgsPixelLossDims *dims, const float *rendered, const float *target,
                          const float *rendered_depth, const float *target_depth, const float *density, float *out,
                          void *stats, void *scratch, void *stream);
int fgs_pixel_loss_stage2(const FgsPixelLossDims *dims, const float *rendered_depth, const float *target_depth,
                          void *stats, void *scratch, void *stream);
int fgs_pixel_loss_stage3(const FgsPixelLossDims *dims, const float *rendered_depth, const float *target_depth, float *out,
                          void *stats, void *scratch, void *stream);
int fgs_pixel_loss_forward(const FgsPixelLossDims *dims, const float *rendered, const float *target,
                           const float *rendered_depth, const float *target_depth, const float *density, float *out,
                           void *stats, void *scratch, void *stream);
int fgs_pixel_loss_backward(const FgsPixelLossDims *dims, const float *rendered, const float *target,
                            const float *rendered_depth, const float *target_depth, const float *density,
                            const void *stats, const float *g_rgb, const float *g_boundary, const float *g_depth,
                            float *g_rendered, float *g_rendered_depth, void *stream);

typedef struct FgsHeadDims {
    int32_t batch, points, k_full, k_used;
    int32_t channels;
    float xy_gain;
    float edge_scale_factor, edge_opacity_boost;
} FgsHeadDims;
int fgs_head_workspace_bytes(const FgsHeadDims *dims, size_t *scratch_bytes);
int fgs_head_forward(const FgsHeadDims *dims, const float *raw, const float *base_xy, const float *base_z, const float *pose,
// ... 157 lines not shown
```

### scratch/profile/bwd_zero_units.py

```python
import ctypes
import os
import sys

import numpy as np
import torch

sys.path.insert(0, os.path.dirname(os.path.dirname(os.path.dirname(os.path.abspath(__file__)))))
import bench

bench._import_compute()
from fresnel_amd import _binding as B
from fresnel_amd import renderer as R

workload = sys.argv[1] if len(sys.argv) > 1 else "config3"
distribution = sys.argv[2] if len(sys.argv) > 2 else "saag"
tuning = sys.argv[3] if len(sys.argv) > 3 else ""
dev = torch.device("cuda:0")
N, S, Bn = bench.WORKLOADS[workload]
pos, scale, quat, col, opa = bench.synth_batch(Bn, N, 1000 * int(workload[-1]), dev, distribution)
leaves = [t.requires_grad_(True) for t in (pos, scale, quat, col, opa)]
cam = R.Camera(0.8 * S, 0.8 * S, S / 2, S / 2, S, S)
ren = R.TileBasedRenderer(S, S).to(dev)
ren.tuning = dict(bwd_zero=1, **({k: int(v) for k, v in (kv.split("=") for kv in tuning.split(","))} if tuning else {}))
g = torch.Generator().manual_seed(4242)
gI = torch.randn(Bn, 3, S, S, generator=g).to(dev)
gD = (torch.randn(Bn, S, S, generator=g) * 0.1).to(dev)

lib = B.load()
if not hasattr(lib, "fgs_bwd_unit_trace"):
    sys.exit("the library has no fgs_bwd_unit_trace: build it with --define FGS_BWD_UNIT_TRACE=1")
lib.fgs_bwd_unit_trace.restype = ctypes.c_long
lib.fgs_bwd_unit_trace.argtypes = [ctypes.c_void_p, ctypes.c_size_t]

for step in range(2):
    for t in leaves:
        t.grad = None
    img, dep = ren(*leaves, cam, return_depth=True)
    node = img.grad_fn
    st = R.inspect_saved(node.saved_tensors[-1], node.dims)
    torch.autograd.backward([img, dep], [gI, gD])
torch.cuda.synchronize()
cap = int(st["layout"].seg_capacity)
seg_len = int(st["layout"].seg_len)
buf = np.zeros((cap, 3), np.uint64)
n = lib.fgs_bwd_unit_trace(buf.ctypes.data, cap)
assert n > 0, n
U = int(st["counters"][2])
rec = buf[:U]
assert (rec[:, 2] >> np.uint64(63)).all(), "a launch slot below U left no record"
unit = (rec[:, 2] & np.uint64(0xFFFFFFFF)).astype(np.int64)
walk = ((rec[:, 2] >> np.uint64(32)) & np.uint64(7)).astype(np.int64)
assert np.array_equal(np.sort(unit), np.arange(U)), "the launch did not run every unit exactly once"
rg = st["ranges"].cpu().numpy().astype(np.int64).reshape(-1, 2)
lens = rg[:, 1] - rg[:, 0]
seg_off = st["seg_off"].cpu().numpy().astype(np.int64)
seg_tile = st["seg_tile"][:U].cpu().numpy().astype(np.int64)
ulen = np.minimum(seg_len, lens[seg_tile[unit]] - (unit - seg_off[seg_tile[unit]]) * seg_len)
E = int(ulen.sum())
print(f"{workload} {distribution} {tuning or '-'}: tile_w {int(st['layout'].tile_w)}, seg_len {seg_len}, U = {U} units, {E} list entries")
for code, name in ((0, "general walk"), (3, "(a) zero units: S == +-0 on every lane of every sub-tile"),
                   (4, "(b) dead, some but not all sub-tiles all-zero"), (1, "(c) dead, no sub-tile all-zero")):
    m = walk == code
    print(f"  {name:62s} {int(m.sum()):7d} units = {100.0 * m.sum() / U:5.1f} %   {int(ulen[m].sum()):9d} entries = {100.0 * ulen[m].sum() / E:5.1f} %")
dead = walk != 0
print(f"  dead units in all: {100.0 * dead.sum() / U:.1f} % of the units, {100.0 * ulen[dead].sum() / E:.1f} % of the entries; "
      f"kind (a) is {100.0 * (walk == 3).sum() / max(int(dead.sum()), 1):.1f} % of the dead units")
if "fwd_close" in st:
    halves = int(st["layout"].tile_w) // 16
    fc = st["fwd_close"].cpu().numpy().astype(np.int64).reshape(-1, 2)[:, :halves]
    closed = (fc >= 0).all(axis=1)
    first_tail = np.where(closed, fc.max(axis=1), np.iinfo(np.int64).max)
    seg = unit - seg_off[seg_tile[unit]]
    tail = seg >= first_tail[seg_tile[unit]]
    zero = (walk == 3) | (walk == 5)
    tz = tail & zero
    print(f"  tail units: {int(tail.sum())} = {100.0 * tail.sum() / U:.1f} % of the units, {int(ulen[tail].sum())} entries = "
          f"{100.0 * ulen[tail].sum() / E:.1f} %; tiles with a tail: {int(np.unique(seg_tile[unit][tail]).size)} of {len(lens)}")
    print(f"  tail zero units: {int(tz.sum())} = {100.0 * tz.sum() / max(int(zero.sum()), 1):.1f} % of the zero units, "
          f"{int(ulen[tz].sum())} entries = {100.0 * ulen[tz].sum() / max(int(ulen[zero].sum()), 1):.1f} % of the zero units' entries, "
          f"{100.0 * ulen[tz].sum() / E:.1f} % of all entries; tail units that are NOT zero units: {int((tail & ~zero).sum())}")
    tt = seg_tile[unit][tail]
    zc = np.bincount(tt, weights=zero[tail].astype(np.float64), minlength=len(lens))
    ac = np.bincount(tt, minlength=len(lens))
    print(f"  tiles whose tail units disagree about the verdict: {int(((zc > 0) & (zc < ac)).sum())}")
else:
    print("  (no saved.fwd_close: the exiting forward did not run, no unit is a tail unit)")
dt = (rec[:, 1].astype(np.int64) - rec[:, 0].astype(np.int64)).astype(np.float64)
span = float(rec[:, 1].max() - rec[:, 0].min())
for code, name in ((0, "general"), (1, "dead, full"), (4, "dead, masked"), (3, "zero units"), (5, "tail exits")):
    m = walk == code
    if m.any():
        print(f"  slot time {name:13s} {dt[m].sum() / 100.0:10.1f} us summed = {100.0 * dt[m].sum() / dt.sum():5.1f} % of all slots' "
              f"({100.0 * m.sum() / U:5.1f} % of the launch slots), mean {dt[m].mean() / 100.0:6.2f} us")
print(f"  all slots: {dt.sum() / 100.0:.1f} us summed over {U} slots; first entry to last exit {span / 100.0:.1f} us")
```

Baseline: 1729 billion.

## Mask all-zero sub-tiles in general backward units and skip zero rows in row-sum

```diff
diff --git a/fresnel_amd/_binding.py b/fresnel_amd/_binding.py
--- a/fresnel_amd/_binding.py
+++ b/fresnel_amd/_binding.py
@@ -15,6 +15,7 @@
 int fgs_backward(FgsDims* dims, ptr cameras pos scale quat color opacity phase saved scratch g_rgb g_depth g_pos g_scale g_quat g_color
                  g_opacity g_phase, stream)
 int fgs_count_pairs(FgsDims* dims, ptr saved out_pairs, stream)
+int fgs_row_sum(FgsDims* dims, ptr saved grad_rows zero_from row_sums, stream)
 int fgs_asm_workspace_bytes(FgsAsmDims* dims, size_t* saved_bytes scratch_bytes)
 int fgs_asm_forward(FgsAsmDims* dims, ptr cameras pos scale quat color opacity phase wavelengths out_rgb saved scratch, stream)
 int fgs_asm_backward(FgsAsmDims* dims, ptr cameras pos scale quat color opacity phase wavelengths saved scratch g_rgb g_pos g_scale
@@ -117,6 +118,7 @@
 FWD_EXIT_OFF, FWD_EXIT_ON = 0x100, 0x200
 BWD_ZERO_OFF, BWD_ZERO_ON = 0x400, 0x800
 BWD_TAIL_OFF, BWD_TAIL_ON = 0x2000, 0x4000
+BWD_SUB_OFF, BWD_SUB_ON = 0x8000, 0x10000
 
 
 class FgsDims(ctypes.Structure):
@@ -322,6 +324,7 @@
     fwd_exit = int(tuning.pop("fwd_exit", 0))
     bwd_zero = int(tuning.pop("bwd_zero", 0))
     bwd_tail = int(tuning.pop("bwd_tail", 0))
+    bwd_sub = int(tuning.pop("bwd_sub", 0))
     for k, v in tuning.items():
         if k not in ("seg_len", "fwd_variant", "bin_mode", "tile_w", "sort_mode"):
             raise FgsError(f"unknown tuning field {k!r}")
@@ -332,8 +335,10 @@
         raise FgsError(f"bwd_zero must be 0, 1 or -1, and 0 with the row-split forward (fwd_variant < 0), got {bwd_zero!r}")
     if bwd_tail not in (0, 1, -1) or (bwd_tail and d.fwd_variant < 0):
         raise FgsError(f"bwd_tail must be 0, 1 or -1, and 0 with the row-split forward (fwd_variant < 0), got {bwd_tail!r}")
+    if bwd_sub not in (0, 1, -1) or (bwd_sub and d.fwd_variant < 0):
+        raise FgsError(f"bwd_sub must be 0, 1 or -1, and 0 with the row-split forward (fwd_variant < 0), got {bwd_sub!r}")
     d.fwd_variant |= ({0: 0, 1: FWD_EXIT_ON, -1: FWD_EXIT_OFF}[fwd_exit] | {0: 0, 1: BWD_ZERO_ON, -1: BWD_ZERO_OFF}[bwd_zero]
-                      | {0: 0, 1: BWD_TAIL_ON, -1: BWD_TAIL_OFF}[bwd_tail])
+                      | {0: 0, 1: BWD_TAIL_ON, -1: BWD_TAIL_OFF}[bwd_tail] | {0: 0, 1: BWD_SUB_ON, -1: BWD_SUB_OFF}[bwd_sub])
     d.dup_capacity = int(dup_capacity)
     return d
 
diff --git a/fresnel_amd/csrc/fgs_api.hip b/fresnel_amd/csrc/fgs_api.hip
--- a/fresnel_amd/csrc/fgs_api.hip
+++ b/fresnel_amd/csrc/fgs_api.hip
@@ -203,6 +203,16 @@
     return FGS_OK;
 }
 
+int fgs_row_sum(const FgsDims *dims, const void *saved, const float *grad_rows, const uint32_t *zero_from, float *row_sums,
+                void *stream) {
+    FgsPlan p;
+    const int rc = fgs_make_plan(dims, &p);
+    if (rc) return rc;
+    if (!saved || !grad_rows || !row_sums) { fgs_set_error("fgs_row_sum: null pointer"); return FGS_EINVAL; }
+    if (p.d.use_phase) { fgs_set_error("fgs_row_sum: the blend path only"); return FGS_EUNSUPPORTED; }
+    return fgs_launch_row_sum(p, reinterpret_cast<const char *>(saved), grad_rows, row_sums, zero_from, reinterpret_cast<hipStream_t>(stream));
+}
+
 int fgs_count_pairs(const FgsDims *dims, const void *saved, uint64_t *out_pairs, void *stream) {
     FgsPlan p;
     const int rc = fgs_make_plan(dims, &p);
diff --git a/fresnel_amd/csrc/fgs_composite.hip b/fresnel_amd/csrc/fgs_composite.hip
--- a/fresnel_amd/csrc/fgs_composite.hip
+++ b/fresnel_amd/csrc/fgs_composite.hip
@@ -490,6 +490,9 @@
 __shared__ __attribute__((aligned(16))) float bwd_red[10 * FGS_RED_PITCH];
 __shared__ __attribute__((aligned(16))) float bwd_red_pairs[12 * FGS_RED_PITCH];
 #define FGS_BWD_G __attribute__((address_space(1)))
+#ifdef FGS_BWD_UNIT_TRACE
+__shared__ uint32_t bwd_trace_sub[3];
+#endif
 
 template <int NSX, bool DEAD>
 __device__ __forceinline__ void composite_bwd_walk(const TileCtx &c, uint32_t lane, uint32_t lx, uint32_t ly, uint32_t dcap, uint32_t alive,
@@ -505,6 +508,9 @@
     float fx0 = (float)(c.X0 + lx), fy0 = (float)(c.Y0 + ly);
     asm("" : "+v"(fx0), "+v"(fy0));
     uint32_t e_prev = ~0u;
+#ifdef FGS_BWD_UNIT_TRACE
+    [[maybe_unused]] uint32_t trace_passes = 0u, trace_zero_passes = 0u;
+#endif
     auto reduce_parked = [&]() {
         const float tot = wave_sum_addtid_finish(red, lane, 10u);
         if ((lane & 3u) == 3u && lane < 4u * FGS_BLEND_ROW_FLOATS && e_prev < dcap) ((FGS_BWD_G float *)grad_rows)[(size_t)e_prev * FGS_BLEND_ROW_FLOATS + (lane >> 2)] = tot;
@@ -648,6 +654,9 @@
             e_prev = e;
             const uint32_t fl = __builtin_amdgcn_readfirstlane(__float_as_uint(q2.w));
             const uint32_t msk = fl & alive;
+#ifdef FGS_BWD_UNIT_TRACE
+            trace_passes += __builtin_popcount(fl & ((1u << NS) - 1u)); trace_zero_passes += __builtin_popcount(fl & bwd_trace_sub[0]);
+#endif
             const uint32_t cbits = __float_as_uint(q2.z), rbits = __float_as_uint(q2.w);
             const float ca = q0.z, cbc = q0.w, cd = q1.x, lop = q1.y;
             const float dxa = fx0 - q0.x, dya = fy0 - q0.y, dyb = dya + 8.0f;
@@ -713,6 +722,9 @@
         __syncthreads();
     }
     if constexpr (DEAD) reduce_parked_dead(); else reduce_parked();
+#ifdef FGS_BWD_UNIT_TRACE
+    if (!DEAD) { bwd_trace_sub[1] = trace_passes; bwd_trace_sub[2] = trace_zero_passes; }
+#endif
 }
 
 template <int NSX>
@@ -806,6 +818,19 @@
 }
 
 template <int NSX>
+__device__ __forceinline__ uint32_t composite_bwd_zero_subtiles(const TileCtx &c, uint32_t lx, uint32_t ly, uint32_t W, uint32_t H,
+                                                                const float (&S)[2 * NSX], const float (&T)[2 * NSX]) {
+    uint32_t zero = 0u;
+#pragma unroll
+    for (int s = 0; s < 2 * NSX; ++s) {
+        const uint32_t px = c.X0 + 8u * (s % NSX) + lx, py = c.Y0 + 8u * (s / NSX) + ly;
+        const bool veto = (px < W && py < H && __float_as_uint(T[s]) != 0u) || (__float_as_uint(S[s]) & 0x7FFFFFFFu) != 0u;
+        if (__ballot(veto) == 0ull) zero |= 1u << s;
+    }
+    return zero;
+}
+
+template <int NSX>
 __global__ __launch_bounds__(64) void k_bwd_tail_verdict(
     uint32_t ntiles, uint32_t tiles, uint32_t tiles_x, uint32_t W, uint32_t H, float bg0, float bg1, float bg2, uint32_t dcap,
     const uint32_t *__restrict__ counters, const uint32_t *__restrict__ seg_off, const float *__restrict__ seg_ckpt,
@@ -946,7 +971,7 @@
     }
     if (dead_unit) {
         uint32_t walk = (1u << NS) - 1u;
-        if (zero_units) {
+        if (zero_units & 1u) {
             walk = composite_bwd_nonzero_subtiles<NSX>(S);
             if (walk == 0u) {
                 composite_bwd_zero_rows<NSX>(c, dcap, dup_ids, rec, dup_off, grad_rows);
@@ -962,8 +987,12 @@
         FGS_BWD_TRACE_EXIT(walk == (1u << NS) - 1u ? 1 : 4);
         return;
     }
+#ifdef FGS_BWD_UNIT_TRACE
+    bwd_trace_sub[0] = seg != 0 && !(t_eps > 0.0f) ? composite_bwd_zero_subtiles<NSX>(c, lx, ly, W, H, S, T) : 0u;
+#endif
+    if ((zero_units & 2u) && seg != 0 && !(t_eps > 0.0f)) alive &= ~composite_bwd_zero_subtiles<NSX>(c, lx, ly, W, H, S, T);
     composite_bwd_walk<NSX, false>(c, lane, lx, ly, dcap, alive, dup_ids, rec, dup_off, grad_rows, gr, gg, gb, gd, S, T);
-    FGS_BWD_TRACE_EXIT(0);
+    FGS_BWD_TRACE_EXIT((unsigned long long)bwd_trace_sub[1] << 3 | (unsigned long long)bwd_trace_sub[2] << 16 | (unsigned long long)(bwd_trace_sub[0] != 0u) << 29);
 }
 
 #ifndef FGS_PHASE_SCAN
@@ -1364,7 +1393,7 @@
 #define FGS_BWD_LAUNCH(NSXV)                                                                                              \
     hipLaunchKernelGGL(k_composite_bwd<NSXV>, dim3(ugrid), dim3(64), FGS_BWD_DYN_LDS, st, tiles, tiles_x, W, H, bg0, bg1, bg2, dcap, \
                        counters, seg_off, seg_tile, seg_ckpt, ranges, dup_ids, rec, dup_off, pix, g_rgb, g_depth, grad_rows, t_eps, unit_order, fwd_close, \
-                       (uint32_t)p.bwd_zero, (const uint32_t *)zero_from FGS_BWD_TRACE_ARG)
+                       (uint32_t)p.bwd_zero | (p.bwd_sub ? 2u : 0u) , (const uint32_t *)zero_from FGS_BWD_TRACE_ARG)
     if (p.tile_w == 32) FGS_BWD_LAUNCH(4); else FGS_BWD_LAUNCH(2);
 #undef FGS_BWD_LAUNCH
 #undef FGS_BWD_TRACE_ARG
diff --git a/fresnel_amd/csrc/fgs_internal.h b/fresnel_amd/csrc/fgs_internal.h
--- a/fresnel_amd/csrc/fgs_internal.h
+++ b/fresnel_amd/csrc/fgs_internal.h
@@ -29,6 +29,9 @@
                            float *g_scale, float *g_quat, float *g_color, float *g_opacity, float *g_phase,
                            hipStream_t st, float *row_sums = nullptr ,
                            const uint32_t *zero_from = nullptr );
+
+int fgs_launch_row_sum(const FgsPlan &p, const char *saved, const float *grad_rows, float *row_sums,
+                       const uint32_t *zero_from , hipStream_t st);
 
 int fgs_launch_asm_project_bwd(const FgsPlan &p, const float *cams, const float *pos, const float *scale,
                                const float *quat, const float *color, const float *phase, int phase_channels,
diff --git a/fresnel_amd/csrc/fgs_plan.cpp b/fresnel_amd/csrc/fgs_plan.cpp
--- a/fresnel_amd/csrc/fgs_plan.cpp
+++ b/fresnel_amd/csrc/fgs_plan.cpp
@@ -31,11 +31,12 @@
     const int exit_flags = d->fwd_variant >= 0 ? (d->fwd_variant & (FGS_FWD_EXIT_OFF | FGS_FWD_EXIT_ON)) : 0;
     const int zero_flags = d->fwd_variant >= 0 ? (d->fwd_variant & (FGS_BWD_ZERO_OFF | FGS_BWD_ZERO_ON)) : 0;
     const int tail_flags = d->fwd_variant >= 0 ? (d->fwd_variant & (FGS_BWD_TAIL_OFF | FGS_BWD_TAIL_ON)) : 0;
-    const int fv = d->fwd_variant - exit_flags - zero_flags - tail_flags, afv = fv < -16 || fv > 16 ? 3  : (fv < 0 ? -fv : fv);
+    const int sub_flags = d->fwd_variant >= 0 ? (d->fwd_variant & (FGS_BWD_SUB_OFF | FGS_BWD_SUB_ON)) : 0;
+    const int fv = d->fwd_variant - exit_flags - zero_flags - tail_flags - sub_flags, afv = fv < -16 || fv > 16 ? 3  : (fv < 0 ? -fv : fv);
     if (d->seg_len < 0 || d->seg_len > 512 || d->seg_len % 64 != 0 || (afv != 0 && afv != 1 && afv != 2 && afv != 4 && !(fv == 8 || fv == 16)) ||
         d->bin_mode < 0 || d->bin_mode > 2 || (d->tile_w != 0 && d->tile_w != 16 && d->tile_w != 32) || d->sort_mode < 0 || d->sort_mode > 11 ||
         exit_flags == (FGS_FWD_EXIT_OFF | FGS_FWD_EXIT_ON) || zero_flags == (FGS_BWD_ZERO_OFF | FGS_BWD_ZERO_ON) ||
-        tail_flags == (FGS_BWD_TAIL_OFF | FGS_BWD_TAIL_ON)) {
+        tail_flags == (FGS_BWD_TAIL_OFF | FGS_BWD_TAIL_ON) || sub_flags == (FGS_BWD_SUB_OFF | FGS_BWD_SUB_ON)) {
         fgs_set_error("invalid tuning: seg_len=%d fwd_variant=%d bin_mode=%d tile_w=%d sort_mode=%d", d->seg_len, d->fwd_variant,
                       d->bin_mode, d->tile_w, d->sort_mode);
         return FGS_EINVAL;
@@ -147,6 +148,7 @@
     const bool exit_ok = p->fwd_parts > 0 && layers == 1 && segment_ckpt;
     p->fwd_exit = exit_ok && (exit_flags == FGS_FWD_EXIT_ON || (exit_flags == 0 && B * p->tiles * (size_t)(p->tile_w / 16) >= 8192));
     p->bwd_zero = zero_flags == FGS_BWD_ZERO_ON || (zero_flags == 0 && B * p->tiles * (size_t)(p->tile_w / 16) >= 8192);
+    p->bwd_sub = sub_flags == FGS_BWD_SUB_ON || (sub_flags == 0 && p->bwd_zero);
     p->s_fwd_max = o;
     if (p->fwd_exit) {
         p->s_fwd_max = o = align256(o + B * p->tiles * 2 * 4);
diff --git a/fresnel_amd/csrc/fgs_plan.h b/fresnel_amd/csrc/fgs_plan.h
--- a/fresnel_amd/csrc/fgs_plan.h
+++ b/fresnel_amd/csrc/fgs_plan.h
@@ -35,6 +35,7 @@
     bool has_unit_order;
     bool fwd_exit;
     bool bwd_zero;
+    bool bwd_sub;
     bool bwd_tail;
     size_t s_fwd_max;
     size_t sort_words;
diff --git a/fresnel_amd/csrc/fgs_project.hip b/fresnel_amd/csrc/fgs_project.hip
--- a/fresnel_amd/csrc/fgs_project.hip
+++ b/fresnel_amd/csrc/fgs_project.hip
@@ -219,6 +219,7 @@
     out[1] = r1;
 }
 
+#define FGS_ROW_SUM_MASK_ROWS 32u
 __global__ __launch_bounds__(256) __attribute__((amdgpu_waves_per_eu(8, 8))) void k_row_sum(int32_t total, int32_t N, uint32_t dcap,
                                                  const uint32_t *__restrict__ order,
                                                  const uint32_t *__restrict__ dup_off,
@@ -226,7 +227,7 @@
                                                  const float *__restrict__ grad_rows, const float *__restrict__ rec,
                                                  float *__restrict__ sums, const uint32_t *__restrict__ zero_from,
                                                  const uint32_t *__restrict__ zero_min, uint32_t tiles, uint32_t tiles_x,
-                                                 uint32_t tile_w) {
+                                                 uint32_t tile_w, [[maybe_unused]] uint32_t prefetch) {
     const int32_t tid = blockIdx.x * 256 + threadIdx.x;
     const int32_t ri = tid >> 2;
     const uint32_t sub = threadIdx.x & 3u;
@@ -285,6 +286,53 @@
             m[0] += a.x; m[1] += a.y; m[2] += bq.x; m[3] += bq.y; m[4] += cq.x; m[5] += cq.y;
             acc[6] += dq.x; acc[7] += dq.y; acc[8] += eq.x; acc[9] += eq.y;
         };
+        if (prefetch && zf && cnt <= 4u * FGS_ROW_SUM_MASK_ROWS) {
+            const uint32_t mine = cnt > sub ? (cnt - sub + 3u) >> 2 : 0u;
+            uint32_t wmask = 0u;
+            for (uint32_t i0 = 0; i0 < mine; i0 += 4u) {
+                uint32_t z[4];
+#pragma unroll
+                for (uint32_t j = 0; j < 4u; ++j) {
+                    const uint32_t row = sub + 4u * (i0 + j);
+                    const uint32_t ky = (uint32_t)(((float)row + 0.5f) * inv_rw), t = t0 + ky * tiles_x + (row - ky * rw);
+                    z[j] = i0 + j < mine ? (t < tiles ? zf[t] : 0xFFFFFFFFu) : 0u;
+                }
+#pragma unroll
+                for (uint32_t j = 0; j < 4u; ++j)
+                    if (rank < z[j]) wmask |= 1u << (i0 + j);
+            }
+            while (wmask) {
+                const uint32_t i1 = (uint32_t)__builtin_ctz(wmask);
+                wmask &= wmask - 1u;
+                const float2 *r = reinterpret_cast<const float2 *>(base + (size_t)(sub + 4u * i1) * FGS_BLEND_ROW_FLOATS);
+                if (wmask) {
+                    const uint32_t i2 = (uint32_t)__builtin_ctz(wmask);
+                    wmask &= wmask - 1u;
+                    const float2 *r2 = reinterpret_cast<const float2 *>(base + (size_t)(sub + 4u * i2) * FGS_BLEND_ROW_FLOATS);
+                    const float2 a = r[0], bq = r[1], cq = r[2], dq = r[3], eq = r[4];
+                    const float2 a2 = r2[0], bq2 = r2[1], cq2 = r2[2], dq2 = r2[3], eq2 = r2[4];
+                    add_row(a, bq, cq, dq, eq);
+                    add_row(a2, bq2, cq2, dq2, eq2);
+                } else {
+                    add_row(r[0], r[1], r[2], r[3], r[4]);
+                }
+            }
+            k = cnt;
+        } else if (!zf) {
+            for (; k + 4 < cnt; k += 8) {
+                const float2 *r = reinterpret_cast<const float2 *>(base + (size_t)k * FGS_BLEND_ROW_FLOATS);
+                const float2 *r2 = reinterpret_cast<const float2 *>(base + (size_t)(k + 4) * FGS_BLEND_ROW_FLOATS);
+                const float2 a = r[0], bq = r[1], cq = r[2], dq = r[3], eq = r[4];
+                const float2 a2 = r2[0], bq2 = r2[1], cq2 = r2[2], dq2 = r2[3], eq2 = r2[4];
+                add_row(a, bq, cq, dq, eq);
+                add_row(a2, bq2, cq2, dq2, eq2);
+            }
+            if (k < cnt) {
+                const float2 *r = reinterpret_cast<const float2 *>(base + (size_t)k * FGS_BLEND_ROW_FLOATS);
+                add_row(r[0], r[1], r[2], r[3], r[4]);
+            }
+            k = cnt;
+        }
         for (; k + 4 < cnt; k += 8) {
             const float2 *r = reinterpret_cast<const float2 *>(base + (size_t)k * FGS_BLEND_ROW_FLOATS);
             const float2 *r2 = reinterpret_cast<const float2 *>(base + (size_t)(k + 4) * FGS_BLEND_ROW_FLOATS);
@@ -614,6 +662,28 @@
     return FGS_OK;
 }
 
+static uint32_t fgs_row_sum_max_rows(const FgsPlan &p) {
+    const double span = ceil(2.0 * (double)p.d.max_radius);
+    const double cols = fmin(floor(span / (double)p.tile_w) + 1.0, (double)p.L.tiles_x);
+    const double rows = fmin(floor(span / (double)FGS_TILE) + 1.0, (double)p.L.tiles_y);
+    const double n = cols * rows;
+    return n > 4294967295.0 ? 0xFFFFFFFFu : (uint32_t)n;
+}
+
+int fgs_launch_row_sum(const FgsPlan &p, const char *saved, const float *grad_rows, float *row_sums, const uint32_t *zero_from,
+                       hipStream_t st) {
+    const int32_t total = p.d.batch * p.d.num_gaussians;
+    const int grid = (int)(((size_t)total * 4 + 255) / 256);
+    hipLaunchKernelGGL(k_row_sum, dim3(grid), dim3(256), 0, st, total, p.d.num_gaussians, (uint32_t)p.L.dup_capacity,
+                       reinterpret_cast<const uint32_t *>(saved + p.L.order), reinterpret_cast<const uint32_t *>(saved + p.L.dup_off),
+                       reinterpret_cast<const uint32_t *>(saved + p.L.tile_count), grad_rows,
+                       reinterpret_cast<const float *>(saved + p.L.rec), row_sums, zero_from,
+                       zero_from ? zero_from + (size_t)p.d.batch * p.tiles : nullptr, (uint32_t)p.tiles, (uint32_t)p.L.tiles_x,
+                       (uint32_t)p.tile_w, fgs_row_sum_max_rows(p) <= 4u * FGS_ROW_SUM_MASK_ROWS ? 1u : 0u);
+    FGS_LAUNCH_CHECK("k_row_sum");
+    return FGS_OK;
+}
+
 int fgs_launch_project_bwd(const FgsPlan &p, const float *cams, const float *pos, const float *scale,
                            const float *quat, const char *saved, const float *grad_rows, float *g_pos,
                            float *g_scale, float *g_quat, float *g_color, float *g_opacity, float *g_phase,
@@ -627,11 +697,7 @@
     const float *rec = reinterpret_cast<const float *>(saved + p.L.rec);
     if (!p.d.use_phase) {
         if (!row_sums) { fgs_set_error("fgs_launch_project_bwd: the blend path needs the row-sum scratch"); return FGS_EINVAL; }
-        hipLaunchKernelGGL(k_row_sum, dim3(grid), dim3(256), 0, st, total, p.d.num_gaussians,
-                           (uint32_t)p.L.dup_capacity, order, dup_off, tile_count, grad_rows, rec, row_sums,
-                           p.bwd_tail ? zero_from : nullptr, p.bwd_tail && zero_from ? zero_from + (size_t)p.d.batch * p.tiles : nullptr,
-                           (uint32_t)p.tiles, (uint32_t)p.L.tiles_x, (uint32_t)p.tile_w);
-        FGS_LAUNCH_CHECK("k_row_sum");
+        if (const int rc = fgs_launch_row_sum(p, saved, grad_rows, row_sums, p.bwd_tail ? zero_from : nullptr, st)) return rc;
         hipLaunchKernelGGL((k_project_bwd<0, true>), dim3((total + 255) / 256), dim3(256), 0, st, total,
                            p.d.num_gaussians, p.d.num_cameras, (uint32_t)p.L.dup_capacity, cams, pos, scale, quat,
                            depth_key, order, dup_off, tile_count, row_sums, g_pos, g_scale, g_quat, g_color, g_opacity,
diff --git a/include/fgs.h b/include/fgs.h
--- a/include/fgs.h
+++ b/include/fgs.h
@@ -21,6 +21,8 @@
 #define FGS_BWD_ZERO_ON 0x800
 #define FGS_BWD_TAIL_OFF 0x2000
 #define FGS_BWD_TAIL_ON 0x4000
+#define FGS_BWD_SUB_OFF 0x8000
+#define FGS_BWD_SUB_ON 0x10000
 #define FGS_TUNE_AUTO 0
 #ifndef FGS_PHASE_CKPT
 #define FGS_PHASE_CKPT 8
@@ -87,6 +89,9 @@
                  float *g_phase, void *stream);
 
 int fgs_count_pairs(const FgsDims *dims, const void *saved, uint64_t *out_pairs, void *stream);
+
+int fgs_row_sum(const FgsDims *dims, const void *saved, const float *grad_rows, const uint32_t *zero_from, float *row_sums,
+                void *stream);
 
 typedef struct FgsAsmDims {
     int32_t batch, num_gaussians, width, height;
diff --git a/scratch/profile/bwd_zero_units.py b/scratch/profile/bwd_zero_units.py
--- a/scratch/profile/bwd_zero_units.py
+++ b/scratch/profile/bwd_zero_units.py
@@ -12,12 +12,19 @@
 from fresnel_amd import _binding as B
 from fresnel_amd import renderer as R
 
+opacity = None
+if "--opacity" in sys.argv:
+    i = sys.argv.index("--opacity")
+    opacity = float(sys.argv[i + 1])
+    del sys.argv[i:i + 2]
 workload = sys.argv[1] if len(sys.argv) > 1 else "config3"
 distribution = sys.argv[2] if len(sys.argv) > 2 else "saag"
 tuning = sys.argv[3] if len(sys.argv) > 3 else ""
 dev = torch.device("cuda:0")
 N, S, Bn = bench.WORKLOADS[workload]
 pos, scale, quat, col, opa = bench.synth_batch(Bn, N, 1000 * int(workload[-1]), dev, distribution)
+if opacity is not None:
+    opa.fill_(opacity)
 leaves = [t.requires_grad_(True) for t in (pos, scale, quat, col, opa)]
 cam = R.Camera(0.8 * S, 0.8 * S, S / 2, S / 2, S, S)
 ren = R.TileBasedRenderer(S, S).to(dev)
@@ -62,6 +69,14 @@
                    (4, "(b) dead, some but not all sub-tiles all-zero"), (1, "(c) dead, no sub-tile all-zero")):
     m = walk == code
     print(f"  {name:62s} {int(m.sum()):7d} units = {100.0 * m.sum() / U:5.1f} %   {int(ulen[m].sum()):9d} entries = {100.0 * ulen[m].sum() / E:5.1f} %")
+code = (rec[:, 2] >> np.uint64(32)).astype(np.int64)
+gen = walk == 0
+passes, zpasses, has = (code >> 3) & 0x1FFF, (code >> 16) & 0x1FFF, (code >> 29) & 1
+if gen.any():
+    print(f"  general units: {int(passes[gen].sum())} sub-tile passes ({passes[gen].sum() / max(int(ulen[gen].sum()), 1):.2f} per entry), "
+          f"{int(zpasses[gen].sum())} = {100.0 * zpasses[gen].sum() / max(int(passes[gen].sum()), 1):.2f} % in sub-tiles zero at restart; "
+          f"{int(has[gen].sum())} = {100.0 * has[gen].sum() / gen.sum():.1f} % of the general units have such a sub-tile, "
+          f"{int((zpasses[gen] > 0).sum())} of them a pass in one")
 dead = walk != 0
 print(f"  dead units in all: {100.0 * dead.sum() / U:.1f} % of the units, {100.0 * ulen[dead].sum() / E:.1f} % of the entries; "
       f"kind (a) is {100.0 * (walk == 3).sum() / max(int(dead.sum()), 1):.1f} % of the dead units")
```

Result: faster. 1775 billion, median of 6 (+2.7%).
